# huakunyang/SummerTTS

Hardware: AMD Instinct MI355X
Metric: audio samples/sec (acoustic model + vocoder, phoneme ids -> int16 PCM on host), single_speaker_fast-shaped synthetic blob (higher is better)
Workload: dtype f32 (decoder trunk convs AND the reverse flow's WaveNet convs (wn_flow.hip, one-utterance calls): fp32 operands as 2 fp16 terms = 22-23 of their 24 mantissa bits, 3 fp16 MFMA products per fp32 product, f32 accumulation -- measured error in `parity`, same tolerance as the exact-fp32 leg; batches addi

## Files before the change

include/summertts_hip.h:

```cpp
#ifndef SUMMERTTS_HIP_H_
#define SUMMERTTS_HIP_H_

#include <stdint.h>

#ifdef __cplusplus
extern "C" {
#endif

typedef struct sts_engine sts_engine;

enum {
    STS_OK = 0,
    STS_EINVAL = -1,
    STS_EMODEL = -2,
    STS_EDEVICE = -3,
    STS_ESTATE = -4
};

int sts_create(const float* blob, int64_t blob_bytes, int device, sts_engine** out);
void sts_destroy(sts_engine* e);

int sts_speaker_num(const sts_engine* e);

typedef struct sts_model_info {
    int32_t is_multi_speaker, lang_type, dur_pred_type, dec_type;
    int32_t vocab, hidden, inter_channels, speaker_num, gin_channels;
    int32_t samples_per_frame;
    int32_t sample_rate;
    int64_t blob_floats_consumed;
} sts_model_info;
int sts_get_info(const sts_engine* e, sts_model_info* info);

int sts_infer_ids(sts_engine* e, const int32_t* ids, int32_t n, int32_t sid, float length_scale,
                  int16_t** pcm_out, int32_t* n_out);

typedef int (*sts_chunk_cb)(void* user, const int16_t* pcm, int32_t n_samples, int32_t sample_offset);
int sts_infer_ids_stream(sts_engine* e, const int32_t* ids, int32_t n, int32_t sid, float length_scale,
                         int32_t chunk_frames, sts_chunk_cb cb, void* user, int32_t* n_total);
int sts_stream_halo_frames(const sts_engine* e);

typedef int (*sts_batch_chunk_cb)(void* user, int32_t utt, const int16_t* pcm, int32_t n_samples, int32_t sample_offset);
int sts_infer_ids_batch_stream(sts_engine* e, int32_t B, const int32_t* const* ids, const int32_t* n, const int32_t* sid,
                               const float* length_scale, int32_t chunk_frames, sts_batch_chunk_cb cb, void* user,
                               int32_t* n_total);

int sts_infer_ids_batch(sts_engine* e, int32_t B, const int32_t* const* ids, const int32_t* n,
                        const int32_t* sid, const float* length_scale, int16_t** pcm_out, int32_t* n_out);

int sts_run_batch(sts_engine* e, int32_t B, const int32_t* const* ids, const int32_t* n, const int32_t* sid,
                  const float* length_scale, int32_t* n_out, int64_t* total_out);
int sts_set_host_pcm(sts_engine* e, int enable);
int sts_copy_pcm_device(sts_engine* e, void* device_dst, int64_t capacity_samples);
int sts_copy_pcm_host(sts_engine* e, int16_t* host_dst, int64_t capacity_samples);
int sts_pcm_host_view(sts_engine* e, const int16_t** pcm, int64_t* count);

int sts_set_forced_durations(sts_engine* e, const int32_t* dur, int64_t count);
int sts_set_noise(sts_engine* e, float noise_scale, float noise_scale_w, uint64_t seed);
int sts_get_noise(const sts_engine* e, float* noise_scale, float* noise_scale_w, uint64_t* seed);
int sts_set_output_rate(sts_engine* e, int32_t rate);
int sts_get_output_rate(const sts_engine* e);
int sts_resample_table(int32_t in_rate, int32_t out_rate, int32_t* P, int32_t* Q, int32_t* taps, float* table, int64_t capacity_floats);
#define STS_LOUD_OFF 0
#define STS_LOUD_MEASURE 1
#define STS_LOUD_NORMALIZE 2
typedef struct sts_loudness { float lufs; float peak; float gain; int32_t blocks; } sts_loudness;
int sts_set_loudness(sts_engine* e, int mode, float target_lufs, float peak_dbfs);
int sts_get_loudness_mode(const sts_engine* e, int* mode, float* target_lufs, float* peak_dbfs);
int sts_get_loudness(sts_engine* e, sts_loudness* out, int64_t capacity);
int sts_kweight_coeffs(int32_t rate, double coeffs[10]);
int sts_loudness_measure(int device, const float* x, const int64_t* lengths, int32_t B, int32_t rate,
                         float target_lufs, float peak_dbfs, sts_loudness* out);
#define STS_LIMITER_OFF 0
#define STS_LIMITER_ON 1
typedef struct sts_limiter_stats { float gain; float min_gain; float peak_out; int32_t limited; } sts_limiter_stats;
int sts_set_limiter(sts_engine* e, int mode, float gain_db, float ceiling_dbfs, float lookahead_ms);
int sts_get_limiter_mode(const sts_engine* e, int* mode, float* gain_db, float* ceiling_dbfs, float* lookahead_ms);
int sts_get_limiter(sts_engine* e, sts_limiter_stats* out, int64_t capacity);
int sts_limiter_design(int32_t rate, float gain_db, float ceiling_dbfs, float lookahead_ms, int32_t* H, double* c, double* G);
int sts_limiter_apply(int device, const float* x, const int64_t* lengths, int32_t B, int32_t rate, float gain_db, float ceiling_dbfs,
                      float lookahead_ms, float* y, int16_t* pcm, sts_limiter_stats* stats);
int sts_set_record_taps(sts_engine* e, int enable);
int sts_get_tap(sts_engine* e, const char* name, float** data, int32_t* channels, int64_t* length);
int sts_get_durations(sts_engine* e, int32_t* dur, int64_t capacity);
int sts_set_conv_mode(sts_engine* e, int mode);
int sts_set_conv_math(sts_engine* e, int mode);

enum { STS_DBG_ATTN_BLOCK_MIN_WGS = 1,
       STS_DBG_TAIL_FUSED = 14 ,
       STS_DBG_UPS_ROWPH = 15 ,
       STS_DBG_CHAIN_STREAMS = 13 ,
       STS_DBG_H2P = 11 ,
       STS_DBG_H2P_TILE = 12 ,
       STS_DBG_MEMO_CLEAR = 10 ,
       STS_DBG_PCM_DIRECT = 9 ,
       STS_DBG_DDS_TAIL = 8 ,
       STS_DBG_ATTN_REG = 7 ,
       STS_DBG_LAUNCH_AHEAD = 6 ,
       STS_DBG_FLOW_FUSED = 5  };
enum { STS_DBG_STREAM_RETRY_STEP = 16, STS_DBG_STREAM_DIRECT = 17 };
enum { STS_DBG_POISON = 18 };
int sts_debug_set(sts_engine* e, int key, int value);

typedef struct sts_profile {
    float ms_text_encoder, ms_duration, ms_flow, ms_decoder, ms_total_device;
    float ms_decoder_mfma;
    int32_t decoder_mfma_launches;
    double flops_text_encoder, flops_duration, flops_flow, flops_decoder;
    double flops_decoder_mfma;
    double bytes_decoder_min;
    int64_t frames, samples, phonemes;
    double flops_decoder_mfma_executed;
    double bytes_text_encoder, bytes_duration, bytes_flow;
    float ms_sync_wait_host;
    double flops_decoder_bf16_issued;
    int64_t conv_math_fallbacks;
    int32_t conv_math_pinned;
    int32_t launch_ahead;
    int64_t launch_ahead_misses;
    float us_host_setup;
    float us_host_enqueue;
    float us_host_tail;
    int64_t poison_bytes;
} sts_profile;
int sts_set_profiling(sts_engine* e, int enable);
#define STS_ABI_VERSION 13
int sts_abi_version(void);
int sts_build_flags(void);
int sts_get_profile(const sts_engine* e, sts_profile* p);
int sts_get_profile_ex(const sts_engine* e, void* p, int64_t size_bytes);

int sts_debug_conv1d(int device, const float* x, int32_t Cin, int32_t L, const float* w, const float* bias,
                     int32_t Cout, int32_t k, int32_t pad, int32_t dil, int32_t stride_transposed,
                     int32_t depthwise, float in_slope, int32_t in_act, int mode, float** y, int32_t* Lout);

int sts_debug_conv1d_bench(int device, const float* x, int32_t Cin, int32_t L, const float* w, const float* bias,
                           int32_t Cout, int32_t k, int32_t pad, int32_t dil, int32_t stride_transposed,
                           int32_t depthwise, float in_slope, int32_t in_act, int mode, float** y, int32_t* Lout,
                           int32_t iters, float* ms_out);

int sts_debug_conv_h2p(int device, const float* x, int32_t Cin, int32_t L, const float* w, const float* bias, int32_t Cout, int32_t k,
                       int32_t dil, const float* res, float in_slope, float out_slope, int tile, int members, float* y, float* y16,
                       float* yp, int32_t iters, float* ms_out);

int sts_debug_conv_h2w(int device, const float* x, int32_t C, int32_t L, const float* w, const float* bias, int32_t k, int32_t dil, const float* res,
                       float in_slope, float out_slope, int members, float* y, float* y16, int32_t iters, float* ms_out);

void sts_free(void* p);
const char* sts_last_error(void);

int sts_debug_wino_pack(const float* w, int32_t Cout, int32_t k, int32_t Cin, float* out, int64_t out_floats);

typedef struct sts_pool sts_pool;
int sts_pool_create(const float* blob, int64_t blob_bytes, int device, int n_engines, int max_batch, sts_pool** out);
void sts_pool_destroy(sts_pool* p);
int64_t sts_pool_submit(sts_pool* p, const int32_t* ids, int32_t n, int32_t sid, float length_scale);
int sts_pool_wait(sts_pool* p, int64_t ticket, int16_t** pcm_out, int32_t* n_out);
int sts_pool_stats(sts_pool* p, int64_t* batches, int64_t* requests);
const char* sts_pool_last_error(void);
int64_t sts_pool_submit_ex(sts_pool* p, const int32_t* ids, int32_t n, int32_t sid, float length_scale, float noise_scale,
                           float noise_scale_w, uint64_t seed);
int sts_pool_set_output_rate(sts_pool* p, int32_t rate);
int64_t sts_pool_submit_stream(sts_pool* p, const int32_t* ids, int32_t n, int32_t sid, float length_scale, float noise_scale,
                               float noise_scale_w, uint64_t seed, int32_t chunk_frames, sts_chunk_cb cb, void* user);
int sts_pool_set_loudness(sts_pool* p, int mode, float target_lufs, float peak_dbfs);
int sts_pool_set_limiter(sts_pool* p, int mode, float gain_db, float ceiling_dbfs, float lookahead_ms);

typedef struct sts_multi sts_multi;
int sts_multi_create(const float* blob, int64_t blob_bytes, const int32_t* devices, int32_t n_devices, sts_multi** out);
enum { STS_MULTI_AUTO = 0, STS_MULTI_RCCL = 1, STS_MULTI_DOWNLOAD = 2 };
int sts_multi_create_ex(const float* blob, int64_t blob_bytes, const int32_t* devices, int32_t n_devices, int32_t flags, sts_multi** out);
int sts_multi_gather_mode(const sts_multi* m);
int sts_multi_rccl_ranks(sts_multi* m);
double sts_multi_last_gather_ms(const sts_multi* m);
int sts_multi_set_conv_math(sts_multi* m, int mode);
int sts_multi_set_noise(sts_multi* m, float noise_scale, float noise_scale_w, uint64_t seed);
int sts_multi_set_output_rate(sts_multi* m, int32_t rate);
int sts_multi_set_loudness(sts_multi* m, int mode, float target_lufs, float peak_dbfs);
int sts_multi_set_limiter(sts_multi* m, int mode, float gain_db, float ceiling_dbfs, float lookahead_ms);
int sts_multi_set_rccl_library(const char* path, int allow_repeated_devices);
int64_t sts_multi_gather_layout(const int64_t* counts, int32_t n_ranks, int64_t* offsets);
void sts_multi_destroy(sts_multi* m);
int sts_multi_device_count(const sts_multi* m);
int sts_multi_speaker_num(const sts_multi* m);
int sts_multi_infer_ids_batch(sts_multi* m, int32_t B, const int32_t* const* ids, const int32_t* n, const int32_t* sid,
                              const float* length_scale, int16_t** pcm_out, int32_t* n_out);
int sts_multi_shard_of(const sts_multi* m, int32_t B, const int32_t* n, int32_t* device_slot_out);
const char* sts_multi_last_error(void);

#ifdef __cplusplus
}
#endif
#endif
```

summertts_amd/csrc/capi.hip:

```cpp
#include <stdlib.h>
#include <string.h>

#include <algorithm>
#include <new>
#include <string>
#include <vector>

#include "engine.hpp"

using namespace sts;

struct sts_engine { Engine eng; };

static thread_local std::string g_err;
static int set_err(int code, const std::string& s) { g_err = s; return code; }

extern "C" {

const char* sts_last_error(void) { return g_err.c_str(); }
void sts_free(void* p) { free(p); }

int sts_create(const float* blob, int64_t blob_bytes, int device, sts_engine** out) {
    if (!out) return set_err(STS_EINVAL, "sts_create: null out pointer");
    *out = nullptr;
// ... 19 lines not shown
    info->vocab = m.vocab; info->hidden = m.hidden; info->inter_channels = m.inter;
    info->speaker_num = m.spk_num == 0 ? 1 : m.spk_num; info->gin_channels = m.gin;
    info->samples_per_frame = m.hop_total; info->sample_rate = kNativeRate;
    info->blob_floats_consumed = m.consumed;
    return STS_OK;
}

int sts_run_batch(sts_engine* e, int32_t B, const int32_t* const* ids, const int32_t* n, const int32_t* sid,
                  const float* length_scale, int32_t* n_out, int64_t* total_out) {
    if (!e) return set_err(STS_EINVAL, "null engine");
    int rc = e->eng.run(B, ids, n, sid, length_scale);
    if (rc != STS_OK) return set_err(rc, e->eng.error());
    if (n_out) for (int b = 0; b < B; b++) n_out[b] = e->eng.n_samples[b];
    if (total_out) *total_out = e->eng.total_samples;
    return STS_OK;
}

int sts_copy_pcm_device(sts_engine* e, void* dst, int64_t cap) {
    if (!e || !dst) return set_err(STS_EINVAL, "null argument");
    if (cap < e->eng.total_samples || !e->eng.d_pcm) return set_err(STS_ESTATE, "destination too small or no run yet");
    if (hipMemcpyAsync(dst, e->eng.pcm_in_host_ ? (const void*)e->eng.h_pcm : (const void*)e->eng.d_pcm, (size_t)e->eng.total_samples * 2,
                       e->eng.pcm_in_host_ ? hipMemcpyHostToDevice : hipMemcpyDeviceToDevice, e->eng.stream) != hipSuccess ||
        hipStreamSynchronize(e->eng.stream) != hipSuccess)
        return set_err(STS_EDEVICE, "device copy failed");
    return STS_OK;
}

int sts_copy_pcm_host(sts_engine* e, int16_t* dst, int64_t cap) {
    if (!e || !dst) return set_err(STS_EINVAL, "null argument");
    if (cap < e->eng.total_samples || !e->eng.d_pcm) return set_err(STS_ESTATE, "destination too small or no run yet");
    if (e->eng.h_pcm) { memcpy(dst, e->eng.h_pcm, (size_t)e->eng.total_samples * 2); return STS_OK; }
    if (hipMemcpyAsync(dst, e->eng.d_pcm, (size_t)e->eng.total_samples * 2, hipMemcpyDeviceToHost, e->eng.stream) != hipSuccess ||
        hipStreamSynchronize(e->eng.stream) != hipSuccess)
        return set_err(STS_EDEVICE, "device-to-host copy failed");
    return STS_OK;
}

int sts_pcm_host_view(sts_engine* e, const int16_t** pcm, int64_t* count) {
    if (!e || !pcm || !count) return set_err(STS_EINVAL, "null argument");
    if (!e->eng.h_pcm || !e->eng.d_pcm) return set_err(STS_ESTATE, "no host copy of the PCM (sts_set_host_pcm(e, 1) before the run)");
    *pcm = e->eng.h_pcm; *count = e->eng.total_samples;
    return STS_OK;
}

int sts_infer_ids_batch(sts_engine* e, int32_t B, const int32_t* const* ids, const int32_t* n, const int32_t* sid,
                        const float* length_scale, int16_t** pcm_out, int32_t* n_out) {
    if (!pcm_out || !n_out) return set_err(STS_EINVAL, "null output");
    int64_t total = 0;
    if (!e) return set_err(STS_EINVAL, "null engine");
    const bool was = e->eng.host_pcm;
    e->eng.host_pcm = true;
    int rc = sts_run_batch(e, B, ids, n, sid, length_scale, n_out, &total);
    e->eng.host_pcm = was;
    if (rc != STS_OK) return rc;
    int16_t* all = (int16_t*)malloc((size_t)(total > 0 ? total : 1) * 2);
    if (!all) return set_err(STS_EDEVICE, "out of host memory");
    rc = sts_copy_pcm_host(e, all, total);
    if (rc != STS_OK) { free(all); return rc; }
    int64_t off = 0;
    for (int b = 0; b < B; b++) {
        if (B == 1) { pcm_out[0] = all; break; }
        pcm_out[b] = (int16_t*)malloc((size_t)(n_out[b] > 0 ? n_out[b] : 1) * 2);
        if (!pcm_out[b]) {
            for (int q = 0; q < b; q++) { free(pcm_out[q]); pcm_out[q] = nullptr; }
            free(all);
            return set_err(STS_EDEVICE, "out of host memory");
        }
        memcpy(pcm_out[b], all + off, (size_t)n_out[b] * 2);
        off += n_out[b];
    }
    if (B != 1) free(all);
    return STS_OK;
}

int sts_infer_ids(sts_engine* e, const int32_t* ids, int32_t n, int32_t sid, float length_scale, int16_t** pcm_out,
                  int32_t* n_out) {
    const int32_t* idp[1] = {ids};
    return sts_infer_ids_batch(e, 1, idp, &n, &sid, &length_scale, pcm_out, n_out);
}

int sts_infer_ids_stream(sts_engine* e, const int32_t* ids, int32_t n, int32_t sid, float length_scale, int32_t chunk_frames,
                         sts_chunk_cb cb, void* user, int32_t* n_total) {
    if (!e || !ids || !cb) return set_err(STS_EINVAL, "null argument");
    const int32_t* idp[1] = {ids};
    StreamSpec ss{chunk_frames, cb, user};
    const int rc = e->eng.run(1, idp, &n, &sid, &length_scale, &ss);
    if (rc != STS_OK) return set_err(rc, e->eng.error());
    if (n_total) *n_total = (int32_t)e->eng.total_samples;
    return STS_OK;
}

int sts_infer_ids_batch_stream(sts_engine* e, int32_t B, const int32_t* const* ids, const int32_t* n, const int32_t* sid,
                               const float* length_scale, int32_t chunk_frames, sts_batch_chunk_cb cb, void* user, int32_t* n_total) {
    if (!e) return set_err(STS_EINVAL, "null engine");
    if (B < 1 || !ids || !n || chunk_frames <= 0 || !cb) return set_err(STS_EINVAL, "B >= 1, ids, n, a positive chunk size and a callback are required");
    const int rc = e->eng.run_batch_stream(B, ids, n, sid, length_scale, chunk_frames, cb, user, n_total);
    if (rc != STS_OK) return set_err(rc, e->eng.error());
    return STS_OK;
}

int sts_stream_halo_frames(const sts_engine* e) {
    if (!e) return set_err(STS_EINVAL, "null engine");
    return e->eng.stream_halo();
}

int sts_set_forced_durations(sts_engine* e, const int32_t* dur, int64_t count) {
    if (!e) return set_err(STS_EINVAL, "null engine");
    if (!dur || count <= 0) { e->eng.have_forced = false; return STS_OK; }
    e->eng.forced_dur.assign(dur, dur + count);
    e->eng.have_forced = true;
    return STS_OK;
}

int sts_set_noise(sts_engine* e, float noise_scale, float noise_scale_w, uint64_t seed) {
    if (!e) return set_err(STS_EINVAL, "null engine");
    if (!noise_scale_valid(noise_scale) || !noise_scale_valid(noise_scale_w)) return set_err(STS_EINVAL, "noise scales must be finite and >= 0");
    e->eng.noise = Engine::Noise{noise_scale, noise_scale_w, seed};
    return STS_OK;
}
int sts_get_noise(const sts_engine* e, float* noise_scale, float* noise_scale_w, uint64_t* seed) {
    if (!e) return set_err(STS_EINVAL, "null engine");
    if (noise_scale) *noise_scale = e->eng.noise.ns;
    if (noise_scale_w) *noise_scale_w = e->eng.noise.nsw;
    if (seed) *seed = e->eng.noise.seed;
    return STS_OK;
}
int sts_set_record_taps(sts_engine* e, int enable) { if (!e) return set_err(STS_EINVAL, "null engine"); e->eng.record_taps = enable != 0; return STS_OK; }
int sts_set_conv_math(sts_engine* e, int mode) {
    if (!e) return set_err(STS_EINVAL, "null engine");
    if (mode < 0 || mode > 3) return set_err(STS_EINVAL, "conv math: 0 = split-bf16 (default), 1 = exact fp32, 2 = split-bf16 wherever eligible, 3 = two-term fp16");
    e->eng.conv_math = mode;
    e->eng.h2_consecutive = 0; e->eng.h2_disabled = false;
    return STS_OK;
}
int sts_set_conv_mode(sts_engine* e, int mode) { if (!e) return set_err(STS_EINVAL, "null engine"); e->eng.conv_mode = mode; return STS_OK; }
int sts_debug_set(sts_engine* e, int key, int value) {
    if (!e) return set_err(STS_EINVAL, "null engine");
    switch (key) {
        case STS_DBG_ATTN_BLOCK_MIN_WGS: if (value < 1) return set_err(STS_EINVAL, "threshold must be >= 1"); e->eng.attn_block_min_wgs = value; return STS_OK;
        case STS_DBG_FLOW_FUSED: e->eng.flow_fused = value != 0; return STS_OK;
        case STS_DBG_LAUNCH_AHEAD: if (value < 0 || value > 2) return set_err(STS_EINVAL, "launch_ahead must be 0, 1 or 2"); if ((value == 2) != (e->eng.launch_ahead == 2)) { e->eng.seen_tf_.clear(); e->eng.seen_order_.clear(); } e->eng.launch_ahead = value; return STS_OK;
        case STS_DBG_H2P: e->eng.h2p = value < 0 ? 0 : (value > 4 ? 4 : value); return STS_OK;
        case STS_DBG_H2P_TILE: e->eng.h2p_tile = value; return STS_OK;
        case STS_DBG_CHAIN_STREAMS: e->eng.chain_streams_dbg = value; return STS_OK;
        case STS_DBG_TAIL_FUSED: e->eng.tail_fused = value != 0; return STS_OK;
        case STS_DBG_UPS_ROWPH: e->eng.ups_rowph = value != 0; return STS_OK;
        case STS_DBG_MEMO_CLEAR: e->eng.seen_tf_.clear(); e->eng.seen_order_.clear(); return STS_OK;
        case STS_DBG_ATTN_REG: e->eng.attn_reg = value != 0; return STS_OK;
        case STS_DBG_DDS_TAIL: e->eng.dds_tail = value != 0; return STS_OK;
        case STS_DBG_PCM_DIRECT: e->eng.pcm_direct = value != 0; return STS_OK;
        case STS_DBG_STREAM_RETRY_STEP: e->eng.stream_retry_step = value < 0 ? -1 : value; return STS_OK;
        case STS_DBG_STREAM_DIRECT: e->eng.stream_direct = value != 0; return STS_OK;
        case STS_DBG_POISON: e->eng.poison = (unsigned)value; return STS_OK;
        default: return set_err(STS_EINVAL, "unknown debug key");
    }
}
int sts_set_host_pcm(sts_engine* e, int enable) { if (!e) return set_err(STS_EINVAL, "null engine"); e->eng.host_pcm = enable != 0; return STS_OK; }
int sts_set_profiling(sts_engine* e, int enable) { if (!e) return set_err(STS_EINVAL, "null engine"); e->eng.profiling = enable == 2 ? 2 : (enable != 0 ? 1 : 0); return STS_OK; }

int sts_abi_version(void) { return STS_ABI_VERSION; }

int sts_set_output_rate(sts_engine* e, int32_t rate) {
    if (!e) return set_err(STS_EINVAL, "null engine");
    const int rc = e->eng.set_output_rate(rate);
    return rc == STS_OK ? STS_OK : set_err(rc, e->eng.error());
}
int sts_get_output_rate(const sts_engine* e) {
    if (!e) return set_err(STS_EINVAL, "null engine");
    return e->eng.out_rate;
}
int sts_resample_table(int32_t in_rate, int32_t out_rate, int32_t* P, int32_t* Q, int32_t* taps, float* table, int64_t capacity_floats) {
    ResampleDesign d;
    if (!resample_design(in_rate, out_rate, &d)) return set_err(STS_EINVAL, "rates must be integers in [8000, 48000] with P = out / gcd(in, out) <= 1024");
    const int64_t need = (int64_t)d.P * 2 * d.K;
    if (table && capacity_floats < need) return set_err(STS_EINVAL, "table capacity below P * taps floats");
    if (P) *P = d.P;
    if (Q) *Q = d.Q;
    if (taps) *taps = 2 * d.K;
    if (table) resample_table(d, in_rate, out_rate, table);
    return STS_OK;
}
int sts_set_loudness(sts_engine* e, int mode, float target_lufs, float peak_dbfs) {
    if (!e) return set_err(STS_EINVAL, "null engine");
    const int rc = e->eng.set_loudness(mode, target_lufs, peak_dbfs);
    return rc == STS_OK ? STS_OK : set_err(rc, e->eng.error());
}
int sts_get_loudness_mode(const sts_engine* e, int* mode, float* target_lufs, float* peak_dbfs) {
    if (!e) return set_err(STS_EINVAL, "null engine");
    if (mode) *mode = e->eng.loud_mode;
    if (target_lufs) *target_lufs = e->eng.loud_target;
    if (peak_dbfs) *peak_dbfs = e->eng.loud_peak;
    return STS_OK;
}
int sts_get_loudness(sts_engine* e, sts_loudness* out, int64_t capacity) {
    if (!e) return set_err(STS_EINVAL, "null engine");
    const int64_t n = (int64_t)e->eng.loud_res.size();
    if (!out) return (int)n;
    if (capacity < n) return set_err(STS_EINVAL, "capacity below the last call's utterance count");
    if (n > 0) memcpy(out, e->eng.loud_res.data(), (size_t)n * sizeof(sts_loudness));
    return (int)n;
}
int sts_kweight_coeffs(int32_t rate, double coeffs[10]) {
    if (!coeffs) return set_err(STS_EINVAL, "null argument");
    if (!kweight_coeffs(rate, coeffs)) return set_err(STS_EINVAL, "rate must be an integer in [8000, 48000]");
    return STS_OK;
}
int sts_loudness_measure(int device, const float* x, const int64_t* lengths, int32_t B, int32_t rate, float target_lufs, float peak_dbfs,
                         sts_loudness* out) {
    if (B < 1 || !lengths || !out) return set_err(STS_EINVAL, "B >= 1, lengths and out are required");
    if (!loudness_args_valid(2, target_lufs, peak_dbfs)) return set_err(STS_EINVAL, "target in [-70, 0] LUFS, ceiling in [-30, 0] dBFS");
    LoudArgs a{};
    if (!loud_coef(rate, &a.k)) return set_err(STS_EINVAL, "rate must be an integer in [8000, 48000]");
    std::vector<int> len(B);
    int64_t total = 0, maxl = 0;
    for (int b = 0; b < B; b++) {
        if (lengths[b] < 0 || lengths[b] > (int64_t)1 << 30) return set_err(STS_EINVAL, "lengths must be in [0, 2^30]");
        len[b] = (int)lengths[b]; total += lengths[b]; maxl = std::max<int64_t>(maxl, lengths[b]);
    }
    if (total > 0 && !x) return set_err(STS_EINVAL, "null signal");
    if (hipSetDevice(device) != hipSuccess) return set_err(STS_EDEVICE, "no such device");
    const size_t ws = loud_ws_bytes(B, total), xb = (((size_t)total * 4 + 255) & ~(size_t)255), lb = (((size_t)B * 4 + 255) & ~(size_t)255);
    const size_t ob = (size_t)B * sizeof(sts_loudness);
    char* d = nullptr;
    if (hipMalloc((void**)&d, xb + lb + ob + ws) != hipSuccess) return set_err(STS_EDEVICE, "out of device memory");
    hipStream_t st = nullptr;
    bool ok = hipStreamCreate(&st) == hipSuccess;
    a.x = (const float*)d; a.len = (const int*)(d + xb); a.ilen = 0; a.scale = 1; a.P = 1; a.Q = 1;
    a.target = target_lufs; a.ceiling = peak_dbfs;
    a.out = (float*)(d + xb + lb);
    loud_ws_carve(a, d + xb + lb + ob, B, total);
    ok = ok && (total == 0 || hipMemcpyAsync(d, x, (size_t)total * 4, hipMemcpyHostToDevice, st) == hipSuccess) &&
         hipMemcpyAsync(d + xb, len.data(), (size_t)B * 4, hipMemcpyHostToDevice, st) == hipSuccess;
    if (ok) {
        loudness_run(a, B, maxl, nullptr, st);
        ok = hipGetLastError() == hipSuccess && hipMemcpyAsync(out, a.out, ob, hipMemcpyDeviceToHost, st) == hipSuccess &&
             hipStreamSynchronize(st) == hipSuccess;
    }
    if (st) (void)hipStreamDestroy(st);
    (void)hipFree(d);
    return ok ? STS_OK : set_err(STS_EDEVICE, "loudness measurement failed on the device");
}
int sts_set_limiter(sts_engine* e, int mode, float gain_db, float ceiling_dbfs, float lookahead_ms) {
    if (!e) return set_err(STS_EINVAL, "null engine");
    const int rc = e->eng.set_limiter(mode, gain_db, ceiling_dbfs, lookahead_ms);
    return rc == STS_OK ? STS_OK : set_err(rc, e->eng.error());
}
int sts_get_limiter_mode(const sts_engine* e, int* mode, float* gain_db, float* ceiling_dbfs, float* lookahead_ms) {
    if (!e) return set_err(STS_EINVAL, "null engine");
    if (mode) *mode = e->eng.lim_mode;
    if (gain_db) *gain_db = e->eng.lim_gain_db;
    if (ceiling_dbfs) *ceiling_dbfs = e->eng.lim_ceiling;
    if (lookahead_ms) *lookahead_ms = e->eng.lim_ms;
    return STS_OK;
}
int sts_get_limiter(sts_engine* e, sts_limiter_stats* out, int64_t capacity) {
    if (!e) return set_err(STS_EINVAL, "null engine");
    const int64_t n = (int64_t)e->eng.lim_res.size();
    if (!out) return (int)n;
    if (capacity < n) return set_err(STS_EINVAL, "capacity below the last call's utterance count");
    if (n > 0) memcpy(out, e->eng.lim_res.data(), (size_t)n * sizeof(sts_limiter_stats));
    return (int)n;
}
int sts_limiter_design(int32_t rate, float gain_db, float ceiling_dbfs, float lookahead_ms, int32_t* H, double* c, double* G) {
    LimiterDesign d;
    if (!limiter_design(rate, gain_db, ceiling_dbfs, lookahead_ms, &d))
        return set_err(STS_EINVAL, "rate in [8000, 48000], gain in [-40, 40] dB, ceiling in [-30, 0] dBFS, look-ahead in [0.25, 10] ms");
    if (H) *H = d.H;
    if (c) *c = d.c;
    if (G) *G = d.G;
    return STS_OK;
}
int sts_limiter_apply(int device, const float* x, const int64_t* lengths, int32_t B, int32_t rate, float gain_db, float ceiling_dbfs,
                      float lookahead_ms, float* y, int16_t* pcm, sts_limiter_stats* stats) {
    if (B < 1 || !lengths) return set_err(STS_EINVAL, "B >= 1 and lengths are required");
    LimiterDesign dsg;
    if (!limiter_design(rate, gain_db, ceiling_dbfs, lookahead_ms, &dsg))
        return set_err(STS_EINVAL, "rate in [8000, 48000], gain in [-40, 40] dB, ceiling in [-30, 0] dBFS, look-ahead in [0.25, 10] ms");
    std::vector<int> len(B);
    int64_t total = 0, maxl = 0;
    for (int b = 0; b < B; b++) {
        if (lengths[b] < 0 || lengths[b] > (int64_t)1 << 30) return set_err(STS_EINVAL, "lengths must be in [0, 2^30]");
        len[b] = (int)lengths[b]; total += lengths[b]; maxl = std::max<int64_t>(maxl, lengths[b]);
    }
    if (total > (int64_t)1 << 30) return set_err(STS_EINVAL, "the signals must hold at most 2^30 samples in all");
    if (total > 0 && !x) return set_err(STS_EINVAL, "null signal");
    if (hipSetDevice(device) != hipSuccess) return set_err(STS_EDEVICE, "no such device");
    const size_t xb = (((size_t)total * 4 + 255) & ~(size_t)255), lb = (((size_t)B * 4 + 255) & ~(size_t)255);
    const size_t pb = (((size_t)total * 2 + 255) & ~(size_t)255), sb = (((size_t)B * 16 + 255) & ~(size_t)255);
    char* d = nullptr;
    if (hipMalloc((void**)&d, 2 * xb + lb + pb + sb + 256) != hipSuccess) return set_err(STS_EDEVICE, "out of device memory");
    hipStream_t st = nullptr;
    bool ok = hipStreamCreate(&st) == hipSuccess;
    LimArgs a{};
    a.x = (const float*)d; a.len = (const int*)(d + xb); a.ilen = 0; a.scale = 1; a.P = 1; a.Q = 1;
    a.H = dsg.H; a.c = dsg.c; a.G = dsg.G; a.gloud = nullptr;
    a.y = y ? (float*)(d + xb + lb) : nullptr;
    a.pcm = pcm ? (int16_t*)(d + 2 * xb + lb) : nullptr;
    a.stat = (unsigned*)(d + 2 * xb + lb + pb);
    std::vector<unsigned> raw((size_t)B * 4);
    ok = ok && (total == 0 || hipMemcpyAsync(d, x, (size_t)total * 4, hipMemcpyHostToDevice, st) == hipSuccess) &&
         hipMemcpyAsync(d + xb, len.data(), (size_t)B * 4, hipMemcpyHostToDevice, st) == hipSuccess;
    if (ok) {
        limiter_run(a, B, maxl, st);
        ok = hipGetLastError() == hipSuccess &&
             (!y || total == 0 || hipMemcpyAsync(y, a.y, (size_t)total * 4, hipMemcpyDeviceToHost, st) == hipSuccess) &&
             (!pcm || total == 0 || hipMemcpyAsync(pcm, a.pcm, (size_t)total * 2, hipMemcpyDeviceToHost, st) == hipSuccess) &&
// ... 351 lines not shown
```

summertts_amd/csrc/conv.hip:

```cpp
#include "kernels.hpp"
#include "devmath.hpp"
#include "conv_common.hpp"

namespace sts {

__device__ __forceinline__ float load_in(const ConvArgs& a, const float* xrow, int pos, int in_len, int orig_len) {
    if (pos < 0 || pos >= in_len) return 0.f;
    int src = pos;
    if (a.in_reflect) {
        src = pos - 1;
        if (src < 0) { if (orig_len > 1) src = 1; else return 0.f; }
    }
    float v = xrow[src];
    if (a.in_act) v = v < 0.f ? v * a.in_slope : v;
    return v;
}

#ifndef STS_EXP
#define STS_EXP 0
#endif

#ifndef STS_RA_GROUP
#define STS_RA_GROUP 3
#endif
template <int MW, int NW, int WM, int WN, int RA = 3>
__device__ __forceinline__ void conv_mfma_body(const ConvArgs& a, const int mtiles, const int bx, const int by, const int b) {
    constexpr int MT = 32 * MW * WM, NT = 32 * NW * WN, NTHR = WM * WN * 64;
    extern __shared__ __attribute__((aligned(16))) float smem[];
    const int orig_len = uni(seg_len(a.in_seg, b));
    const int in_len = orig_len + (a.in_reflect ? 1 : 0);
    const int out_len = uni(seg_len(a.out_seg, b));
    const int n_count = a.transposed ? in_len + a.n_extra : out_len;
    const int n0 = bx * NT;
    if (n0 >= n_count) return;
    const int phase = by / mtiles;
    const int m0 = (by - phase * mtiles) * MT;
    const size_t in_base = (size_t)uni(seg_start(a.in_seg, b)), out_base = (size_t)uni(seg_start(a.out_seg, b));
    const float* const xbase = uni(a.x);
    const long x_ld = uni(a.x_ld);
    const int tid = threadIdx.x, lane = tid & 63, wave = tid >> 6;
    const int wm = wave / WN, wn = wave % WN;
    const int l31 = lane & 31, half = lane >> 5;

    const int first = a.tap_off, last = a.tap_off + (a.ntap - 1) * a.tap_step;
    const int lo = first < last ? first : last, hi = first < last ? last : first;
    const int W = NT + (hi - lo);
    constexpr int WIN = NT + MAX_HALO;
    constexpr int ldsw = WIN;
    const int win0 = n0 + lo;

    const float* w = a.w + (size_t)phase * a.ntap * a.Cin_pad * a.Cout_pad;
    const int mbase = m0 + wm * MW * 32;
    f32x16 acc[MW][NW];
#pragma unroll
    for (int i = 0; i < MW; i++)
#pragma unroll
        for (int j = 0; j < NW; j++)
#pragma unroll
            for (int r = 0; r < 16; r++) acc[i][j][r] = 0.f;

    const int nchunk = a.Cin_pad / CK;
    const int nsteps = nchunk * a.ntap;

    const rsrc_t wrs = make_rsrc(w, (unsigned)((size_t)a.ntap * a.Cin_pad * a.Cout_pad * 4));
    const unsigned a_voff = (unsigned)(((size_t)half * a.Cout_pad + mbase + l31) * 4);
    auto load_a = [&](int c, int j, float (&dst)[CK / 2][MW]) {
        const unsigned sbase = (unsigned)((((size_t)j * a.Cin_pad + (size_t)c * CK) * a.Cout_pad) * 4);
#pragma unroll
        for (int p = 0; p < CK / 2; p++)
#pragma unroll
            for (int i = 0; i < MW; i++)
                dst[p][i] = __builtin_bit_cast(float, __builtin_amdgcn_raw_buffer_load_b32(
                    wrs, (int)a_voff, (int)(sbase + (unsigned)(2 * p) * (unsigned)a.Cout_pad * 4u + (unsigned)i * 128u), 0));
    };
    auto load_b = [&](int bufi, int j, float (&dst)[CK / 2][NW]) {
        const float* sb = smem + bufi * (CK * ldsw);
        const int bcol0 = wn * NW * 32 + l31 + j * a.tap_step + a.tap_off - lo;
#pragma unroll
        for (int p = 0; p < CK / 2; p++)
#pragma unroll
            for (int q = 0; q < NW; q++) dst[p][q] = sb[(2 * p + half) * ldsw + bcol0 + q * 32];
    };

    constexpr int RI = (NT + MAX_HALO + NTHR - 1) / NTHR;
    unsigned xoff[RI];
#pragma unroll
    for (int i = 0; i < RI; i++) {
        const int col = tid + i * NTHR;
        const int pos = win0 + col;
        bool v = col < W && pos >= 0 && pos < in_len;
        int src = pos;
        if (a.in_reflect) { src = pos - 1; if (src < 0) { src = 1; v = v && orig_len > 1; } }
        xoff[i] = v ? (unsigned)src * 4u : kOOB;
    }
    float xr[CK][RI];
    int sj = 0, sc = 0;
    auto load_x = [&](int c) {
        if (STS_EXP & 1) { if (c > 0) return; }
#pragma unroll
        for (int i = 0; i < RI; i++)
            if ((i + 1) * NTHR <= WIN || tid < WIN - i * NTHR) {
#pragma unroll
                for (int r = 0; r < CK; r++) {
                    const int ci = c * CK + r;
                    const rsrc_t rs = make_rsrc(xbase + (size_t)ci * x_ld + in_base, ci < a.Cin ? (unsigned)orig_len * 4u : 0u);
                    xr[r][i] = buf_load(rs, xoff[i]);
                }
            }
    };
    auto store_tile = [&](int bufi) {
        if (STS_EXP & 8) { if (bufi >= 0 && sc > 0) return; }
        float* sb = smem + bufi * (CK * ldsw);
#pragma unroll
        for (int i = 0; i < RI; i++)
            if ((i + 1) * NTHR <= WIN || tid < WIN - i * NTHR) {
#pragma unroll
                for (int r = 0; r < CK; r++) {
                    float v = xr[r][i];
                    if (a.in_act) v = v < 0.f ? v * a.in_slope : v;
                    sb[r * ldsw + tid + i * NTHR] = v;
                }
            }
    };

    constexpr int UNR = (RA % 2 == 0) ? RA : 2 * RA;
    float fa[RA][CK / 2][MW], fb[2][CK / 2][NW];
    int aj = 0, ac = 0;
    auto request_a = [&](float (&dst)[CK / 2][MW]) {
        if (!(STS_EXP & 2) || (ac == 0 && aj < 2)) load_a(ac, aj, dst);
        if (++aj == a.ntap) { aj = 0; ac++; }
    };
    auto do_step = [&](float (&acur)[CK / 2][MW], float (&anew)[CK / 2][MW], float (&bcur)[CK / 2][NW],
                       float (&bnxt)[CK / 2][NW], int s) {
        const bool last_tap = sj + 1 == a.ntap;
        int nj = sj + 1, nc = sc;
        if (last_tap) { nj = 0; nc = sc + 1; }
        request_a(anew);
        {
            if (last_tap && s + 1 < nsteps) {
                store_tile(nc & 1);
                if (!(STS_EXP & 4)) __syncthreads();
                if (nc + 1 < nchunk) load_x(nc + 1);
            }
            if (!(STS_EXP & 16)) load_b(nc & 1, nj, bnxt);
        }
#pragma unroll
        for (int p = 0; p < CK / 2; p++)
#pragma unroll
            for (int i = 0; i < MW; i++)
#pragma unroll
                for (int q = 0; q < NW; q++)
                    acc[i][q] = __builtin_amdgcn_mfma_f32_32x32x2f32(acur[p][i], bcur[p][q], acc[i][q], 0, 0, 0);
        sj = nj; sc = nc;
    };
// ... 499 lines not shown
            if (ns == nseg) { ns = 0; nh = sh + 1; if (nh == 2) { nh = 0; nc = sc + 1; } }
            const bool more = s + 1 < nsteps;
            const bool three = ss < n3;
            float v[4];
            load_a(sc, sh, ss, 3, fa[3]);
#pragma unroll
            for (int p = 0; p < 4; p++) v[p] = X[0][p] - X[2][p];
#pragma unroll
            for (int p = 0; p < 4; p++) acc[0] = __builtin_amdgcn_mfma_f32_32x32x2f32(fa[0][p], v[p], acc[0], 0, 0, 0);
            load_a(nc, nh, ns, 0, fa[0]);
#pragma unroll
            for (int p = 0; p < 4; p++) v[p] = X[1][p] + X[2][p];
#pragma unroll
            for (int p = 0; p < 4; p++) acc[1] = __builtin_amdgcn_mfma_f32_32x32x2f32(fa[1][p], v[p], acc[1], 0, 0, 0);
            load_a(nc, nh, ns, 1, fa[1]);
#pragma unroll
            for (int p = 0; p < 4; p++) v[p] = X[2][p] - X[1][p];
#pragma unroll
            for (int p = 0; p < 4; p++) acc[2] = __builtin_amdgcn_mfma_f32_32x32x2f32(fa[2][p], v[p], acc[2], 0, 0, 0);
            load_a(nc, nh, ns, 2, fa[2]);
#pragma unroll
            for (int p = 0; p < 4; p++) v[p] = X[1][p] - X[3][p];
            if (more) {
                if (nc != sc) {
                    store_x(nc & 1, 1);
                    __syncthreads();
                    if (nc + 1 < nchunk) load_x(nc + 1, 0);
                } else if (nh != sh) {
                    if (sc + 1 < nchunk) { store_x((sc + 1) & 1, 0); load_x(sc + 1, 1); }
                }
                load_xv(nc & 1, nh, ns);
            }
            if (three) {
#pragma unroll
                for (int p = 0; p < 4; p++) acc[3] = __builtin_amdgcn_mfma_f32_32x32x2f32(fa[3][p], v[p], acc[3], 0, 0, 0);
            }
            ss = ns; sh = nh; sc = nc;
        }
    }
    __syncthreads();
    {
        const int q = l31 / d, rr = l31 - q * d;
        const int pa = 60 * wn + 2 * d * q + rr, pb = pa + d;
        const int ga = n0 - h2 + pa, gb = n0 - h2 + pb;
        const bool ia = ga >= 0 && ga < len, ib = gb >= 0 && gb < len;
        if (l31 < 30) {
            float b1v[16];
#pragma unroll
            for (int r = 0; r < 16; r++) b1v[r] = a.b1 ? a.b1[m0 + (r & 3) + 8 * (r >> 2) + 4 * half] : 0.f;
            static_for<0, 16>([&](auto rc) {
                constexpr int r = decltype(rc)::value;
                const int row = m0 + (r & 3) + 8 * (r >> 2) + 4 * half;
                const float bv = b1v[r];
                float ya = acc[0][r] + acc[1][r] + acc[2][r] + bv;
                float yb = acc[1][r] - acc[2][r] - acc[3][r] + bv;
                ya = ya < 0.f ? ya * G.slope : ya;
                yb = yb < 0.f ? yb * G.slope : yb;
                t1[row * LD2 + (pa & 1) * H2 + (pa >> 1)] = ia ? ya : 0.f;
                t1[row * LD2 + (pb & 1) * H2 + (pb >> 1)] = ib ? yb : 0.f;
            });
        }
#pragma unroll
        for (int i = 0; i < 4; i++)
#pragma unroll
            for (int r = 0; r < 16; r++) acc[i][r] = 0.f;
    }
    __syncthreads();

    {
        int n3, n2; wino_split(a.k2, &n3, &n2);
        const int nseg = n3 + n2, nsteps = nchunk * 2 * nseg;
        const rsrc_t wrs = make_rsrc(a.wu2, (unsigned)(nseg * 4 * C * C * 4));
        auto load_a = [&](int c, int h, int sg, int xi, float (&dst)[4]) {
            const unsigned sbase = ((unsigned)sg * 4u + (unsigned)xi) * xi_stride + (unsigned)((c * CK + h * 8) * C) * 4u;
#pragma unroll
            for (int p = 0; p < 4; p++)
                dst[p] = __builtin_bit_cast(float, __builtin_amdgcn_raw_buffer_load_b32(wrs, (int)a_voff, (int)(sbase + (unsigned)(2 * p * C * 4)), 0));
        };
        auto load_xv = [&](int c, int h, int sg) {
            const int j0 = sg < n3 ? 3 * sg : 3 * n3 + 2 * (sg - n3);
            const float* sb = t1 + (c * CK + h * 8 + half) * LD2 + 30 * wn + l31;
#pragma unroll
            for (int m = 0; m < 4; m++) {
                const int j = j0 + m;
                const float* sm = sb + (j & 1) * H2 + (j >> 1);
#pragma unroll
                for (int p = 0; p < 4; p++) X[m][p] = sm[2 * p * LD2];
            }
        };
        int sc = 0, sh = 0, ss = 0;
        load_a(0, 0, 0, 0, fa[0]);
        load_a(0, 0, 0, 1, fa[1]);
        load_a(0, 0, 0, 2, fa[2]);
        load_xv(0, 0, 0);
        for (int s = 0; s < nsteps; s++) {
            int ns = ss + 1, nh = sh, nc = sc;
            if (ns == nseg) { ns = 0; nh = sh + 1; if (nh == 2) { nh = 0; nc = sc + 1; } }
            const bool more = s + 1 < nsteps;
            const bool three = ss < n3;
            float v[4];
            load_a(sc, sh, ss, 3, fa[3]);
#pragma unroll
            for (int p = 0; p < 4; p++) v[p] = X[0][p] - X[2][p];
#pragma unroll
            for (int p = 0; p < 4; p++) acc[0] = __builtin_amdgcn_mfma_f32_32x32x2f32(fa[0][p], v[p], acc[0], 0, 0, 0);
            load_a(nc, nh, ns, 0, fa[0]);
#pragma unroll
            for (int p = 0; p < 4; p++) v[p] = X[1][p] + X[2][p];
#pragma unroll
            for (int p = 0; p < 4; p++) acc[1] = __builtin_amdgcn_mfma_f32_32x32x2f32(fa[1][p], v[p], acc[1], 0, 0, 0);
            load_a(nc, nh, ns, 1, fa[1]);
#pragma unroll
            for (int p = 0; p < 4; p++) v[p] = X[2][p] - X[1][p];
#pragma unroll
            for (int p = 0; p < 4; p++) acc[2] = __builtin_amdgcn_mfma_f32_32x32x2f32(fa[2][p], v[p], acc[2], 0, 0, 0);
            load_a(nc, nh, ns, 2, fa[2]);
#pragma unroll
            for (int p = 0; p < 4; p++) v[p] = X[1][p] - X[3][p];
            load_xv(more ? nc : 0, nh, ns);
            if (three) {
#pragma unroll
                for (int p = 0; p < 4; p++) acc[3] = __builtin_amdgcn_mfma_f32_32x32x2f32(fa[3][p], v[p], acc[3], 0, 0, 0);
            }
            ss = ns; sh = nh; sc = nc;
        }
    }
    if (l31 < 30) {
        const int oa = 60 * wn + 2 * l31, ob = oa + 1;
        const bool va = oa < NT && n0 + oa < len, vb = ob < NT && n0 + ob < len;
        const size_t opos = base + (size_t)(n0 + oa);
        static_for<0, 2>([&](auto hc) {
            constexpr int hb = decltype(hc)::value * 8;
            float b2v[8], xa[8], xb[8];
#pragma unroll
            for (int r = 0; r < 8; r++) {
                const int row = m0 + ((hb + r) & 3) + 8 * ((hb + r) >> 2) + 4 * half;
                const size_t o = (size_t)row * G.ld + opos;
                b2v[r] = a.b2 ? a.b2[row] : 0.f;
                xa[r] = va ? a.x[o] : 0.f;
                xb[r] = vb ? a.x[o + 1] : 0.f;
            }
            static_for<0, 8>([&](auto rc) {
                constexpr int r = decltype(rc)::value;
                const int row = m0 + ((hb + r) & 3) + 8 * ((hb + r) >> 2) + 4 * half;
                const float bv = b2v[r];
                const float ya = acc[0][hb + r] + acc[1][hb + r] + acc[2][hb + r] + bv;
                const float yb = acc[1][hb + r] - acc[2][hb + r] - acc[3][hb + r] + bv;
                const size_t o = (size_t)row * G.ld + opos;
                if (va) a.y[o] = ya + xa[r];
                if (vb) a.y[o + 1] = yb + xb[r];
            });
        });
    }
}

template <int MW, int NW>
__global__ __launch_bounds__(1024) void conv_mfma_splitk_kernel(ConvArgs a, int mtiles) {
    constexpr int G = 4, E = MW * NW * 16;
    constexpr int D = MW * NW == 1 ? 6 : (MW * NW == 2 ? 4 : 3);
    extern __shared__ __attribute__((aligned(16))) float red[];
    const int KS = blockDim.x >> 6;
    const int nsl = a.kslices > 1 ? a.kslices : 1;
    const int b = blockIdx.z / nsl, slice = blockIdx.z - b * nsl;
    const int orig_len = seg_len(a.in_seg, b);
    const int in_len = orig_len + (a.in_reflect ? 1 : 0);
    const int out_len = seg_len(a.out_seg, b);
    const int n_count = a.transposed ? in_len + a.n_extra : out_len;
    const int n0 = blockIdx.x * 32 * NW;
    if (n0 >= n_count) return;
    const int phase = blockIdx.y / mtiles;
    const int m0 = (blockIdx.y - phase * mtiles) * 32 * MW;
    const size_t in_base = (size_t)seg_start(a.in_seg, b), out_base = (size_t)seg_start(a.out_seg, b);
    const int tid = threadIdx.x, lane = tid & 63, wave = tid >> 6;
    const int l31 = lane & 31, half = lane >> 5;
    const float* w = a.w + (size_t)phase * a.ntap * a.Cin_pad * a.Cout_pad;
    bool mvalid[MW];
#pragma unroll
    for (int i = 0; i < MW; i++) mvalid[i] = (m0 + i * 32) < a.Cout_pad;

    f32x16 acc[MW][NW];
#pragma unroll
    for (int i = 0; i < MW; i++)
#pragma unroll
        for (int q = 0; q < NW; q++)
#pragma unroll
            for (int r = 0; r < 16; r++) acc[i][q][r] = 0.f;

    const int gpt = a.Cin_pad / (2 * G);
    const int gall = a.ntap * gpt;
    const int gper = (gall + nsl - 1) / nsl;
    const int gfirst = slice * gper;
    const int ngroups = (STS_EXP & 64) ? gfirst : (gfirst + gper < gall ? gfirst + gper : gall);
    float ra[D][G][MW], rb[D][G][NW];
    const int swave = __builtin_amdgcn_readfirstlane(wave);
    const int sKS = __builtin_amdgcn_readfirstlane(KS);
    const rsrc_t xrs = make_rsrc(a.x + in_base, (unsigned)(((size_t)(a.Cin - 1) * a.x_ld + orig_len) * 4));
    const rsrc_t wrs = make_rsrc(w, (unsigned)((size_t)a.ntap * a.Cin_pad * a.Cout_pad * 4));
    const unsigned ld4 = (unsigned)a.x_ld * 4u;
    const unsigned x_lane = (unsigned)half * ld4;
    const unsigned a_lane = (unsigned)(((size_t)half * a.Cout_pad + m0 + l31) * 4);
    const int lanepos = n0 + l31;
    int lj = (gfirst + swave) / gpt, lc = (gfirst + swave - lj * gpt) * 2 * G;
    const int jstep = sKS / gpt, cstep = (sKS - jstep * gpt) * 2 * G;

    auto load_group = [&](float (&fa)[G][MW], float (&fb)[G][NW]) {
        const int shift = lj * a.tap_step + a.tap_off;
        unsigned off[NW];
#pragma unroll
        for (int q = 0; q < NW; q++) {
            int pos = lanepos + q * 32 + shift;
            bool v = pos >= 0 && pos < in_len;
            if (a.in_reflect) { pos = pos - 1; if (pos < 0) { pos = 1; v = v && orig_len > 1; } }
            off[q] = v ? (unsigned)pos * 4u + x_lane : kOOB;
        }
        const unsigned xs0 = (unsigned)lc * ld4;
        const unsigned ws0 = (unsigned)((((size_t)lj * a.Cin_pad + lc) * a.Cout_pad) * 4);
#pragma unroll
        for (int i = 0; i < G; i++) {
            const bool cv = lc + 2 * i + half < a.Cin;
#pragma unroll
            for (int q = 0; q < NW; q++)
                fb[i][q] = __builtin_bit_cast(float, __builtin_amdgcn_raw_buffer_load_b32(xrs, (int)(cv ? off[q] : kOOB), (int)(xs0 + (unsigned)(2 * i) * ld4), 0));
#pragma unroll
            for (int k = 0; k < MW; k++)
                fa[i][k] = __builtin_bit_cast(float, __builtin_amdgcn_raw_buffer_load_b32(
                    wrs, (int)a_lane, (int)(ws0 + (unsigned)(2 * i) * (unsigned)a.Cout_pad * 4u + (unsigned)k * 128u), 0));
        }
        lj += jstep; lc += cstep;
        if (lc >= a.Cin_pad) { lc -= a.Cin_pad; lj++; }
    };

    int gnext = gfirst + swave;
#pragma unroll
    for (int d = 0; d < D; d++) { if (gnext < ngroups) load_group(ra[d], rb[d]); gnext += sKS; }
    int gcur = gfirst + swave;
    while (gcur < ngroups) {
#pragma unroll
        for (int d = 0; d < D; d++) {
            if (gcur < ngroups) {
#pragma unroll
                for (int i = 0; i < G; i++) {
                    float bq[NW];
#pragma unroll
                    for (int q = 0; q < NW; q++) {
                        float v = rb[d][i][q];
                        if (a.in_act) v = v < 0.f ? v * a.in_slope : v;
                        bq[q] = v;
                    }
#pragma unroll
                    for (int k = 0; k < MW; k++)
#pragma unroll
                        for (int q = 0; q < NW; q++)
                            acc[k][q] = __builtin_amdgcn_mfma_f32_32x32x2f32(ra[d][i][k], bq[q], acc[k][q], 0, 0, 0);
                }
                if (gnext < ngroups) load_group(ra[d], rb[d]);
            }
            gnext += sKS; gcur += sKS;
        }
    }

    static_for<0, MW>([&](auto ic) {
        constexpr int i = decltype(ic)::value;
        static_for<0, NW>([&](auto qc) {
            constexpr int q = decltype(qc)::value;
            static_for<0, 16>([&](auto rc) {
                constexpr int r = decltype(rc)::value;
                red[((size_t)wave * E + (i * NW + q) * 16 + r) * 64 + lane] = acc[i][q][r];
            });
        });
    });
    __syncthreads();
    const int out_off = a.out_off + phase;
    const bool gate = a.epi == EPI_GATE;
    for (int e = wave; e < E; e += KS) {
        const int i = e / (NW * 16);
        const int q = (e >> 4) % NW, r = e & 15;
        if (gate && r >= 8) continue;
        const int n = n0 + q * 32 + l31;
        const int pos = n * a.out_stride + out_off;
        if (n >= n_count || pos < 0 || pos >= out_len) continue;
        const size_t opos = out_base + (size_t)pos;
        const int rowp = m0 + i * 32 + (r & 3) + 8 * (r >> 2) + 4 * half;
        float v = 0.f, v2 = 0.f;
        for (int k = 0; k < KS; k++) {
            v += red[((size_t)k * E + (i * NW + q) * 16 + r) * 64 + lane];
            if (gate) v2 += red[((size_t)k * E + (i * NW + q) * 16 + r + 8) * 64 + lane];
        }
        if (gate) {
            if (!mvalid[i]) continue;
            if (a.bias) { v += a.bias[rowp]; v2 += a.bias[rowp + 16]; }
            if (a.ubias) { v += a.ubias[(size_t)rowp * a.ubias_ld + b]; v2 += a.ubias[(size_t)(rowp + 16) * a.ubias_ld + b]; }
            const int ch = (rowp >> 5) * 16 + (rowp & 15);
            if (ch < a.H) a.y[(size_t)ch * a.y_ld + opos] = tanh_ref(v) * sigmoid_ref(v2);
        } else {
            if (rowp >= a.Cout) continue;
            if (nsl > 1) {
                if (slice == 0) { if (a.bias) v += a.bias[rowp]; if (a.ubias) v += a.ubias[(size_t)rowp * a.ubias_ld + b]; }
                a.y[(size_t)slice * a.kslice_stride + (size_t)rowp * a.y_ld + opos] = v;
                continue;
            }
            if (a.bias) v += a.bias[rowp];
            if (a.ubias) v += a.ubias[(size_t)rowp * a.ubias_ld + b];
            epi_scalar(a, rowp, opos, v);
        }
    }
}

struct TileCfg { int MW, NW, WM, WN; };
static const TileCfg kTiles[] = {
    {2, 2, 2, 2},
    {2, 2, 1, 4},
    {1, 4, 1, 4},
    {2, 1, 1, 4},
    {1, 1, 1, 4},
    {1, 2, 1, 4},
};
constexpr int kNumTiles = 6;

bool conv_mfma_eligible(const ConvArgs& a) {
    if (a.depthwise) return false;
    if (a.Cin < 32) return false;
    if (a.Cout < 8 && a.max_n >= 4096) return false;
    if (a.Cin_pad % CK != 0 || a.Cout_pad % 32 != 0) return false;
    int first = a.tap_off, last = a.tap_off + (a.ntap - 1) * a.tap_step;
    int halo = first < last ? last - first : first - last;
    if (halo > MAX_HALO) return false;
    if (a.epi == EPI_GATE && !a.gate_perm) return false;
    if (a.epi == EPI_TANH_PCM) return false;
    return true;
}

static int pick_tile(const ConvArgs& a, int nphase) {
    const long nt = (a.max_n + 127) / 128;
    if (a.Cout_pad % 64 == 0 && nt * (a.Cout_pad / 64) * nphase * a.B >= 512) return 3;
    return 4;
}

template <int MW, int NW, int WM, int WN>
static void launch_mfma(const ConvArgs& a, int nphase, hipStream_t st) {
    constexpr int MT = 32 * MW * WM, NT = 32 * NW * WN;
    const int mt = (a.Cout_pad + MT - 1) / MT;
    const int nx = (a.max_n + NT - 1) / NT, ny = mt * nphase;
    size_t lds = (size_t)2 * CK * (NT + MAX_HALO) * sizeof(float);
    hipLaunchKernelGGL((conv_mfma_kernel<MW, NW, WM, WN>), dim3(mapped_grid(nx, ny, a.B)), dim3(WM * WN * 64), lds, st, a, mt, nx, ny);
}

template <int MW, int NW>
static void launch_splitk(const ConvArgs& a, int nphase, hipStream_t st) {
    const int mt = (a.Cout_pad + 32 * MW - 1) / (32 * MW);
    const int nt = (a.max_n + 32 * NW - 1) / (32 * NW);
    const int nsl = a.kslices > 1 ? a.kslices : 1;
    const long steps = ((long)a.ntap * (a.Cin_pad / 8) + nsl - 1) / nsl;
    constexpr int E = MW * NW * 16;
    const bool sparse = (long)mt * nt * nphase * a.B * nsl <= 256;
    const int ks_cap = E <= 16 ? 16 : (E <= 32 ? (sparse ? 16 : 8) : 4);
    int ks = 1;
    while (ks < ks_cap && steps / (ks * 2) >= 6 && (long)mt * nt * nphase * a.B * nsl * ks * 2 <= 4096) ks *= 2;
    dim3 grid(nt, mt * nphase, a.B * nsl);
    size_t lds = (size_t)ks * E * 64 * sizeof(float);
    hipLaunchKernelGGL((conv_mfma_splitk_kernel<MW, NW>), grid, dim3(ks * 64), lds, st, a, mt);
}

template <int MW, int NW, int WM, int WN>
static void launch_mfma_group(const ConvGroup& G, hipStream_t st) {
    constexpr int MT = 32 * MW * WM, NT = 32 * NW * WN;
    const ConvArgs& a = G.g[0];
    const int mt = (a.Cout_pad + MT - 1) / MT;
    const int nx = (a.max_n + NT - 1) / NT;
    size_t lds = (size_t)2 * CK * (NT + MAX_HALO) * sizeof(float);
    hipLaunchKernelGGL((conv_mfma_group_kernel<MW, NW, WM, WN>), dim3(mapped_grid(nx, mt, a.B * G.n)), dim3(WM * WN * 64), lds, st, G,
                       mt, a.B, nx, mt);
}

bool resblock_layer_eligible(const ResLayerGroup& G) {
    if (G.n < 1 || G.n > kMaxGroup || (G.C != 32 && G.C != 64 && G.C != 128) || G.max_n <= 0 || G.B <= 0) return false;
    for (int i = 0; i < G.n; i++) {
        const ResLayerArgs& a = G.g[i];
        if (!(a.k1 & 1) || !(a.k2 & 1) || a.k1 < 1 || a.k2 < 1) return false;
        if (a.dil1 * (a.k1 - 1) > RL_XW - RL_W1 || a.k2 - 1 > 32) return false;
        if (a.x == a.y) return false;
    }
    return true;
}

void resblock_layer(const ResLayerGroup& Gin, hipStream_t st) {
    ResLayerGroup G = Gin;
    for (int i = 1; i < G.n; i++)
        for (int j = i; j > 0 && G.g[j].k1 + G.g[j].k2 > G.g[j - 1].k1 + G.g[j - 1].k2; j--) {
            ResLayerArgs t = G.g[j]; G.g[j] = G.g[j - 1]; G.g[j - 1] = t;
        }
    int nx = 0;
    for (int i = 0; i < G.n; i++) {
        const int NT = RL_W1 - (G.g[i].k2 - 1);
        const int n = (G.max_n + NT - 1) / NT;
        if (n > nx) nx = n;
    }
    const size_t stage = (size_t)2 * CK * RL_XW, park = (size_t)G.C * RL_W1 + 64;
    const size_t lds = (stage > park ? stage : park) * sizeof(float);
    const dim3 grid(mapped_grid(nx, 1, G.B * G.n));
    if (G.C == 32) hipLaunchKernelGGL((resblock_layer_kernel<1, 1>), grid, dim3(256), lds, st, G, nx);
    else if (G.C == 64) hipLaunchKernelGGL((resblock_layer_kernel<2, 1>), grid, dim3(256), lds, st, G, nx);
    else hipLaunchKernelGGL((resblock_layer_kernel<2, 2>), grid, dim3(512), lds, st, G, nx);
}

bool conv_wino_eligible(const ConvArgs& a) {
    if (!a.wu || a.transposed || a.depthwise || a.in_reflect || a.out_stride != 1 || a.out_off != 0) return false;
    const int d = a.tap_step;
    if (d <= 0 || d > 6 || 30 % d != 0 || a.ntap < 2) return false;
    if (a.Cin_pad % CK != 0 || a.Cout_pad % 32 != 0 || a.Cin < 32) return false;
    if ((a.ntap - 1) * d > MAX_HALO || 121 + d * ((a.ntap + 1) / 2) >= WINO_H) return false;
    if (a.epi == EPI_GATE || a.epi == EPI_TANH_PCM) return false;
    int n3, n2; wino_split(a.ntap, &n3, &n2);
    return n3 == a.wino_n3 && n2 == a.wino_n2 && n3 >= 0;
}
static size_t wino_lds() { return (size_t)2 * CK * WINO_LD * sizeof(float); }
void conv_wino(const ConvArgs& a, hipStream_t st) {
    if (a.max_n <= 0 || a.B <= 0) return;
    const int nx = (a.max_n + WINO_NT - 1) / WINO_NT, ny = a.Cout_pad / 32;
    hipLaunchKernelGGL(conv_wino_kernel, dim3(mapped_grid(nx, ny, a.B)), dim3(256), wino_lds(), st, a, nx, ny);
}
void wino_pack(const float* w, long s_out, long s_tap, long s_in, int Cout, int k, int Cin, int Cin_pad, int Cout_pad, float* dst) {
    int n3, n2; wino_split(k, &n3, &n2);
    const int nseg = n3 + n2;
    const size_t slab = (size_t)Cin_pad * Cout_pad;
    for (size_t i = 0; i < (size_t)nseg * 4 * slab; i++) dst[i] = 0.f;
    for (int sg = 0; sg < nseg; sg++) {
        const int j0 = sg < n3 ? 3 * sg : 3 * n3 + 2 * (sg - n3), len = sg < n3 ? 3 : 2;
        for (int o = 0; o < Cout; o++)
            for (int ci = 0; ci < Cin; ci++) {
                double g[3] = {0, 0, 0};
                for (int t = 0; t < len; t++) g[t] = (double)w[(size_t)o * s_out + (size_t)(j0 + t) * s_tap + (size_t)ci * s_in];
                const double u[4] = {g[0], 0.5 * (g[0] + g[1] + g[2]), 0.5 * (g[0] - g[1] + g[2]), g[2]};
                for (int xi = 0; xi < 4; xi++) dst[((size_t)sg * 4 + xi) * slab + (size_t)ci * Cout_pad + o] = (float)u[xi];
            }
    }
}

bool resblock_wino_eligible(const ResLayerGroup& G) {
    if (!resblock_layer_eligible(G)) return false;
    for (int i = 0; i < G.n; i++) {
        const ResLayerArgs& a = G.g[i];
        if (!a.wu1 || !a.wu2 || a.k1 < 2 || a.k2 < 2 || a.k2 > 15) return false;
        if (a.dil1 < 1 || a.dil1 > 6 || 30 % a.dil1 != 0 || (a.k1 - 1) * a.dil1 > MAX_HALO) return false;
    }
    return true;
}

template <int WM, int WN>
static void launch_resblock_wino(const ResLayerGroup& G, hipStream_t st) {
    constexpr int P = 60 * WN, LD1 = 2 * (30 * WN + 40), LD2 = 2 * (30 * WN + 16);
    int nx = 0;
    for (int i = 0; i < G.n; i++) {
        const int NT = P - (G.g[i].k2 - 1);
        const int n = (G.max_n + NT - 1) / NT;
        if (n > nx) nx = n;
    }
    const size_t stage = (size_t)2 * CK * LD1, park = (size_t)32 * WM * LD2 + 64;
    const size_t lds = (stage > park ? stage : park) * sizeof(float);
    hipLaunchKernelGGL((resblock_wino_kernel<WM, WN>), dim3(mapped_grid(nx, 1, G.B * G.n)), dim3(64 * WM * WN), lds, st, G, nx);
}

void resblock_wino(const ResLayerGroup& Gin, hipStream_t st) {
    ResLayerGroup G = Gin;
    for (int i = 1; i < G.n; i++)
        for (int j = i; j > 0 && G.g[j].k1 + G.g[j].k2 > G.g[j - 1].k1 + G.g[j - 1].k2; j--) {
            ResLayerArgs t = G.g[j]; G.g[j] = G.g[j - 1]; G.g[j - 1] = t;
        }
    if (G.C == 32) launch_resblock_wino<1, 4>(G, st);
    else if (G.C == 64) launch_resblock_wino<2, 2>(G, st);
    else launch_resblock_wino<4, 2>(G, st);
}

bool conv_group_eligible(const ConvGroup& G) {
    if (G.n < 2 || G.n > kMaxGroup) return false;
    const ConvArgs& r = G.g[0];
    for (int i = 0; i < G.n; i++) {
        const ConvArgs& a = G.g[i];
        if (!conv_mfma_eligible(a) || a.transposed || a.epi == EPI_GATE) return false;
        if (a.Cout_pad != r.Cout_pad || a.max_n != r.max_n || a.B != r.B) return false;
    }
    return true;
}

void conv_mfma_group(const ConvGroup& Gin, hipStream_t st, int tile) {
    ConvGroup G = Gin;
    if (G.g[0].max_n <= 0 || G.g[0].B <= 0) return;
    for (int i = 1; i < G.n; i++)
        for (int j = i; j > 0 && (long)G.g[j].ntap * G.g[j].Cin_pad > (long)G.g[j - 1].ntap * G.g[j - 1].Cin_pad; j--) {
            ConvArgs t = G.g[j]; G.g[j] = G.g[j - 1]; G.g[j - 1] = t;
        }
    if (tile != 1 && tile != 3 && tile != 4 && tile != 5) {
        const ConvArgs& a = G.g[0];
        const long nt = (a.max_n + 127) / 128;
        tile = (a.Cout_pad % 64 == 0 && nt * (a.Cout_pad / 64) * a.B * G.n >= 1024) ? 3 : 4;
    }
    switch (tile) {
        case 1: launch_mfma_group<2, 2, 1, 4>(G, st); break;
        case 3: launch_mfma_group<2, 1, 1, 4>(G, st); break;
        case 5: launch_mfma_group<1, 2, 1, 4>(G, st); break;
        default: launch_mfma_group<1, 1, 1, 4>(G, st); break;
    }
}

void conv_mfma(const ConvArgs& a, hipStream_t st, int tile) {
    int nphase = a.transposed ? a.out_stride : 1;
    if (a.max_n <= 0 || a.B <= 0) return;
    bool splitk = tile == 6 || tile == 7 || a.kslices > 1;
    int nw = tile == 7 ? 2 : 1;
    if (a.kslices > 1 && tile != 7) tile = 6;
    if (tile < 0 || tile > 7) {
        tile = pick_tile(a, nphase);
        const TileCfg& t = kTiles[tile];
// ... 206 lines not shown
```

summertts_amd/csrc/engine.hip:

```cpp
#include "run_ctx.hpp"
#include <time.h>
#include "knobs.hpp"
#include "../../include/tts_logger.h"

#include <algorithm>
#include <chrono>
#include <math.h>
#include <stdlib.h>
#include <string.h>
#include <thread>

namespace sts {

Engine::~Engine() {
    if (stream) (void)hipStreamSynchronize(stream);
    free_model(model);
    if (arenaT_.base) (void)hipFree(arenaT_.base);
    if (arenaF_.base) (void)hipFree(arenaF_.base);
    if (pinned_) (void)hipHostFree(pinned_);
    if (pinned_pcm_) (void)hipHostFree(pinned_pcm_);
    if (d_rs_table) (void)hipFree(d_rs_table);
    if (loud_host_) (void)hipHostFree(loud_host_);
    if (lim_host_) (void)hipHostFree(lim_host_);
    if (ovf_host_) (void)hipHostFree(ovf_host_);
    if (hmap_) (void)hipHostFree(hmap_);
    if (arrive_) (void)hipFree(arrive_);
    if (have_events_) {
        for (auto& e : ev_) (void)hipEventDestroy(e);
        (void)hipEventDestroy(ev_fork_);
        if (ev_setup_) (void)hipEventDestroy(ev_setup_);
        for (auto& e : ev_join_) (void)hipEventDestroy(e);
        for (auto& a : aux_) if (a) (void)hipStreamDestroy(a);
    }
    if (stream) (void)hipStreamDestroy(stream);
}

static int default_conv_math();
static inline void cpu_relax() {
#if defined(__x86_64__) || defined(__i386__)
    __builtin_ia32_pause();
#elif defined(__aarch64__) || defined(__arm__)
    asm volatile("yield" ::: "memory");
#else
    std::this_thread::yield();
#endif
}

int Engine::init(const float* blob, int64_t bytes, int dev) {
    conv_math = default_conv_math();
    int count = 0;
    if (hipGetDeviceCount(&count) != hipSuccess || count <= 0)
        return fail(STS_EDEVICE, "no HIP device visible: the SummerTTS HIP engine needs an AMD GPU (gfx950) -- there is no CPU fallback");
    if (dev < 0 || dev >= count) return fail(STS_EINVAL, "device index out of range");
    device = dev;
    HIPCK(hipSetDevice(dev));
    HIPCK(hipStreamCreateWithFlags(&stream, hipStreamNonBlocking));
    for (auto& e : ev_) HIPCK(hipEventCreate(&e));
    HIPCK(hipEventCreateWithFlags(&ev_fork_, hipEventDisableTiming));
    HIPCK(hipEventCreateWithFlags(&ev_setup_, hipEventDisableTiming));
    for (auto& e : ev_join_) HIPCK(hipEventCreateWithFlags(&e, hipEventDisableTiming));
    {
        int lo = 0, hi = 0;
        (void)hipDeviceGetStreamPriorityRange(&lo, &hi);
        for (int k = 0; k < kAux; k++) {
            int pr = lo + (hi - lo) * k / (kAux > 1 ? kAux - 1 : 1);
            HIPCK(hipStreamCreateWithPriority(&aux_[k], hipStreamNonBlocking, pr));
        }
    }
    cur_ = stream;
    have_events_ = true;
    if (!blob || bytes < 32) return fail(STS_EMODEL, "model blob too small");
    if (!load_model(blob, bytes / (int64_t)sizeof(float), model)) return fail(STS_EMODEL, "model parse failed: " + model.error);
    return STS_OK;
}

bool Engine::ensure(Arena& a, size_t bytes) {
    if (bytes <= a.cap) return true;
    (void)hipStreamSynchronize(stream);
    if (a.base) (void)hipFree(a.base);
    a.base = nullptr; a.cap = 0;
    size_t want = bytes + bytes / 4 + (1u << 20);
    if (hipMalloc((void**)&a.base, want) != hipSuccess) { if (hipMalloc((void**)&a.base, bytes) != hipSuccess) return false; want = bytes; }
    a.cap = want;
    return true;
}

bool Engine::ensure_pinned(size_t bytes) {
    if (bytes <= pinned_cap_) return true;
    (void)hipStreamSynchronize(stream);
    if (pinned_) (void)hipHostFree(pinned_);
    pinned_ = nullptr; pinned_cap_ = 0;
    size_t want = bytes * 2 + 4096;
    if (hipHostMalloc((void**)&pinned_, want, hipHostMallocDefault) != hipSuccess) return false;
    pinned_cap_ = want;
    return true;
}

void Engine::poison_arena(const Arena& a) {
    if (!poison || !a.base || a.used == 0) return;
    const size_t words = (a.used + 3) / 4;
    if (hipMemsetD32Async((hipDeviceptr_t)a.base, (int)poison, words, stream) == hipSuccess) poison_bytes_ += (int64_t)words * 4;
}
void Engine::poison_host16(void* p, size_t samples) {
    if (!poison || !p) return;
    const uint16_t v = (uint16_t)(poison & 0xffffu);
    uint16_t* q = (uint16_t*)p;
    for (size_t i = 0; i < samples; i++) q[i] = v;
    poison_bytes_ += (int64_t)samples * 2;
}
void Engine::poison_host32(void* p, size_t words) {
    if (!poison || !p) return;
    uint32_t* q = (uint32_t*)p;
    for (size_t i = 0; i < words; i++) q[i] = poison;
    poison_bytes_ += (int64_t)words * 4;
}

void Engine::stage_begin(int s) { cur_stage_ = s; }
static double now_us() { return std::chrono::duration<double, std::micro>(std::chrono::steady_clock::now().time_since_epoch()).count(); }
void Engine::mark(int i) { if (profiling == 1 || (profiling == 2 && (i == 5 || i == 6))) (void)hipEventRecord(ev_[i], stream); }

static int default_conv_math() {
    const char* v = getenv("STS_CONV_MATH");
    if (!v || !*v) return 3;
    if (!strcmp(v, "f16x2") || !strcmp(v, "3")) return 3;
    if (!strcmp(v, "bf16x3") || !strcmp(v, "0")) return 0;
    if (!strcmp(v, "f32") || !strcmp(v, "fp32") || !strcmp(v, "1")) return 1;
    tts_log(TTS_LOG_WARNING, (std::string("summertts_hip: STS_CONV_MATH=") + v + " is not one of f16x2 | bf16x3 | f32 -- ignored, the default (f16x2) applies\n").c_str());
    return 3;
}

ConvArgs Engine::conv_args(const DConv& c, const float* x, const Lvl& lin, float* y, const Lvl& lout, const ConvOpt& o, double* flops) {
    ConvArgs a;
    memset(&a, 0, sizeof(a));
    a.x = x; a.x_ld = lin.ld; a.y = y; a.y_ld = lout.ld;
    a.w = c.w; a.wb3 = c.wb3; a.bias = c.bias; a.ubias = o.ubias; a.ubias_ld = lout.nb;
    if (conv_math == 3 && c.wh2) { a.wb3 = c.wh2; a.math = 1; a.wscale = c.h2_scale; a.ovf = ovf_; }
    a.res = o.res; a.res_ld = o.res_ld ? o.res_ld : lout.ld;
    a.aux = o.aux; a.aux_ld = o.aux_ld ? o.aux_ld : lout.ld;
    a.pcm = o.pcm;
    a.Cin = c.Cin; a.Cout = c.Cout; a.Cin_pad = c.Cin_pad; a.Cout_pad = c.Cout_pad;
    if (c.transposed) {
        a.ntap = c.J; a.tap_step = -1; a.tap_off = 0; a.out_stride = c.stride; a.out_off = -c.pad;
        a.transposed = 1; a.n_extra = c.J - 1; a.max_n = lin.max_len + c.J - 1;
    } else {
        a.ntap = c.k; a.tap_step = c.dil; a.tap_off = -(o.pad_l >= 0 ? o.pad_l : c.pad); a.out_stride = 1; a.out_off = 0;
        a.max_n = lout.max_len;
    }
    a.depthwise = c.depthwise;
    a.in_act = o.in_act; a.in_slope = o.slope; a.in_reflect = o.reflect;
    a.epi = o.epi; a.epi_flag = o.epi_flag; a.epi_scale = o.epi_scale; a.H = c.H; a.gate_perm = c.gate_perm;
    a.in_seg = lin.seg; a.out_seg = lout.seg; a.B = lout.nb;
    a.kslices = o.kslices; a.kslice_stride = o.kslice_stride;
    if (o.nsum >= 2) { a.xs1 = o.sum1; a.xs2 = o.sum2; a.nsum = o.nsum; }
    const double positions = c.transposed ? (double)lin.total : (double)lout.total;
    const double fl = 2.0 * c.macs_per_out * positions;
    flops_[cur_stage_] += fl;
    {
        const size_t wfl = c.depthwise ? (size_t)c.k * c.Cout : (size_t)c.k * c.Cin * c.Cout;
        double by = 4.0 * ((double)c.Cin * lin.total + (double)c.Cout * lout.total);
        if (o.res || o.epi == EPI_SUB || o.epi == EPI_RESSKIP) by += 4.0 * (double)c.Cout * lout.total;
        bytes_[cur_stage_] += by;
        bytes_w_[cur_stage_] += 4.0 * (double)wfl;
    }
    if (flops) *flops = fl;
    return a;
}

void Engine::conv(const DConv& c, const float* x, const Lvl& lin, float* y, const Lvl& lout, const ConvOpt& o) {
    double fl = 0;
    ConvArgs a = conv_args(c, x, lin, y, lout, o, &fl);
    const bool can_mfma = conv_mode != 1 && conv_mfma_eligible(a);
    const bool use_bf3 = conv_mode == 0 && conv_math != 1 && o.tile < 0 && conv_bf3_eligible(a) &&
                         (in_mfma_region_ || conv_math == 2 || conv_bf3_blocks(a) >= 384);
    if (use_bf3 && c.transposed && ups_rowph && a.epi == EPI_STORE && !a.ubias && (a.math == 1 ? c.wh2r : c.wb3r)) {
        a.wb3 = a.math == 1 ? c.wh2r : c.wb3r;
        a.bias = c.bias ? c.bias_r : nullptr;
        a.Cout = a.Cout_pad = c.Cout_pad * c.stride;
        a.rowph = c.stride;
    }
    if (a.nsum >= 2 && !(use_bf3 ? conv_bf3_takes_sum(a) : (!can_mfma && conv_cout1_takes(a)))) {
        const float* r[3] = {x, o.sum1, o.sum2};
        sum_scale(o.sum_dst, r, a.nsum, o.sum_n, cur_);
        a.x = o.sum_dst; a.xs1 = a.xs2 = nullptr; a.nsum = 0;
    }
    if (use_bf3) {
        if (in_mfma_region_) { mfma_flops_ += fl; bf16_exec_ += products() * fl; mfma_launches_++; }
        static const int bt = exp_int("STS_BF3_TILE", -1);
        conv_bf3(a, cur_, bt);
    } else if (can_mfma) {
        if (in_mfma_region_) { mfma_flops_ += fl; mfma_exec_ += fl; mfma_launches_++; }
        conv_mfma(a, cur_, o.tile >= 0 ? o.tile : (conv_mode >= 2 ? conv_mode - 2 : -1));
    } else {
        if (a.kslices > 1 && a.kslice_stride > 0)
            (void)hipMemsetAsync(a.y + a.kslice_stride, 0, (size_t)(a.kslices - 1) * (size_t)a.kslice_stride * sizeof(float), cur_);
        conv_generic(a, cur_);
    }
}

int Engine::pick_kslices(const DConv& c, const Lvl& lout) const {
    if (conv_mode != 0 || c.depthwise || c.transposed || c.Cin < 32) return 1;
    const long tiles = (long)((lout.max_len + 31) / 32) * (c.Cout_pad / 32) * lout.nb;
    const long groups = (long)c.k * (c.Cin_pad / 8);
    int s = 1;
    while (s < 8 && tiles * (s * 2) <= 256 && groups / (s * 2) >= 24) s *= 2;
    return s;
}

void Engine::ln(const DLn& l, const float* a, const float* b, const float* res, float* y, const Lvl& lv, int pre_relu, int post_gelu, int nb, long b_stride) {
    LnArgs g;
    memset(&g, 0, sizeof(g));
    g.a = a; g.a_ld = lv.ld; g.b = b; g.b_ld = lv.ld; g.res = res; g.res_ld = lv.ld; g.y = y; g.y_ld = lv.ld;
    g.nb = nb; g.b_stride = b_stride;
    g.gamma = l.g; g.beta = l.b; g.C = l.C; g.pre_relu = pre_relu; g.post_gelu = post_gelu;
    g.seg = lv.seg; g.B = lv.nb; g.max_len = lv.max_len;
    bytes_[cur_stage_] += 4.0 * (double)l.C * (double)lv.total * (2.0 + (b ? 1.0 : 0.0) + (res ? 1.0 : 0.0));
    layer_norm(g, cur_);
}

float* Engine::dds(const DDds& d, float* h, float* t1, float* t2, const Lvl& lv, const DConv* pre, const float* pre_in, const float* pre_res,
                   const SplineTail* tail, bool* tail_done) {
    if (tail_done) *tail_done = false;
    static const bool no_col = exp_flag("STS_NO_COL_LAYER");
    float* cur = h;
    bool pre_pending = pre != nullptr;
    auto run_pre = [&]() {
        if (!pre_pending) return;
        pre_pending = false;
        const float* in = pre_in;
        if (!in) { (void)hipMemsetAsync(t2, 0, (size_t)lv.total * sizeof(float), cur_); in = t2; }
        ConvOpt oa; oa.epi = EPI_RESADD; oa.res = pre_res;
        conv(*pre, in, lv, h, lv, oa);
    };
    for (int i = 0; i < d.n; i++) {
        const DConv& c = d.sep[i];
        const DConv& pw = d.pw[i];
        if (!no_col && conv_mode != 1 && !pw.depthwise && pw.k == 1 && pw.Cin == pw.Cout && pw.Cin == d.n1[i].C && pw.Cin == d.n2[i].C &&
            pw.Cin_pad == pw.Cin) {
            ColLayerArgs g;
            memset(&g, 0, sizeof(g));
            float* nxt = cur == h ? t1 : h;
            g.x = cur; g.x_ld = lv.ld;
            g.dw_w = c.w; g.dw_b = c.bias; g.dw_k = c.k; g.dw_dil = c.dil; g.dw_pad = c.pad; g.dw_ld = c.Cout_pad;
            g.g1 = d.n1[i].g; g.b1 = d.n1[i].b;
            g.wc = pw.wc; g.bias = pw.bias;
            g.g2 = d.n2[i].g; g.b2 = d.n2[i].b; g.post_gelu = 1;
            g.res = cur; g.res_ld = lv.ld; g.y = nxt; g.y_ld = lv.ld; g.C = pw.Cin;
            g.seg = lv.seg; g.B = lv.nb; g.max_len = lv.max_len;
            if (pre_pending && i == 0 && pre->Cin == 1 && pre->k == 1 && pre->Cout == pw.Cin && !pre->depthwise && pre_res) {
                g.x = pre_res; g.res = pre_res; g.xs_w = pre->w; g.xs_b = pre->bias; g.xr = pre_in;
                if (col_layer_eligible(g)) {
                    pre_pending = false;
                    flops_[cur_stage_] += 2.0 * pre->macs_per_out * (double)lv.total;
                } else { g.x = cur; g.res = cur; g.xs_w = g.xs_b = g.xr = nullptr; }
            }
            run_pre();
            if (tail && tail_done && dds_tail && i == d.n - 1 && tail->proj && tail->proj->k == 1 && !tail->proj->depthwise && tail->proj->Cout == 29 &&
                tail->proj->Cout_pad == 32 && tail->proj->Cin == pw.Cin && tail->proj->Cin_pad == pw.Cin && tail->proj->w && tail->proj->bias) {
                ColLayerArgs gt = g;
                gt.tp_w = tail->proj->w; gt.tp_b = tail->proj->bias; gt.tp_fs = tail->filter_sqrt;
                gt.tp_r0 = tail->r0; gt.tp_r1 = tail->r1; gt.tp_o0 = tail->o0; gt.tp_o1 = tail->o1;
                if (col_layer_eligible(gt)) {
                    flops_[cur_stage_] += 2.0 * (c.macs_per_out + pw.macs_per_out + tail->proj->macs_per_out) * (double)lv.total;
                    bytes_[cur_stage_] += 4.0 * ((double)pw.Cin * lv.total + (double)pw.Cin * pw.Cout + (double)pw.Cin * 32 + 4.0 * lv.total);
                    col_layer(gt, cur_);
                    *tail_done = true;
                    return nxt;
                }
            }
            if (col_layer_eligible(g)) {
                flops_[cur_stage_] += 2.0 * (c.macs_per_out + pw.macs_per_out) * (double)lv.total;
                bytes_[cur_stage_] += 4.0 * ((double)pw.Cin * lv.total * 2.0 + (double)pw.Cin * pw.Cout);
                col_layer(g, cur_);
                cur = nxt;
                continue;
            }
        }
        run_pre();
        {
            LnArgs g;
            memset(&g, 0, sizeof(g));
            g.a = cur; g.a_ld = lv.ld; g.y = t2; g.y_ld = lv.ld;
            g.gamma = d.n1[i].g; g.beta = d.n1[i].b; g.C = d.n1[i].C; g.post_gelu = 1;
            g.dw_w = c.w; g.dw_b = c.bias; g.dw_k = c.k; g.dw_dil = c.dil; g.dw_pad = c.pad; g.dw_ld = c.Cout_pad;
            g.seg = lv.seg; g.B = lv.nb; g.max_len = lv.max_len;
            flops_[cur_stage_] += 2.0 * c.macs_per_out * (double)lv.total;
            bytes_[cur_stage_] += 4.0 * (double)g.C * (double)lv.total * 2.0;
            layer_norm(g, cur_);
        }
        float* other = cur == h ? t1 : h;
        conv(pw, t2, lv, other, lv, ConvOpt());
        ln(d.n2[i], other, nullptr, cur, cur, lv, 0, 1);
    }
    return cur;
}

void Engine::tap(const char* name, const float* d, int channels, long ld, long length) {
    if (!record_taps) return;
    Tap& t = taps[name];
    t.channels = channels; t.length = length;
    t.data.resize((size_t)channels * length);
    (void)hipStreamSynchronize(stream);
    (void)hipMemcpy2D(t.data.data(), (size_t)length * sizeof(float), d, (size_t)ld * sizeof(float),
                      (size_t)length * sizeof(float), (size_t)channels, hipMemcpyDeviceToHost);
}

int Engine::set_output_rate(int rate) {
    if (rate == 0) rate = kNativeRate;
    ResampleDesign d;
    if (rate != kNativeRate && !resample_design(kNativeRate, rate, &d)) return fail(STS_EINVAL, "output rate must be 0 or an integer in [8000, 48000] with P = rate / gcd(16000, rate) <= 1024");
    if (rate == out_rate) return STS_OK;
    if (rate == kNativeRate) { out_rate = rate; rs = ResampleDesign(); return STS_OK; }
    std::vector<float> h((size_t)d.P * 2 * d.K);
    resample_table(d, kNativeRate, rate, h.data());
    HIPCK(hipSetDevice(device));
    if (stream) HIPCK(hipStreamSynchronize(stream));
    float* t = nullptr;
    HIPCK(hipMalloc((void**)&t, h.size() * sizeof(float)));
    if (hipMemcpy(t, h.data(), h.size() * sizeof(float), hipMemcpyHostToDevice) != hipSuccess) { (void)hipFree(t); return fail(STS_EDEVICE, "resampler table upload failed"); }
    if (d_rs_table) (void)hipFree(d_rs_table);
    d_rs_table = t; out_rate = rate; rs = d;
    return STS_OK;
}
int Engine::set_loudness(int mode, float target, float peak) {
    if (!loudness_args_valid(mode, target, peak))
        return fail(STS_EINVAL, "loudness: mode 0 (off), 1 (measure) or 2 (normalize), target in [-70, 0] LUFS, ceiling in [-30, 0] dBFS");
    loud_mode = mode; loud_target = target; loud_peak = peak;
    return STS_OK;
}
int Engine::set_limiter(int mode, float gain_db, float ceiling_dbfs, float lookahead_ms) {
    if (!limiter_args_valid(mode, gain_db, ceiling_dbfs, lookahead_ms))
        return fail(STS_EINVAL, "limiter: mode 0 (off) or 1 (on), gain in [-40, 40] dB, ceiling in [-30, 0] dBFS, look-ahead in [0.25, 10] ms");
    lim_mode = mode; lim_gain_db = gain_db; lim_ceiling = ceiling_dbfs; lim_ms = lookahead_ms;
    return STS_OK;
}
int Engine::stream_halo() const {
    const int h = decoder_halo_frames(model);
    long long extra = resampling() ? rs.K : 0;
    if (lim_mode != 0) {
        LimiterDesign d;
        if (limiter_design(out_rate, lim_gain_db, lim_ceiling, lim_ms, &d)) {
            const long long P = resampling() ? rs.P : 1, Q = resampling() ? rs.Q : 1;
            extra += (2LL * d.H * Q + P - 1) / P + 1;
        }
    }
    return h + (int)((extra + model.hop_total - 1) / model.hop_total);
}

int Engine::run_setup(RunCtx& c) {
    Model& M = model;
    const int B = c.B; const int32_t* const* ids = c.ids; const int32_t* n = c.n; const int32_t* sid = c.sid; const float* ls = c.ls;
    std::vector<int>& offT = c.offT; std::vector<int>& lenT = c.lenT;
    offT.assign(B, 0); lenT.assign(B, 0);
    long& Ttot = c.Ttot; int& maxT = c.maxT;
    Ttot = 0; maxT = 0;
    for (int b = 0; b < B; b++) {
        if (n[b] <= 0 || !ids[b]) return fail(STS_EINVAL, "utterance with no phonemes");
        for (int i = 0; i < n[b]; i++)
            if (ids[b][i] < 0 || ids[b][i] >= M.vocab) return fail(STS_EINVAL, "phoneme id outside the model vocabulary");
        offT[b] = (int)Ttot; lenT[b] = n[b]; Ttot += n[b]; if (n[b] > maxT) maxT = n[b];
    }
    if (Ttot > (1 << 24)) return fail(STS_EINVAL, "batch too large");
    if ((size_t)(M.hidden / 2 + 8 + 5 * (size_t)maxT) * 4 > 150 * 1024) return fail(STS_EINVAL, "utterance too long for the attention kernel");
    if (have_forced && (long)forced_dur.size() != Ttot) { have_forced = false; return fail(STS_EINVAL, "forced durations do not match the batch"); }

    c.nz.resize(B);
    for (int b = 0; b < B; b++) {
        c.nz[b] = (int)noise_utt.size() == B ? noise_utt[b] : Noise{noise.ns, noise.nsw, noise.seed + (uint64_t)b};
        if (M.dur_type != 0) c.nz[b].nsw = 0.f;
        c.any_ns |= c.nz[b].ns != 0.f; c.any_nsw |= c.nz[b].nsw != 0.f;
    }

    const int H = c.H = M.hidden, C = c.C = M.inter;
    const int FF = c.FF = M.n_layers ? M.ffn[0].c1.Cout : 0;
    const int fdp = c.fdp = M.dur_type == 0 ? M.sdp_pre.Cout : M.fix_c1.Cout;
    const int wnH = c.wnH = M.n_flows ? M.cp[0].wn.H : 0;
    const int wnL = c.wnL = M.n_flows ? M.cp[0].wn.n : 0;

    Lvl& lvT = c.lvT; lvT = Lvl(); lvT.nb = B; lvT.max_len = maxT; lvT.total = Ttot; lvT.ld = Ttot;
    const int ffn2_slices = c.ffn2_slices = M.n_layers ? pick_kslices(M.ffn[0].c2, lvT) : 1;
    BufT& bt = c.bt;
    auto layoutT = [&](Arena& A) {
        A.used = 0;
        bt.meta_i = A.get<int>((size_t)9 * B + 8 + 5 * (size_t)B + 2 * (size_t)Ttot);
        bt.ls = (float*)(bt.meta_i + ((size_t)9 * B + 8));
        bt.ns = bt.ls + B; bt.nsw = bt.ns + B;
        bt.seed = (uint64_t*)(bt.nsw + B);
        bt.ids = (int*)(bt.seed + B);
        bt.forced = bt.ids + Ttot;
        bt.x = A.get<float>((size_t)H * Ttot); bt.qkv = A.get<float>((size_t)3 * H * Ttot);
        bt.att = A.get<float>((size_t)H * Ttot); bt.y = A.get<float>((size_t)H * Ttot * ffn2_slices);
        bt.x1 = A.get<float>((size_t)H * Ttot); bt.ffh = A.get<float>((size_t)FF * Ttot);
        bt.m = A.get<float>((size_t)C * Ttot);
        bt.logs = (c.any_ns || record_taps) ? A.get<float>((size_t)C * Ttot) : nullptr;
        bt.dh = A.get<float>((size_t)(fdp > H ? fdp : H) * Ttot); bt.dt1 = A.get<float>((size_t)fdp * Ttot);
        bt.dt2 = A.get<float>((size_t)fdp * Ttot); bt.dc = A.get<float>((size_t)fdp * Ttot);
        bt.dhh = A.get<float>((size_t)fdp * Ttot); bt.dp29 = A.get<float>((size_t)29 * Ttot);
        for (auto& r : bt.dr) r = A.get<float>(Ttot);
        bt.dlogw = A.get<float>(Ttot);
        bt.dur = A.get<int>(Ttot + B); bt.cum = A.get<int>(Ttot);
        bt.frames = bt.dur + Ttot;
        bt.g = A.get<float>((size_t)(M.gin > 0 ? M.gin : 1) * B);
        bt.cond_dp = A.get<float>((size_t)(fdp > H ? fdp : H) * B);
        bt.cond_dec = A.get<float>((size_t)(M.up_init > 0 ? M.up_init : 1) * B);
        bt.cond_wn = A.get<float>((size_t)(2 * wnH * wnL + 4) * B * (M.n_flows > 0 ? M.n_flows : 1));
    };
    arenaT_.measuring = true; layoutT(arenaT_);
    if (!ensure(arenaT_, arenaT_.used + 4096)) return fail(STS_EDEVICE, "out of device memory (phoneme-level workspace)");
    arenaT_.measuring = false; layoutT(arenaT_);
    poison_arena(arenaT_);

    const size_t meta_ints = c.meta_ints = (size_t)9 * B + 8;
    const size_t up_bytes = c.up_bytes = (meta_ints + 5 * (size_t)B + 2 * (size_t)Ttot) * 4 + 1024;
    if (!ensure_pinned(up_bytes + ((size_t)Ttot + B) * 4)) return fail(STS_EDEVICE, "pinned host allocation failed");
    int* pm = c.pm = (int*)pinned_;
    int* p_offT = c.p_offT = pm, *p_lenT = c.p_lenT = pm + B, *p_sid = c.p_sid = pm + 2 * B, *p_one = c.p_one = pm + 5 * B;
    c.p_offF = pm + 3 * B; c.p_lenF = pm + 4 * B;
    for (int b = 0; b < B; b++) { p_offT[b] = offT[b]; p_lenT[b] = lenT[b]; p_sid[b] = sid ? sid[b] : 0; }
    p_one[0] = 0; p_one[1] = B;
    if (B == 1) { int* pw0 = pm + 5 * B + 2; c.p_offF[0] = 0; c.p_lenF[0] = 0; pw0[0] = 0; pw0[1] = 0; pw0[2] = 0; }
    int* d_offT = c.d_offT = bt.meta_i, *d_lenT = c.d_lenT = bt.meta_i + B, *d_one = c.d_one = bt.meta_i + 5 * B;
    c.d_sid = bt.meta_i + 2 * B; c.d_offF = bt.meta_i + 3 * B; c.d_lenF = bt.meta_i + 4 * B; c.d_win = bt.meta_i + 5 * B + 2;
    float* p_ls = (float*)(pm + meta_ints);
    for (int b = 0; b < B; b++) p_ls[b] = ls ? ls[b] : 1.0f;
    float* p_ns = p_ls + B; float* p_nsw = p_ns + B; uint64_t* p_seed = (uint64_t*)(p_nsw + B);
    for (int b = 0; b < B; b++) { p_ns[b] = c.nz[b].ns; p_nsw[b] = c.nz[b].nsw; p_seed[b] = c.nz[b].seed; }
    int* p_ids = (int*)(p_seed + B);
    for (int b = 0; b < B; b++) memcpy(p_ids + offT[b], ids[b], sizeof(int) * n[b]);
    int* p_forced = p_ids + Ttot;
    if (have_forced) memcpy(p_forced, forced_dur.data(), sizeof(int) * Ttot);
    HIPCK(hipMemcpyAsync(bt.meta_i, pm, (meta_ints + 5 * (size_t)B + (size_t)Ttot * (have_forced ? 2 : 1)) * 4, hipMemcpyHostToDevice, stream));
    if (B > 1) HIPCK(hipEventRecord(ev_setup_, stream));

    static const bool no_inline_seg_knob = exp_flag("STS_NO_INLINE_SEG");
    const bool no_inline_seg = c.no_inline_seg = no_inline_seg_knob;
    const bool inl = c.inl = B == 1 && !no_inline_seg;
    c.ms = M.is_ms == 1;
    lvT.seg = inl ? SegView{nullptr, nullptr, 1, 0, 0, lenT[0]} : SegView{d_offT, d_lenT, 1, 0, 0, 0};
    Lvl& lvB = c.lvB; lvB = Lvl(); lvB.seg = no_inline_seg ? SegView{d_one, d_one + 1, 1, 0, 0, 0} : SegView{nullptr, nullptr, 1, 0, 0, B};
    lvB.nb = 1; lvB.max_len = B; lvB.total = B; lvB.ld = B;

    return STS_OK;
}

int Engine::run_text_encoder(RunCtx& c) {
    RUN_ALIASES(c)
    stage_begin(0);
    static const bool no_colp = exp_flag("STS_NO_COL_LAYER") || exp_flag("STS_NO_COL_PROJ");
    const long colp_blocks = (long)((Ttot + 15) / 16);
    const bool colp_grid = (long)((maxT + 15) / 16) * B <= 512;
    auto produce_x_and_conv = [&](int l, const DConv& c, float* y) {
        ColProjArgs pj;
        memset(&pj, 0, sizeof(pj));
        pj.x_out = bt.x; pj.x_ld = Ttot; pj.wc = c.wc; pj.bias = c.bias_rows; pj.Cout = c.Cout; pj.npass = (c.Cout + H - 1) / H;
        pj.y = y; pj.y_ld = Ttot; pj.C = H; pj.seg = lvT.seg; pj.B = B; pj.max_len = maxT;
        if (l == 0) { pj.ids = bt.ids; pj.emb = M.emb; pj.vocab = M.vocab; pj.emb_scale = sqrtf((float)M.hidden); }
        else { pj.a = bt.x1; pj.a_ld = Ttot; pj.bp = bt.y; pj.b_ld = Ttot; pj.nb = ffn2_slices; pj.b_stride = (long)H * Ttot;
               pj.gamma = M.ln2[l - 1].g; pj.beta = M.ln2[l - 1].b; }
        const bool ok = !no_colp && conv_mode != 1 && colp_grid && (pj.npass == 1 || colp_blocks >= 24) && c.k == 1 && c.Cin == H && M.emb_size == H && c.wc &&
                        (l == 0 || M.ln2[l - 1].C == H) && col_proj_eligible(pj);
        if (ok) {
            flops_[0] += 2.0 * c.macs_per_out * (double)Ttot;
            bytes_[0] += 4.0 * ((double)H * Ttot * (l == 0 ? 1.0 : 2.0 + ffn2_slices) + (double)c.Cout * Ttot + (double)H * c.Cout);
            col_proj(pj, stream);
            return;
        }
        if (l == 0) embed(bt.ids, M.emb, M.vocab, M.emb_size, sqrtf((float)M.hidden), bt.x, Ttot, (int)Ttot, stream);
        else ln(M.ln2[l - 1], bt.x1, bt.y, nullptr, bt.x, lvT, 0, 0, ffn2_slices, (long)H * Ttot);
        conv(c, bt.x, lvT, y, lvT, ConvOpt());
    };
    for (int l = 0; l < M.n_layers; l++) {
        const DMha& a = M.mha[l];
        produce_x_and_conv(l, a.qkv, bt.qkv);
        AttnArgs at;
        memset(&at, 0, sizeof(at));
        at.q = bt.qkv; at.k = bt.qkv + (size_t)H * Ttot; at.v = bt.qkv + (size_t)2 * H * Ttot; at.o = bt.att; at.ld = Ttot;
        at.relk = a.relk; at.relv = a.relv; at.kc = a.kc; at.px = a.px; at.win = a.win; at.nheads = 2;
        at.seg = lvT.seg; at.B = B; at.max_len = maxT; at.block_min_wgs = attn_block_min_wgs; at.attn_reg = attn_reg;
        attention(at, stream);
        flops_[0] += 2.0 * 2.0 * (double)a.ch * (double)maxT * (double)Ttot;
        bytes_[0] += 4.0 * 4.0 * (double)H * (double)Ttot;
        {
            static const bool no_col = exp_flag("STS_NO_COL_LAYER");
            ColLayerArgs g;
            memset(&g, 0, sizeof(g));
            g.x = bt.att; g.x_ld = Ttot; g.wc = a.o.wc; g.bias = a.o.bias;
            g.add = bt.x; g.add_ld = Ttot; g.g2 = M.ln1[l].g; g.b2 = M.ln1[l].b; g.y = bt.x1; g.y_ld = Ttot; g.C = H;
            g.seg = lvT.seg; g.B = B; g.max_len = maxT;
            if (!no_col && conv_mode != 1 && a.o.Cin == H && a.o.Cout == H && a.o.Cin_pad == H && M.ln1[l].C == H && col_layer_eligible(g)) {
                flops_[0] += 2.0 * a.o.macs_per_out * (double)Ttot;
                bytes_[0] += 4.0 * ((double)H * Ttot * 3.0 + (double)H * H);
                col_layer(g, stream);
            } else {
                conv(a.o, bt.att, lvT, bt.y, lvT, ConvOpt());
                ln(M.ln1[l], bt.x, bt.y, nullptr, bt.x1, lvT, 0, 0);
            }
        }
        const DFfn& f = M.ffn[l];
        ConvOpt o1; o1.pad_l = f.ksize == 1 ? 0 : (f.ksize - 1) / 2;
        conv(f.c1, bt.x1, lvT, bt.ffh, lvT, o1);
        ConvOpt o2 = o1; o2.in_act = 1; o2.slope = 0.f;
        o2.kslices = ffn2_slices; o2.kslice_stride = (long)H * Ttot;
        conv(f.c2, bt.ffh, lvT, bt.y, lvT, o2);
    }
    produce_x_and_conv(M.n_layers, M.proj, bt.m);
    if (bt.logs) conv(M.proj_logs, bt.x, lvT, bt.logs, lvT, ConvOpt());
    tap("x_enc", bt.x, H, Ttot, Ttot);
    tap("m", bt.m, C, Ttot, Ttot);
    if (bt.logs) tap("logs", bt.logs, C, Ttot, Ttot);
    mark(1);
    return STS_OK;
}

int Engine::run_durations(RunCtx& c) {
    Model& M = model;
    const int B = c.B; const StreamSpec* const ss = c.ss; const long Ttot = c.Ttot;
    [[maybe_unused]] const int H = c.H, fdp = c.fdp;
    Lvl &lvT = c.lvT, &lvB = c.lvB; BufT& bt = c.bt;
    const size_t up_bytes = c.up_bytes; int* const pm = c.pm; int* const p_offF = c.p_offF; int* const p_lenF = c.p_lenF;
    int* const d_sid = c.d_sid; int* const d_offF = c.d_offF;
    const bool inl = c.inl, ms = c.ms; const int maxT = c.maxT; (void)maxT;

    stage_begin(1);
    if (ms) gather_speaker(M.emb_g, M.spk_num, M.gin, d_sid, B, bt.g, stream);

    const float* r_final = nullptr;
    if (M.dur_type == 0) {
        ConvOpt op;
        if (ms) { conv(M.sdp_cond, bt.g, lvB, bt.cond_dp, lvB, ConvOpt()); op.ubias = bt.cond_dp; }
        conv(M.sdp_pre, bt.x, lvT, bt.dh, lvT, op);
        const float* dh = dds(M.sdp_dds, bt.dh, bt.dt1, bt.dt2, lvT);
        conv(M.sdp_proj, dh, lvT, bt.dc, lvT, ConvOpt());
        const float *r0 = nullptr, *r1 = nullptr;
        float *n0 = bt.dr[2], *n1 = bt.dr[3], *s0 = bt.dr[0], *s1 = bt.dr[1];
        if (c.any_nsw) { sdp_noise(lvT.seg, B, maxT, bt.nsw, bt.seed, bt.dr[0], bt.dr[1], stream); r0 = bt.dr[0]; r1 = bt.dr[1]; }
        else if (M.sdp_flows <= 1) { HIPCK(hipMemsetAsync(bt.dr[0], 0, (size_t)Ttot * 4, stream)); r0 = bt.dr[0]; }
        for (int i = M.sdp_flows - 1; i > 0; i--) {
            const DConvFlow& cf = M.cf[i];
            const SplineTail tl{&cf.proj, sqrtf((float)cf.filter), r0, r1, n0, n1};
            bool tail_done = false;
            const float* dhh = dds(cf.dds, bt.dhh, bt.dt1, bt.dt2, lvT, &cf.pre, r0, bt.dc, &tl, &tail_done);
            if (!tail_done) {
                conv(cf.proj, dhh, lvT, bt.dp29, lvT, ConvOpt());
                spline_step(bt.dp29, Ttot, sqrtf((float)cf.filter), r0, r1, n0, n1, Ttot, stream);
            }
            r0 = n0; r1 = n1;
            float* t;
            t = n0; n0 = s0; s0 = t;
            t = n1; n1 = s1; s1 = t;
        }
        r_final = r0;
    } else {
        const float* xin = bt.x;
        if (ms) {
            conv(M.fix_cond, bt.g, lvB, bt.cond_dp, lvB, ConvOpt());
            HIPCK(hipMemcpyAsync(bt.dh, bt.x, (size_t)H * Ttot * 4, hipMemcpyDeviceToDevice, stream));
            add_ubias(bt.dh, Ttot, bt.cond_dp, H, lvT.seg, B, maxT, stream);
            xin = bt.dh;
        }
        conv(M.fix_c1, xin, lvT, bt.dt1, lvT, ConvOpt());
        ln(M.fix_n1, bt.dt1, nullptr, nullptr, bt.dt1, lvT, 1, 0);
        conv(M.fix_c2, bt.dt1, lvT, bt.dt2, lvT, ConvOpt());
        ln(M.fix_n2, bt.dt2, nullptr, nullptr, bt.dt2, lvT, 1, 0);
        conv(M.fix_proj, bt.dt2, lvT, bt.dr[0], lvT, ConvOpt());
        r_final = bt.dr[0];
    }
    static const bool no_mapped = exp_flag("STS_NO_MAPPED_SYNC");
    const size_t hm_ints = (size_t)Ttot + B + 1;
    if (!no_mapped && hm_ints > hmap_cap_) {
        (void)hipStreamSynchronize(stream);
        if (hmap_) (void)hipHostFree(hmap_);
        hmap_ = nullptr; hmap_dev_ = nullptr; hmap_cap_ = 0;
        if (hipHostMalloc((void**)&hmap_, (hm_ints * 2 + 64) * 4, hipHostMallocMapped) == hipSuccess &&
            hipHostGetDevicePointer((void**)&hmap_dev_, hmap_, 0) == hipSuccess) { hmap_cap_ = hm_ints * 2 + 64; memset(hmap_, 0, hmap_cap_ * 4); }
        else { if (hmap_) (void)hipHostFree(hmap_); hmap_ = nullptr; hmap_dev_ = nullptr; }
        if (!arrive_ && hipMalloc((void**)&arrive_, 64) == hipSuccess) (void)hipMemsetAsync(arrive_, 0, 64, stream);
    }
    const bool mapped = c.mapped = !no_mapped && hmap_ && arrive_;
    if (mapped) { seq_ = seq_ == 0x7fffffff ? 1 : seq_ + 1; }
    long pred = 0;
    c.req_keys.assign(B, 0ull);
    for (int b = 0; b < B; b++) {
        unsigned long long h = 1469598103934665603ull;
        auto mix = [&h](unsigned v) { for (int q = 0; q < 4; q++) { h ^= (v >> (8 * q)) & 0xffu; h *= 1099511628211ull; } };
        mix((unsigned)c.n[b]);
        if (launch_ahead != 2) {
            mix((unsigned)(c.sid ? c.sid[b] : 0)); { const float lsb = c.ls ? c.ls[b] : 1.0f; unsigned u; memcpy(&u, &lsb, 4); mix(u); }
            for (int t = 0; t < c.n[b]; t++) mix((unsigned)c.ids[b][t]);
        }
        if (c.nz[b].nsw != 0.f) {
            unsigned u; memcpy(&u, &c.nz[b].nsw, 4); mix(u); mix((unsigned)c.nz[b].seed); mix((unsigned)(c.nz[b].seed >> 32));
            h ^= 0x5bd1e995ull; h *= 1099511628211ull;
        }
        c.req_keys[b] = h | 1ull;
    }
    c.predF.clear();
    if (launch_ahead && !ss && !have_forced && !record_taps && mapped) {
        c.predF.resize(B);
        for (int b = 0; b < B; b++) {
            const auto it = seen_tf_.find(c.req_keys[b]);
            if (it == seen_tf_.end()) { c.predF.clear(); break; }
            c.predF[b] = it->second;
        }
    }
    if (B == 1 && !c.predF.empty()) pred = c.predF[0];
    c.ahead = pred > 0;
    c.ahead_b = B > 1 && !c.predF.empty();
    c.hop = M.hop_total;
    const long cap = c.ahead ? (pred + 63) / 64 * 64 : 0;
    durations(r_final, M.dur_type == 0 ? 1 : 0, M.ea_m, M.ea_logs, bt.ls, have_forced ? bt.forced : nullptr, bt.dlogw,
              bt.dur, bt.cum, bt.frames, lvT.seg, B, stream, mapped ? hmap_dev_ : nullptr, Ttot, seq_, arrive_,
              c.ahead ? c.d_lenF : nullptr, c.ahead ? c.d_win + 2 : nullptr, (int)cap);
    c.forced = have_forced;
    have_forced = false;
    mark(2);
    sync_wait_ms_ = 0;
    if (c.ahead) {
        c.Ftot = cap; c.maxF = (int)cap;
        return frame_geometry(c);
    }
    if (c.ahead_b) {
        HIPCK(hipEventSynchronize(ev_setup_));
        c.Ftot = 0; c.maxF = 0;
        for (int b = 0; b < B; b++) {
            const int f = (int)c.predF[b];
            c.p_offF[b] = (int)c.Ftot; c.p_lenF[b] = f; c.Ftot += f; if (f > c.maxF) c.maxF = f;
        }
        return frame_geometry(c);
    }
    int rc = wait_frame_counts(c);
    if (rc != STS_OK) return rc;
    return frame_geometry(c);
}

static inline int wait_class(long phonemes) { int c = 0; while ((1L << (c + 1)) <= phonemes && c < 23) c++; return c; }
void Engine::nap_before_wait(int which, long phonemes) {
    if (!polite_wait) return;
    const WaitEst& e = wait_est_[which][wait_class(phonemes)];
    if (e.us <= 0.0 || e.phonemes <= 0) return;
    const double scale = phonemes < e.phonemes ? (double)phonemes / (double)e.phonemes : 1.0;
    const double nap = e.us * scale * 0.8 - 70.0;
    if (nap < 40.0) return;
    struct timespec ts; ts.tv_sec = (time_t)(nap * 1e-6); ts.tv_nsec = (long)((nap - (double)ts.tv_sec * 1e6) * 1e3);
    (void)nanosleep(&ts, nullptr);
}
void Engine::note_wait(int which, long phonemes, double waited_us, bool was_ready_at_wake) {
    if (!polite_wait) return;
    WaitEst& e = wait_est_[which][wait_class(phonemes)];
    if (e.us <= 0.0) { e.us = waited_us * 0.5; e.phonemes = phonemes; }
    else if (was_ready_at_wake) e.us *= 0.85;
    else { e.us = e.us * 0.7 + waited_us * 0.3; e.phonemes = phonemes; }
}
int Engine::final_sync(long phonemes) {
    if (!polite_wait) { HIPCK(hipStreamSynchronize(stream)); return STS_OK; }
    const double t0 = now_us();
    nap_before_wait(1, phonemes);
// ... 654 lines not shown
```

summertts_amd/csrc/engine.hpp:

```cpp
#pragma once
#include <hip/hip_runtime.h>

#include <deque>
#include <map>
#include <unordered_map>
#include <string>
#include <vector>

#include "../../include/summertts_hip.h"
#include "kernels.hpp"
#include "model.hpp"

namespace sts {

struct Arena {
    char* base = nullptr; size_t cap = 0, used = 0; bool measuring = false;
    void* alloc(size_t bytes) {
        size_t a = (used + 255) & ~(size_t)255;
        used = a + bytes;
        if (measuring) return nullptr;
        return base + a;
    }
    template <typename T> T* get(size_t count) { return (T*)alloc(count * sizeof(T)); }
};

struct Lvl {
    SegView seg; int nb = 0; int max_len = 0; long total = 0; long ld = 0;
};

struct ConvOpt {
    int in_act = 0; float slope = 0.f; int reflect = 0;
    int epi = EPI_STORE, epi_flag = 0; float epi_scale = 1.f;
    const float* res = nullptr; long res_ld = 0;
    float* aux = nullptr; long aux_ld = 0;
    int16_t* pcm = nullptr;
    const float* ubias = nullptr;
    int pad_l = -1;
    int tile = -1;
    int kslices = 1; long kslice_stride = 0;
    const float* sum1 = nullptr; const float* sum2 = nullptr; int nsum = 0; float* sum_dst = nullptr; long sum_n = 0;
};

struct StreamSpec {
    int chunk_frames; int (*cb)(void* user, const int16_t* pcm, int32_t n_samples, int32_t sample_offset); void* user;
    int (*bcb)(void* user, int32_t utt, const int16_t* pcm, int32_t n_samples, int32_t sample_offset) = nullptr;
    int32_t* delivered = nullptr;
};
int decoder_halo_frames(const Model& M);
struct WinGeom;
inline bool noise_scale_valid(float s) { return s >= 0.f && s <= 3.0e38f; }
inline bool loudness_args_valid(int mode, float target, float peak) {
    return mode >= 0 && mode <= 2 && target >= -70.f && target <= 0.f && peak >= -30.f && peak <= 0.f;
}
void limiter_stats_decode(const unsigned* raw, int B, sts_limiter_stats* out);

struct Tap { std::vector<float> data; int channels = 0; long length = 0; };
constexpr int kNativeRate = 16000;

class Engine {
public:
    ~Engine();
    int init(const float* blob, int64_t bytes, int device);
    int run(int B, const int32_t* const* ids, const int32_t* n, const int32_t* sid, const float* ls, const StreamSpec* ss = nullptr);
    int run_once(int B, const int32_t* const* ids, const int32_t* n, const int32_t* sid, const float* ls, const StreamSpec* ss);
    int run_batch_stream(int B, const int32_t* const* ids, const int32_t* n, const int32_t* sid, const float* ls, int chunk_frames,
                         int (*cb)(void*, int32_t, const int16_t*, int32_t, int32_t), void* user, int32_t* n_total);
    const std::string& error() const { return err_; }

    Model model;
    int device = 0;
    std::vector<int32_t> n_samples;
    int64_t total_samples = 0;
    int16_t* d_pcm = nullptr;
    const int16_t* pcm_hbm() const { return pcm_in_host_ ? nullptr : d_pcm; }
    float host_us_setup_ = 0, host_us_enq_ = 0;
    double host_t0_ = 0, host_t_sync_ = 0;
    bool pcm_in_host_ = false;
    const int16_t* h_pcm = nullptr;
    bool host_pcm = false;
    std::vector<int32_t> durations_h;
    std::map<std::string, Tap> taps;
    sts_profile prof{};
    struct Noise { float ns = 0.f, nsw = 0.f; uint64_t seed = 0; };
    Noise noise;
    std::vector<Noise> noise_utt;
    int out_rate = kNativeRate;
    ResampleDesign rs;
    float* d_rs_table = nullptr;
    bool resampling() const { return out_rate != kNativeRate; }
    long long out_count(long long native) const { return resampling() ? (native * rs.P + rs.Q - 1) / rs.Q : native; }
    int set_output_rate(int rate);
    int stream_halo() const;
    int loud_mode = 0; float loud_target = -16.f, loud_peak = -1.f;
    std::vector<sts_loudness> loud_res;
    int set_loudness(int mode, float target, float peak);
    int lim_mode = 0; float lim_gain_db = 0.f, lim_ceiling = -1.f, lim_ms = 5.f;
    std::vector<sts_limiter_stats> lim_res;
    int set_limiter(int mode, float gain_db, float ceiling_dbfs, float lookahead_ms);
    std::vector<int32_t> forced_dur; bool have_forced = false;
    bool record_taps = false; int profiling = 0;
    int conv_mode = 0;
    int conv_math = 3;
    long h2_fallbacks = 0;
    int h2_consecutive = 0; bool h2_disabled = false;
    double products() const { return conv_math == 3 ? 3.0 : 6.0; }
    int pcm_direct = 1;
    int dds_tail = 1;
    int attn_reg = 1;
    int attn_block_min_wgs = 96;
    int launch_ahead = 1;
    long ahead_misses = 0;
    static constexpr size_t kMemoEntries = 1024;
    std::unordered_map<unsigned long long, long> seen_tf_; std::deque<unsigned long long> seen_order_;
    bool polite_wait = false;
    struct WaitEst { double us = 0.0; long phonemes = 0; };
    WaitEst wait_est_[2][24];
    void nap_before_wait(int which, long phonemes);
    void note_wait(int which, long phonemes, double waited_us, bool was_ready_at_wake);
    int final_sync(long phonemes);
    int ups_rowph = 1;
    int tail_fused = 1;
    int chain_streams_dbg = -1;
    int h2p = 1;
    int h2p_tile = -1;
    int flow_fused = 1;
    int stream_retry_step = -1;
    int stream_direct = 0;
    unsigned poison = 0;
    int64_t poison_bytes_ = 0;
    hipStream_t stream = nullptr;

private:
    int fail(int code, const std::string& msg) { err_ = msg; return code; }
    bool ensure(Arena& a, size_t bytes);
    bool ensure_pinned(size_t bytes);
    void poison_arena(const Arena& a);
    void poison_host16(void* p, size_t samples);
    void poison_host32(void* p, size_t words);
    ConvArgs conv_args(const DConv& c, const float* x, const Lvl& lin, float* y, const Lvl& lout, const ConvOpt& o, double* flops);
    void conv(const DConv& c, const float* x, const Lvl& lin, float* y, const Lvl& lout, const ConvOpt& o);
    void ln(const DLn& l, const float* a, const float* b, const float* res, float* y, const Lvl& lv, int pre_relu, int post_gelu, int nb = 1, long b_stride = 0);
    int pick_kslices(const DConv& c, const Lvl& lout) const;
    struct SplineTail { const DConv* proj; float filter_sqrt; const float* r0; const float* r1; float* o0; float* o1; };
    float* dds(const DDds& d, float* h, float* t1, float* t2, const Lvl& lv, const DConv* pre = nullptr, const float* pre_in = nullptr,
               const float* pre_res = nullptr, const SplineTail* tail = nullptr, bool* tail_done = nullptr);
    struct RunCtx;
    struct ResStage;
    int run_setup(RunCtx& c);
    int run_text_encoder(RunCtx& c);
    int run_durations(RunCtx& c);
    int run_frame_workspace(RunCtx& c);
    int run_flow(RunCtx& c);
    int run_decode(RunCtx& c, int nw, long Wtot, int maxW, int zoff0, int wlen0);
    int decode_end(RunCtx& c, const float* wave, const WinGeom& win, long Wtot, int maxW);
    int wait_frame_counts(RunCtx& c);
    int frame_geometry(RunCtx& c);
    int run_output(RunCtx& c);
    int run_stream_steps(RunCtx& c);
    void tap(const char* name, const float* d, int channels, long ld, long length);
    void stage_begin(int s);
    void mark(int i);

    std::string err_;
    Arena arenaT_, arenaF_;
    char* pinned_ = nullptr; size_t pinned_cap_ = 0;
    char* pinned_pcm_ = nullptr; size_t pinned_pcm_cap_ = 0;
    int16_t* pinned_pcm_dev_ = nullptr;
    unsigned* ovf_host_ = nullptr; unsigned* ovf_ = nullptr;
    int* hmap_ = nullptr; int* hmap_dev_ = nullptr; size_t hmap_cap_ = 0;
    unsigned* arrive_ = nullptr; int seq_ = 0;
    float* loud_host_ = nullptr; float* loud_dev_ = nullptr; int loud_cap_ = 0;
    LoudCoef loud_k_{}; int loud_k_rate_ = 0;
    unsigned* lim_host_ = nullptr; int lim_cap_ = 0;
    hipEvent_t ev_[8] = {};
    static constexpr int kAux = 3;
    hipStream_t aux_[kAux] = {};
    hipEvent_t ev_fork_ = nullptr, ev_join_[kAux] = {};
    hipEvent_t ev_setup_ = nullptr;
    hipStream_t cur_ = nullptr;
    bool have_events_ = false;
    int cur_stage_ = 0;
    double flops_[4] = {0, 0, 0, 0};
    double bytes_[4] = {0, 0, 0, 0};
    double bytes_w_[4] = {0, 0, 0, 0};
    double mfma_flops_ = 0, mfma_exec_ = 0, bf16_exec_ = 0, sync_wait_ms_ = 0; int mfma_launches_ = 0; bool in_mfma_region_ = false;
};

}
```

summertts_amd/csrc/kernels.hpp:

```cpp
#pragma once
#include <hip/hip_runtime.h>
#include <stdint.h>

namespace sts {

struct SegView {
    const int* off;
    const int* len;
    int scale;
    int extra;
    int ioff, ilen;
};

enum Epilogue : int {
    EPI_STORE = 0,
    EPI_RESADD = 1,
    EPI_SUB = 3,
    EPI_GATE = 4,
    EPI_RESSKIP = 5,
    EPI_TANH_PCM = 6,
};

struct ConvArgs {
    const float* x; long x_ld;
    float* y; long y_ld;
    const float* w;
    const float* bias;
    const float* ubias; int ubias_ld;
    const float* res; long res_ld;
    float* aux; long aux_ld;
    int16_t* pcm;
    int Cin, Cout, Cin_pad, Cout_pad, ntap;
    int tap_step, tap_off;
    int out_stride, out_off;
    int transposed, n_extra;
    int depthwise;
    int in_act; float in_slope;
    int in_reflect;
    int epi, epi_flag; float epi_scale; int H;
    int gate_perm;
    SegView in_seg, out_seg;
    int B, max_n;
    int kslices; long kslice_stride;
    const float* wu; int wino_n3, wino_n2;
    const void* wb3;
    int keep_lo, keep_hi;
    int math; float wscale; unsigned* ovf;
    const float* xs1; const float* xs2; int nsum;
    int rowph;
};

__host__ __device__ inline void wino_split(int k, int* n3, int* n2) { *n2 = (k % 3 == 0) ? 0 : (k % 3 == 2 ? 1 : 2); *n3 = (k - 2 * *n2) / 3; }
void wino_pack(const float* w, long s_out, long s_tap, long s_in, int Cout, int k, int Cin, int Cin_pad, int Cout_pad, float* dst);
bool conv_wino_eligible(const ConvArgs& a);
void conv_wino(const ConvArgs& a, hipStream_t st);

struct LnArgs {
    const float* a; long a_ld;
    const float* b; long b_ld;
    int nb; long b_stride;
    const float* res; long res_ld;
    float* y; long y_ld;
    const float* gamma; const float* beta;
    int C;
    int pre_relu, post_gelu;
    const float* dw_w; const float* dw_b; int dw_k, dw_dil, dw_pad, dw_ld;
    SegView seg; int B, max_len;
};

struct ColLayerArgs {
    const float* x; long x_ld;
    const float* xs_w; const float* xs_b; const float* xr;
    const float* dw_w; const float* dw_b; int dw_k, dw_dil, dw_pad, dw_ld;
    const float* g1; const float* b1;
    const float* wc; const float* bias;
    const float* add; long add_ld;
    const float* g2; const float* b2; int post_gelu;
    const float* res; long res_ld;
    float* y; long y_ld;
    int C;
    SegView seg; int B, max_len;
    const float* tp_w; const float* tp_b;
    float tp_fs;
    const float* tp_r0; const float* tp_r1;
    float* tp_o0; float* tp_o1;
};
bool col_layer_eligible(const ColLayerArgs& a);
bool col_layer_width_ok(int C);
void col_layer_pack(const float* w, int C, float* dst);
void col_layer(const ColLayerArgs& a, hipStream_t st);

struct ColProjArgs {
    const int* ids; const float* emb; int vocab; float emb_scale;
    const float* a; long a_ld; const float* bp; long b_ld; int nb; long b_stride;
    const float* gamma; const float* beta;
    float* x_out; long x_ld;
    const float* wc; const float* bias; int Cout, npass;
    float* y; long y_ld;
    int C;
    SegView seg; int B, max_len;
};
bool col_proj_eligible(const ColProjArgs& a);
void col_proj(const ColProjArgs& a, hipStream_t st);
void col_proj_pack(const float* w, int C, int Cout, float* dst);

struct AttnArgs {
    const float* q; const float* k; const float* v; float* o; long ld;
    const float* relk; const float* relv;
    int kc, px, win, nheads;
    SegView seg; int B, max_len;
    int block_min_wgs;
    int attn_reg;
};


struct FlowLayerArgs {
    SegView seg; int B, max_len; long tot;
    int H, half, G, Cg, k, halo;
    int layer;
    const float* x0; long x0_ld; const float* pend; int pend_n; long pend_stride; float* x0_out; long x0_out_ld;
    const void* w_pre; const float* b_pre; float s_pre;
    const float* h_in; const float* part_in; int part_n; long part_stride;
    float* h_out;
    float* part_out;
    float* macc; long macc_stride; int macc_init;
    const void* w_gate; const float* b_gate; float s_gate;
    const float* ubias; int ubias_ld;
    const void* w_c; float s_c; int rows_c, rows_res;
    const float* b_res; const float* b_m;
    unsigned* ovf;
};
struct FlowFinishArgs {
    SegView seg; int B, max_len; int half;
    const float* src; long src_ld; float* dst; long dst_ld;
    const float* macc; int n; long macc_stride;
};
bool flow_layer_shape_ok(int H, int half, int k, int dil, int n_layers);
int flow_layer_groups(int H);
void flow_layer(const FlowLayerArgs& a, hipStream_t st);
void flow_finish(const FlowFinishArgs& a, hipStream_t st);

bool conv_mfma_eligible(const ConvArgs& a);
void conv_mfma(const ConvArgs& a, hipStream_t st, int tile = -1);
constexpr int kMaxGroup = 4;
struct ConvGroup { ConvArgs g[kMaxGroup]; int n; };
struct ResLayerArgs {
    const float* x; float* y;
    const float *w1, *b1, *w2, *b2;
    int k1, dil1, k2;
    const float *wu1, *wu2;
    const void *wb1, *wb2;
    float ws1, ws2;
};
struct ResLayerGroup {
    ResLayerArgs g[kMaxGroup];
    int n, C; long ld; float slope;
    SegView seg; int B; int max_n;
    int math; unsigned* ovf;
};
bool resblock_layer_eligible(const ResLayerGroup& G);
void resblock_layer(const ResLayerGroup& G, hipStream_t st);
bool resblock_wino_eligible(const ResLayerGroup& G);
void resblock_wino(const ResLayerGroup& G, hipStream_t st);
bool conv_group_eligible(const ConvGroup& G);
bool conv_bf3_eligible(const ConvArgs& a);
bool conv_bf3_takes_sum(const ConvArgs& a);
bool conv_cout1_takes(const ConvArgs& a);
void conv_bf3(const ConvArgs& a, hipStream_t st, int tile = -1);
long conv_bf3_blocks(const ConvArgs& a);
bool conv_bf3_group_eligible(const ConvGroup& G);
void conv_bf3_group(const ConvGroup& G, hipStream_t st, int tile = -1);
size_t bf3_pack(const float* wp, int nphase, int ntap, int Cin_pad, int Cout_pad, void* dst, bool perm_k = false, int math = 0, float* wscale = nullptr);
bool resblock_bf3_eligible(const ResLayerGroup& G);
void resblock_bf3(const ResLayerGroup& G, hipStream_t st, int variant = -1);
void conv_mfma_group(const ConvGroup& G, hipStream_t st, int tile = -1);

struct H2PArgs {
    const void* xp; long xp_ld;
    const void* wb; float wscale;
    const float* bias;
    const float* res16; long res_ld;
    float* y; long y_ld;
    float* y16; long y16_ld;
    void* yp; long yp_ld; float yp_slope;
    int Cin, Cout, ntap, tap_step, tap_off;
};
struct H2PGroup { H2PArgs g[kMaxGroup]; int n; SegView seg; int B, max_n; unsigned* ovf; };
bool conv_h2p_group_eligible(const H2PGroup& G);
void conv_h2p_group(const H2PGroup& G, hipStream_t st, int tile = -1);
struct H2WArgs {
    const float* x16; long x_ld;
    const void* wu; float wscale;
    const float* bias;
    const float* res16; long res_ld;
    float* y16; long y16_ld;
    float* y; long y_ld;
    float in_slope, out_slope;
    int C, k, dil;
};
struct H2WGroup { H2WArgs g[kMaxGroup]; int n; SegView seg; int B, max_n; unsigned* ovf; };
bool conv_h2w_group_eligible(const H2WGroup& G);
void conv_h2w_group(const H2WGroup& G, hipStream_t st);
int h2w_transform_weights(const float* wp, int k, int Cin, int Cout, float* dst);
void to_x16(const float* x, long x_ld, int C, long n, float* x16, long out_ld, hipStream_t st);
void split_planes(const float* x, long x_ld, int C, const SegView& seg, int nb, long max_n, float slope, void* planes, float* x16, long out_ld,
                  unsigned* ovf, hipStream_t st);
void conv_generic(const ConvArgs& a, hipStream_t st);

void embed(const int* ids, const float* emb, int vocab, int H, float scale, float* x, long ld, int total, hipStream_t st);
void layer_norm(const LnArgs& a, hipStream_t st);
void attention(const AttnArgs& a, hipStream_t st);
void add_ubias(float* y, long ld, const float* u, int C, SegView seg, int B, int max_len, hipStream_t st);
void gather_speaker(const float* emb_g, int spk_num, int gin, const int* sid, int B, float* g, hipStream_t st);
void sum_scale(float* y, const float* const* r, int count, long n, hipStream_t st);
void flip_channels(float* x, long ld, int C, long n, float* tmp, hipStream_t st);

void spline_step(const float* h, long ld, float filter_sqrt, const float* r0, const float* r1,
                 float* o0, float* o1, long n, hipStream_t st);
void durations(const float* r0, int sdp, float ea_m, float ea_logs, const float* ls, const int* forced,
               float* logw_out, int* dur, int* cum, int* frames, SegView seg, int B, hipStream_t st,
               int* host_out = nullptr, long total = 0, int seq = 0, unsigned* arrive = nullptr,
               int* len_out = nullptr, int* win_len_out = nullptr, int cap = 0);
struct PriorNoise { const float* logs; const float* ns; const uint64_t* seed; };
void expand_frames(const float* m, long m_ld, const int* cum, SegView segT, SegView segF, int C,
                   float* z, long z_ld, int B, int max_frames, hipStream_t st, const PriorNoise* nz = nullptr);
void sdp_noise(SegView seg, int B, int max_len, const float* nsw, const uint64_t* seed, float* r0, float* r1, hipStream_t st);

void istft_spectrum(const float* sb, long ld, int rows, float* spec, long total, hipStream_t st);
void istft_ola(const float* spec, long ld, int bands, int band_rows, SegView seg_frames, float* tm, long tm_ld,
               SegView seg_tm, int B, int max_n, hipStream_t st);
void synth_fir(const float* tm, long tm_ld, SegView seg_tm, const float* fir, int ntap, int pad, float gain, float bias,
               float* wave, int16_t* pcm, SegView seg_out, int B, int max_n, hipStream_t st);
bool istft_tail_fused_ok(int bands, int ntap, int pad);
void istft_tail_fused(const float* sb, long ld, SegView seg_frames, const float* fir, int ntap, int pad, float gain, float bias, float* wave, int16_t* pcm,
                      SegView seg_out, int B, int max_n, hipStream_t st);
void quantize_pcm(const float* wave, int16_t* pcm, long n, hipStream_t st);

constexpr int kResampleMinRate = 8000, kResampleMaxRate = 48000, kResampleMaxP = 1024, kResampleMaxK = 72;
struct ResampleDesign { int P = 1, Q = 1, K = 0; };
bool resample_design(int in_rate, int out_rate, ResampleDesign* d);
void resample_table(const ResampleDesign& d, int in_rate, int out_rate, float* table);
struct ResampleArgs {
    const float* x; SegView seg;
    const float* table; int P, Q, K;
    int16_t* pcm; float* wave_out;
    int stream; long long u0, L_utt, j0, j1;
    const long long* wtab;
};
void resample_pcm(const ResampleArgs& a, int nwin, long long max_out, hipStream_t st);
void stream_pack(const int16_t* src, int16_t* dst, const int* src_off, const int* dst_off, int nwin, long long max_n, hipStream_t st);

constexpr int kLoudMinRate = 8000, kLoudMaxRate = 48000, kLoudPow = 9;
bool kweight_coeffs(int rate, double c[10]);
struct LoudCoef { double c[10]; double Mp[kLoudPow][16]; int S; };
bool loud_coef(int rate, LoudCoef* k);
struct LoudArgs {
    const float* x;
    const int* len; int ilen, scale, P, Q;
    float target, ceiling;
    LoudCoef k;
    long long* utab; double* E; double* tsum; float* tpeak; float* gain;
    float* out;
    int no_clamp;
};
size_t loud_ws_bytes(int B, long long total_samples);
void loud_ws_carve(LoudArgs& a, void* ws, int B, long long total_samples);
void loudness_run(const LoudArgs& a, int B, long long max_len, int16_t* pcm, hipStream_t st);

constexpr int kLimMinRate = 8000, kLimMaxRate = 48000, kLimMaxH = 480;
bool limiter_args_valid(int mode, float gain_db, float ceiling_dbfs, float lookahead_ms);
struct LimiterDesign { int H = 0; double c = 1.0, G = 1.0; };
bool limiter_design(int rate, float gain_db, float ceiling_dbfs, float lookahead_ms, LimiterDesign* d);
struct LimArgs {
    const float* x;
    const int* len; int ilen, scale, P, Q;
    int H; double c, G;
    const float* gloud;
    float* y; int16_t* pcm;
    unsigned* stat;
    const long long* wtab;
    int use_seg1; long long seg1[7];
};
void limiter_run(const LimArgs& a, int B, long long max_out, hipStream_t st);

}
```

summertts_amd/csrc/misc_kernels.hip:

```cpp
#include "kernels.hpp"
#include "devmath.hpp"
#include "knobs.hpp"
#include "noise.hpp"
#include <stdlib.h>

namespace sts {

__device__ __forceinline__ int seg_start(const SegView& s, int b) { return (s.off ? s.off[b] : s.ioff) * s.scale + b * s.extra; }
__device__ __forceinline__ int seg_len(const SegView& s, int b) { return (s.off ? s.len[b] : s.ilen) * s.scale + s.extra; }

__device__ __forceinline__ float wave_sum(float v) {
#pragma unroll
    for (int o = 32; o > 0; o >>= 1) v += __shfl_xor(v, o, 64);
    return v;
}

__global__ void embed_kernel(const int* ids, const float* emb, int vocab, int H, float scale, float* x, long ld, int total) {
    long i = (long)blockIdx.x * blockDim.x + threadIdx.x;
    if (i >= (long)H * total) return;
    int h = (int)(i / total), pos = (int)(i - (long)h * total);
    int id = ids[pos];
    if (id < 0 || id >= vocab) id = 0;
    x[(size_t)h * ld + pos] = emb[(size_t)h * vocab + id] * scale;
}
void embed(const int* ids, const float* emb, int vocab, int H, float scale, float* x, long ld, int total, hipStream_t st) {
    long n = (long)H * total;
    if (n <= 0) return;
    hipLaunchKernelGGL(embed_kernel, dim3((unsigned)((n + 255) / 256)), dim3(256), 0, st, ids, emb, vocab, H, scale, x, ld, total);
}

constexpr int LN_G = 32;
__device__ __forceinline__ float ln_input(const LnArgs& a, int c, size_t p, int pos, int len) {
    float v;
    if (a.dw_w) {
        v = a.dw_b ? a.dw_b[c] : 0.f;
        const float* row = a.a + (size_t)c * a.a_ld + (p - pos);
        int j = 0;
        for (; j + 2 < a.dw_k; j += 3) {
            const int q0 = pos + j * a.dw_dil - a.dw_pad, q1 = q0 + a.dw_dil, q2 = q1 + a.dw_dil;
            const float w0 = a.dw_w[(size_t)j * a.dw_ld + c], w1 = a.dw_w[(size_t)(j + 1) * a.dw_ld + c], w2 = a.dw_w[(size_t)(j + 2) * a.dw_ld + c];
            const float x0 = row[q0 >= 0 && q0 < len ? q0 : pos], x1 = row[q1 >= 0 && q1 < len ? q1 : pos], x2 = row[q2 >= 0 && q2 < len ? q2 : pos];
            v += w0 * ((q0 >= 0 && q0 < len) ? x0 : 0.f);
            v += w1 * ((q1 >= 0 && q1 < len) ? x1 : 0.f);
            v += w2 * ((q2 >= 0 && q2 < len) ? x2 : 0.f);
        }
        for (; j < a.dw_k; j++) {
            const int q = pos + j * a.dw_dil - a.dw_pad;
            if (q >= 0 && q < len) v += a.dw_w[(size_t)j * a.dw_ld + c] * row[q];
        }
    } else {
        v = a.a[(size_t)c * a.a_ld + p];
    }
    if (a.b) {
        if (a.nb > 1) {
            float pb[8];
#pragma unroll
            for (int q = 0; q < 8; q++) pb[q] = q < a.nb ? a.b[(size_t)q * a.b_stride + (size_t)c * a.b_ld + p] : 0.f;
            float bs = pb[0];
#pragma unroll
            for (int q = 1; q < 8; q++) bs += pb[q];
            v += bs;
        } else {
            v += a.b[(size_t)c * a.b_ld + p];
        }
    }
    if (a.pre_relu && v < 0.f) v = 0.f;
    return v;
}
__global__ __launch_bounds__(1024) void layer_norm_kernel(LnArgs a) {
    __shared__ float rs[LN_G][33], rq[LN_G][33];
    const int b = blockIdx.y;
    const int len = seg_len(a.seg, b);
    const int tx = threadIdx.x & 31, cy = threadIdx.x >> 5;
    const int pos = blockIdx.x * 32 + tx;
    const bool live = pos < len;
    const size_t p = (size_t)seg_start(a.seg, b) + (live ? pos : 0);
    constexpr int MAXV = 8;
    float vals[MAXV], gam[MAXV], bet[MAXV], rsd[MAXV];
    float s = 0.f, sq = 0.f;
    if (live) {
#pragma unroll
        for (int u = 0; u < MAXV; u++) {
            const int c = cy + u * LN_G;
            if (c < a.C) { gam[u] = a.gamma[c]; bet[u] = a.beta[c]; rsd[u] = a.res ? a.res[(size_t)c * a.res_ld + p] : 0.f; }
        }
#pragma unroll
        for (int u = 0; u < MAXV; u++) {
            const int c = cy + u * LN_G;
            if (c < a.C) { const float v = ln_input(a, c, p, pos, len); vals[u] = v; s += v; sq += v * v; }
        }
        for (int c = cy + MAXV * LN_G; c < a.C; c += LN_G) { const float v = ln_input(a, c, p, pos, len); s += v; sq += v * v; }
    }
    rs[cy][tx] = s; rq[cy][tx] = sq;
    __syncthreads();
    if (!live) return;
    s = 0.f; sq = 0.f;
#pragma unroll
    for (int k = 0; k < LN_G; k++) { s += rs[k][tx]; sq += rq[k][tx]; }
    const float mean = s / (float)a.C;
    const float scale = (float)(1. / (float)a.C);
    const float var = sq * scale - mean * mean;
    const float den = (float)sqrt((double)var + 1e-05);
    auto finish = [&](int c, float v) {
        float o = ((v - mean) / den) * a.gamma[c] + a.beta[c];
        if (a.post_gelu) o = gelu_ref(o);
        if (a.res) o = a.res[(size_t)c * a.res_ld + p] + o;
        a.y[(size_t)c * a.y_ld + p] = o;
    };
#pragma unroll
    for (int u = 0; u < MAXV; u++) {
        const int c = cy + u * LN_G;
        if (c < a.C) {
            float o = ((vals[u] - mean) / den) * gam[u] + bet[u];
            if (a.post_gelu) o = gelu_ref(o);
            if (a.res) o = rsd[u] + o;
            a.y[(size_t)c * a.y_ld + p] = o;
        }
    }
    for (int c = cy + MAXV * LN_G; c < a.C; c += LN_G) finish(c, ln_input(a, c, p, pos, len));
}
void layer_norm(const LnArgs& a, hipStream_t st) {
    if (a.max_len <= 0 || a.B <= 0) return;
    hipLaunchKernelGGL(layer_norm_kernel, dim3((a.max_len + 31) / 32, a.B), dim3(1024), 0, st, a);
}

__global__ __launch_bounds__(256) void attention_kernel(AttnArgs a) {
    extern __shared__ __attribute__((aligned(16))) float sm[];
    const int b = blockIdx.z, h = blockIdx.y, i = blockIdx.x;
    const int T = seg_len(a.seg, b);
    if (i >= T) return;
    const size_t base = (size_t)seg_start(a.seg, b);
    const int kc = a.kc, tid = threadIdx.x, lane = tid & 63, wave = tid >> 6;
    float* qs = sm;
    float* red = sm + kc;
    float* P = sm + kc + 8;
    float* part = P + T;
    const float sq = sqrtf((float)kc);
    for (int c = tid; c < kc; c += 256) qs[c] = a.q[(size_t)(h * kc + c) * a.ld + base + i] / sq;
    __syncthreads();
    float* qrel = part + 4 * T;
    if (a.win > 0) {
        const int l16 = tid & 15;
        for (int r = tid >> 4; r < a.px; r += 16) {
            float s = 0.f;
            for (int c = l16; c < kc; c += 16) s += qs[c] * a.relk[(size_t)c * a.px + r];
#pragma unroll
            for (int o = 8; o > 0; o >>= 1) s += __shfl_xor(s, o, 16);
            if (l16 == 0) qrel[r] = s;
        }
    }
    const int cw = (kc + 3) / 4, c0 = wave * cw, c1 = c0 + cw < kc ? c0 + cw : kc;
    for (int j = lane; j < T; j += 64) {
        const float* kp = a.k + (size_t)(h * kc) * a.ld + base + j;
        float s0 = 0.f, s1 = 0.f, s2 = 0.f, s3 = 0.f;
        int c = c0;
#pragma unroll 2
        for (; c + 3 < c1; c += 4) {
            s0 += qs[c] * kp[(size_t)c * a.ld];
            s1 += qs[c + 1] * kp[(size_t)(c + 1) * a.ld];
            s2 += qs[c + 2] * kp[(size_t)(c + 2) * a.ld];
            s3 += qs[c + 3] * kp[(size_t)(c + 3) * a.ld];
        }
        for (; c < c1; c++) s0 += qs[c] * kp[(size_t)c * a.ld];
        part[wave * T + j] = (s0 + s1) + (s2 + s3);
    }
    __syncthreads();
    float psum = 0.f;
    for (int j = tid; j < T; j += 256) {
        float sc = (part[j] + part[T + j]) + (part[2 * T + j] + part[3 * T + j]);
        const int r = j - i + a.win;
        if (a.win > 0 && r >= 0 && r < a.px) sc += qrel[r];
        const float e = expf(sc);
        P[j] = e;
        psum += e;
    }
    psum = wave_sum(psum);
    if (lane == 0) red[wave] = psum;
    __syncthreads();
    const float sum = red[0] + red[1] + red[2] + red[3];
    for (int j = tid; j < T; j += 256) P[j] = P[j] / sum;
    __syncthreads();
    for (int cc = tid >> 1; cc < kc; cc += 128) {
        const int jh = tid & 1;
        const int j0 = jh ? (T + 1) / 2 : 0, j1 = jh ? T : (T + 1) / 2;
        const float* vp = a.v + (size_t)(h * kc + cc) * a.ld + base;
        float o0 = 0.f, o1 = 0.f, o2 = 0.f, o3 = 0.f;
        int j = j0;
        for (; j + 3 < j1; j += 4) {
            o0 += P[j] * vp[j]; o1 += P[j + 1] * vp[j + 1]; o2 += P[j + 2] * vp[j + 2]; o3 += P[j + 3] * vp[j + 3];
        }
        for (; j < j1; j++) o0 += P[j] * vp[j];
        float o = (o0 + o1) + (o2 + o3);
        o += __shfl_xor(o, 1, 64);
        if (jh == 0) {
            float orel = 0.f;
            if (a.win > 0) {
                for (int r = 0; r < a.px; r++) {
                    const int jj = i + r - a.win;
                    if (jj >= 0 && jj < T) orel += P[jj] * a.relv[(size_t)cc * a.px + r];
                }
            }
            a.o[(size_t)(h * kc + cc) * a.ld + base + i] = o + orel;
        }
    }
}
constexpr int ATR_CW = 24;
constexpr int ATR_LD = 65;

template <int JPL>
__global__ __launch_bounds__(256) void attention_reg_kernel(AttnArgs a) {
    extern __shared__ __attribute__((aligned(16))) float sm[];
    constexpr int TMAX = 64 * JPL;
    const int b = blockIdx.z, h = blockIdx.y, i = blockIdx.x;
    const int T = seg_len(a.seg, b);
    if (i >= T) return;
    const size_t base = (size_t)seg_start(a.seg, b);
    const int kc = a.kc, px = a.px, win = a.win, tid = threadIdx.x, lane = tid & 63;
    const int wave = __builtin_amdgcn_readfirstlane(tid >> 6);
    float* red = sm;
    float* P = sm + 8;
    float* part = P + TMAX;
    float* qr = part + 4 * TMAX;
    float* buf = qr + 128;
    const int cw = (kc + 3) / 4, c0 = wave * cw, nc = (c0 + cw < kc ? c0 + cw : kc) - c0;
    const float sq = sqrtf((float)kc);

    float qv[ATR_CW], kv[ATR_CW][JPL], rk[ATR_CW], vv[ATR_CW][JPL], rv[16];
    int jc[JPL];
#pragma unroll
    for (int jj = 0; jj < JPL; jj++) jc[jj] = lane + 64 * jj < T ? lane + 64 * jj : T - 1;
    const int occ = tid >> 1, ohf = tid & 1;
    const int occ_c = occ < kc ? occ : kc - 1, lane_px = lane < px ? lane : px - 1;
    const int qch = c0 + lane < kc ? c0 + lane : kc - 1;
    const float qlane = a.q[(size_t)(h * kc + qch) * a.ld + base + i];
#pragma unroll
    for (int c = 0; c < ATR_CW; c++) {
        const int ch = c0 + c < kc ? c0 + c : kc - 1;
#pragma unroll
        for (int jj = 0; jj < JPL; jj++) kv[c][jj] = a.k[(size_t)(h * kc + ch) * a.ld + base + jc[jj]];
    }
    if (win > 0) {
#pragma unroll
        for (int c = 0; c < ATR_CW; c++) {
            const int ch = c0 + c < kc ? c0 + c : kc - 1;
            rk[c] = a.relk[(size_t)ch * px + lane_px];
        }
    }
#pragma unroll
    for (int c = 0; c < ATR_CW; c++) {
        const int ch = c0 + c < kc ? c0 + c : kc - 1;
#pragma unroll
        for (int jj = 0; jj < JPL; jj++) vv[c][jj] = a.v[(size_t)(h * kc + ch) * a.ld + base + jc[jj]];
    }
    if (win > 0) {
#pragma unroll
        for (int r = 0; r < 16; r++) rv[r] = a.relv[(size_t)occ_c * px + (r < px ? r : px - 1)];
    }
    const float qscaled = qlane / sq;
#pragma unroll
    for (int c = 0; c < ATR_CW; c++) {
        const bool live = c < nc;
        qv[c] = __builtin_bit_cast(float, __builtin_amdgcn_readlane(__builtin_bit_cast(int, qscaled), c));
        rk[c] = (live && win > 0) ? rk[c] : 0.f;
#pragma unroll
        for (int jj = 0; jj < JPL; jj++) {
            const bool ok = live && lane + 64 * jj < T;
            kv[c][jj] = ok ? kv[c][jj] : 0.f;
            vv[c][jj] = ok ? vv[c][jj] : 0.f;
        }
    }

#pragma unroll
    for (int jj = 0; jj < JPL; jj++) {
        float s0 = 0.f, s1 = 0.f, s2 = 0.f, s3 = 0.f;
#pragma unroll
// ... 142 lines not shown
        v += __shfl_xor(v, 1, 64); v += __shfl_xor(v, 2, 64); v += __shfl_xor(v, 4, 64); v += __shfl_xor(v, 8, 64);
        if (col == 0) rsum[wave * 16 + 4 * quad + r] = v;
    }
    __syncthreads();
    for (int e = tid; e < ntile * 256; e += 256) {
        const int i = e & 15;
        const float sum = (rsum[i] + rsum[16 + i]) + (rsum[32 + i] + rsum[48 + i]);
        P[e] = P[e] / sum;
    }
    __syncthreads();

    const int nct = kc / 16;
    attn_f32x4 oacc[8];
#pragma unroll
    for (int n = 0; n < 8; n++) oacc[n] = attn_f32x4{0.f, 0.f, 0.f, 0.f};
    for (int j0 = 0; j0 < T; j0 += 64) {
        for (int e0 = tid; e0 < kc * 64; e0 += 256 * 8) {
            float vv[8];
#pragma unroll
            for (int u = 0; u < 8; u++) {
                const int e = e0 + u * 256, c = e >> 6, jj = e & 63;
                vv[u] = (e < kc * 64 && j0 + jj < T) ? a.v[(size_t)(h * kc + c) * a.ld + base + j0 + jj] : 0.f;
            }
#pragma unroll
            for (int u = 0; u < 8; u++) {
                const int e = e0 + u * 256, c = e >> 6, jj = e & 63;
                if (e < kc * 64) vbuf[jj * VLD + c] = vv[u];
            }
        }
        __syncthreads();
        for (int ks = wave; ks < 16; ks += 4) {
            const int jj = 4 * ks + quad;
            if (j0 + 4 * ks >= T) break;
            const float pa = P[(size_t)(j0 + jj) * 16 + col];
#pragma unroll
            for (int n = 0; n < 8; n++)
                if (n < nct) oacc[n] = __builtin_amdgcn_mfma_f32_16x16x4f32(pa, vbuf[jj * VLD + n * 16 + col], oacc[n], 0, 0, 0);
        }
        __syncthreads();
    }
    float* red = vbuf;
#pragma unroll
    for (int n = 0; n < 8; n++)
        if (n < nct) {
#pragma unroll
            for (int r = 0; r < 4; r++) red[((wave * 8 + n) * 64 + lane) * 4 + r] = oacc[n][r];
        }
    __syncthreads();
    for (int e = tid; e < nct * 256; e += 256) {
        const int n = e >> 8, ln = (e >> 2) & 63, r = e & 3;
        const int i = 4 * (ln >> 4) + r, ch = n * 16 + (ln & 15);
        if (i0 + i >= T) continue;
        float o = 0.f;
#pragma unroll
        for (int w = 0; w < 4; w++) o += red[((w * 8 + n) * 64 + ln) * 4 + r];
        float orel = 0.f;
        if (win > 0) {
            float rv[32];
#pragma unroll
            for (int rr = 0; rr < 32; rr++) rv[rr] = rr < px ? a.relv[(size_t)ch * px + rr] : 0.f;
#pragma unroll
            for (int rr = 0; rr < 32; rr++) {
                const int jj = i0 + i + rr - win;
                if (rr < px && jj >= 0 && jj < T) orel += P[(size_t)jj * 16 + i] * rv[rr];
            }
        }
        a.o[(size_t)(h * kc + ch) * a.ld + base + i0 + i] = o + orel;
    }
}

static size_t attention_mfma_lds(const AttnArgs& a, int Tpad) {
    const size_t red = (size_t)4 * 8 * 64 * 4, vb = (size_t)64 * (a.kc + ATT_VLD_PAD);
    return ((size_t)a.kc * 16 + 16 * 32 + 64 + (size_t)Tpad * 16 + (vb > red ? vb : red)) * sizeof(float);
}

void attention(const AttnArgs& a, hipStream_t st) {
    if (a.max_len <= 0 || a.B <= 0) return;
    {
        static const bool no_mfma = exp_flag("STS_NO_ATTN_MFMA");
        const int Tpad = (a.max_len + 63) / 64 * 64;
        const size_t lds = attention_mfma_lds(a, Tpad);
        const long wgs = (long)((a.max_len + 15) / 16) * a.nheads * a.B;
        const long min_wgs = a.block_min_wgs > 0 ? a.block_min_wgs : 96;
        if (!no_mfma && wgs >= min_wgs && a.kc % 16 == 0 && a.kc <= 128 && a.px <= 32 && lds <= 150 * 1024) {
            if (lds > 48 * 1024)
                hipFuncSetAttribute((const void*)attention_mfma_kernel, hipFuncAttributeMaxDynamicSharedMemorySize, (int)lds);
            hipLaunchKernelGGL(attention_mfma_kernel, dim3((a.max_len + 15) / 16, a.nheads, a.B), dim3(256), lds, st, a, Tpad);
            return;
        }
    }
    if (a.attn_reg && a.kc <= 4 * ATR_CW && a.px <= 16 && a.max_len <= 256) {
        if (a.max_len <= 128) hipLaunchKernelGGL(attention_reg_kernel<2>, dim3(a.max_len, a.nheads, a.B), dim3(256), attention_reg_lds(2), st, a);
        else hipLaunchKernelGGL(attention_reg_kernel<4>, dim3(a.max_len, a.nheads, a.B), dim3(256), attention_reg_lds(4), st, a);
        return;
    }
    size_t lds = (size_t)(a.kc + 8 + (a.px > 16 ? a.px : 16) + 5 * (size_t)a.max_len) * sizeof(float);
    if (lds > 48 * 1024)
        hipFuncSetAttribute((const void*)attention_kernel, hipFuncAttributeMaxDynamicSharedMemorySize, (int)lds);
    hipLaunchKernelGGL(attention_kernel, dim3(a.max_len, a.nheads, a.B), dim3(256), lds, st, a);
}

__global__ void add_ubias_kernel(float* y, long ld, const float* u, SegView seg, int B) {
    const int b = blockIdx.z, c = blockIdx.y;
    const int pos = blockIdx.x * 256 + threadIdx.x;
    if (pos >= seg_len(seg, b)) return;
    y[(size_t)c * ld + seg_start(seg, b) + pos] += u[(size_t)c * B + b];
}
void add_ubias(float* y, long ld, const float* u, int C, SegView seg, int B, int max_len, hipStream_t st) {
    if (max_len <= 0 || C <= 0 || B <= 0) return;
    hipLaunchKernelGGL(add_ubias_kernel, dim3((max_len + 255) / 256, C, B), dim3(256), 0, st, y, ld, u, seg, B);
}

__global__ void gather_speaker_kernel(const float* emb_g, int spk_num, int gin, const int* sid, int B, float* g) {
    int i = blockIdx.x * blockDim.x + threadIdx.x;
    if (i >= gin * B) return;
    int c = i / B, b = i - c * B;
    int s = sid[b];
    if (s < 0 || s >= spk_num) s = 0;
    g[i] = emb_g[(size_t)c * spk_num + s];
}
void gather_speaker(const float* emb_g, int spk_num, int gin, const int* sid, int B, float* g, hipStream_t st) {
    int n = gin * B;
    if (n <= 0) return;
    hipLaunchKernelGGL(gather_speaker_kernel, dim3((n + 255) / 256), dim3(256), 0, st, emb_g, spk_num, gin, sid, B, g);
}

struct SumPtrs { const float* r[8]; };
__global__ void sum_scale_kernel(float* y, SumPtrs p, int count, float div, long n, int vec) {
    long i = ((long)blockIdx.x * blockDim.x + threadIdx.x) * 4;
    if (i >= n) return;
    if (vec && i + 3 < n) {
        float4 a = *reinterpret_cast<const float4*>(p.r[0] + i);
        for (int k = 1; k < count; k++) {
            const float4 b = *reinterpret_cast<const float4*>(p.r[k] + i);
            a.x += b.x; a.y += b.y; a.z += b.z; a.w += b.w;
        }
        a.x = a.x / div; a.y = a.y / div; a.z = a.z / div; a.w = a.w / div;
        *reinterpret_cast<float4*>(y + i) = a;
    } else {
        for (long j = i; j < n && j < i + 4; j++) {
            float a = p.r[0][j];
            for (int k = 1; k < count; k++) a += p.r[k][j];
            y[j] = a / div;
        }
    }
}
void sum_scale(float* y, const float* const* r, int count, long n, hipStream_t st) {
    if (n <= 0 || count <= 0 || count > 8) return;
    SumPtrs p;
    for (int k = 0; k < 8; k++) p.r[k] = r[k < count ? k : 0];
    int vec = ((uintptr_t)y & 15) == 0;
    for (int k = 0; k < count; k++) vec = vec && (((uintptr_t)r[k] & 15) == 0);
    long thr = (n + 3) / 4;
    hipLaunchKernelGGL(sum_scale_kernel, dim3((unsigned)((thr + 255) / 256)), dim3(256), 0, st, y, p, count, (float)count, n, vec);
}

__global__ void flip_copy_kernel(const float* x, long ld, int C, long n, float* tmp) {
    long i = (long)blockIdx.x * blockDim.x + threadIdx.x;
    if (i >= n) return;
    const int c = blockIdx.y;
    tmp[(size_t)c * n + i] = x[(size_t)(C - 1 - c) * ld + i];
}
__global__ void copy_back_kernel(float* x, long ld, long n, const float* tmp) {
    long i = (long)blockIdx.x * blockDim.x + threadIdx.x;
    if (i >= n) return;
    const int c = blockIdx.y;
    x[(size_t)c * ld + i] = tmp[(size_t)c * n + i];
}
void flip_channels(float* x, long ld, int C, long n, float* tmp, hipStream_t st) {
    if (n <= 0 || C <= 0) return;
    dim3 g((unsigned)((n + 255) / 256), C);
    hipLaunchKernelGGL(flip_copy_kernel, g, dim3(256), 0, st, x, ld, C, n, tmp);
    hipLaunchKernelGGL(copy_back_kernel, g, dim3(256), 0, st, x, ld, n, tmp);
}

__global__ void spline_step_kernel(const float* h, long ld, float fs, const float* r0, const float* r1,
                                   float* o0, float* o1, long n) {
    long i = (long)blockIdx.x * blockDim.x + threadIdx.x;
    if (i >= n) return;
    float hv[29];
#pragma unroll
    for (int j = 0; j < 29; j++) hv[j] = h[(size_t)j * ld + i];
    const float a = r0 ? r0[i] : 0.f;
    o0[i] = rq_spline_inverse(r1 ? r1[i] : 0.f, hv, fs);
    o1[i] = a;
}
void spline_step(const float* h, long ld, float filter_sqrt, const float* r0, const float* r1, float* o0, float* o1,
                 long n, hipStream_t st) {
    if (n <= 0) return;
    hipLaunchKernelGGL(spline_step_kernel, dim3((unsigned)((n + 127) / 128)), dim3(128), 0, st, h, ld, filter_sqrt, r0, r1, o0, o1, n);
}

constexpr int kMaxDur = 100000;
__global__ __launch_bounds__(256) void durations_kernel(const float* r0, int sdp, float ea_m, float ea_logs,
                                                        const float* ls, const int* forced, float* logw_out,
                                                        int* dur, int* cum, int* frames, SegView seg,
                                                        int* host_out, long total, int seq, unsigned* arrive, int B,
                                                        int* len_out, int* win_len_out, int cap) {
    __shared__ int wsum[4];
    __shared__ int carry_s;
    const int b = blockIdx.x;
    const int T = seg_len(seg, b);
    const size_t base = (size_t)seg_start(seg, b);
    const int tid = threadIdx.x, lane = tid & 63, wave = tid >> 6;
    if (tid == 0) carry_s = 0;
    __syncthreads();
    const float scale = ls[b];
    for (int t0 = 0; t0 < T; t0 += 256) {
        const int t = t0 + tid;
        int d = 0;
        if (t < T) {
            float lw = r0[base + t];
            if (sdp) lw = (lw - ea_m) * expf(ea_logs * (-1.0f));
            if (logw_out) logw_out[base + t] = lw;
            if (forced) d = forced[base + t];
            else {
                const float w = expf(lw) * scale;
                const float c = ceilf(w);
                d = (c >= (float)kMaxDur) ? kMaxDur : (c > 0.f ? (int)c : 0);
            }
            if (d < 0) d = 0;
            dur[base + t] = d;
            if (host_out) host_out[1 + base + t] = d;
        }
        int v = d;
#pragma unroll
        for (int o = 1; o < 64; o <<= 1) { int u = __shfl_up(v, o, 64); if (lane >= o) v += u; }
        if (lane == 63) wsum[wave] = v;
        __syncthreads();
        int pre = carry_s;
        for (int k = 0; k < wave; k++) pre += wsum[k];
        if (t < T) cum[base + t] = pre + v;
        __syncthreads();
        if (tid == 255) carry_s = pre + v;
        __syncthreads();
    }
    if (tid == 0) {
        const int f = carry_s < 1 ? 1 : carry_s;
        frames[b] = f;
        if (len_out) { const int fc = f < cap ? f : cap; len_out[b] = fc; win_len_out[b] = fc; }
    }
    if (host_out) {
        if (tid == 0) host_out[1 + total + b] = carry_s < 1 ? 1 : carry_s;
        __threadfence_system();
        __syncthreads();
        if (tid == 0) {
            const unsigned prev = atomicAdd(arrive, 1u);
            if (prev == (unsigned)B - 1u) {
                *arrive = 0u;
                __threadfence_system();
                __hip_atomic_store(host_out, seq, __ATOMIC_RELEASE, __HIP_MEMORY_SCOPE_SYSTEM);
            }
        }
    }
}
void durations(const float* r0, int sdp, float ea_m, float ea_logs, const float* ls, const int* forced,
               float* logw_out, int* dur, int* cum, int* frames, SegView seg, int B, hipStream_t st,
               int* host_out, long total, int seq, unsigned* arrive, int* len_out, int* win_len_out, int cap) {
    if (B <= 0) return;
    hipLaunchKernelGGL(durations_kernel, dim3(B), dim3(256), 0, st, r0, sdp, ea_m, ea_logs, ls, forced, logw_out, dur, cum, frames, seg,
                       host_out, total, seq, arrive, B, len_out, win_len_out, cap);
}

template <bool NOISE>
__global__ __launch_bounds__(256) void expand_frames_kernel(const float* m, long m_ld, const int* cum, SegView segT,
                                                            SegView segF, int C, float* z, long z_ld, PriorNoise nz) {
    const int b = blockIdx.z;
    const int F = seg_len(segF, b), T = seg_len(segT, b);
    const int f = blockIdx.x * 256 + threadIdx.x;
    if (blockIdx.x * 256 >= F) return;
    const size_t tb = (size_t)seg_start(segT, b), fb = (size_t)seg_start(segF, b);
    __shared__ int cs[1024];
    const bool staged = T <= 1024;
    if (staged) {
        for (int i = threadIdx.x; i < T; i += 256) cs[i] = cum[tb + i];
        __syncthreads();
    }
    if (f >= F) return;
    int lo = 0, hi = T;
    if (staged) { while (lo < hi) { int mid = (lo + hi) >> 1; if (cs[mid] > f) hi = mid; else lo = mid + 1; } }
    else { while (lo < hi) { int mid = (lo + hi) >> 1; if (cum[tb + mid] > f) hi = mid; else lo = mid + 1; } }
    const int c0 = blockIdx.y * 16, c1 = c0 + 16 < C ? c0 + 16 : C;
    if (lo >= T) { for (int c = c0; c < c1; c++) z[(size_t)c * z_ld + fb + f] = 0.f; return; }
    if constexpr (NOISE) {
        const float ns = nz.ns[b];
        if (ns != 0.f) {
            const uint64_t seed = nz.seed[b];
            for (int c = c0; c < c1; c++) {
                const float eps = noise_normal(seed, kNoiseStreamPrior, (uint64_t)c * (uint64_t)F + (uint64_t)f);
                const float v = __fmul_rn(__fmul_rn(eps, nz.logs[(size_t)c * m_ld + tb + lo]), ns);
                z[(size_t)c * z_ld + fb + f] = __fadd_rn(m[(size_t)c * m_ld + tb + lo], v);
            }
            return;
        }
    }
#pragma unroll 4
    for (int c = c0; c < c1; c++) z[(size_t)c * z_ld + fb + f] = m[(size_t)c * m_ld + tb + lo];
}
void expand_frames(const float* m, long m_ld, const int* cum, SegView segT, SegView segF, int C, float* z, long z_ld,
                   int B, int max_frames, hipStream_t st, const PriorNoise* nz) {
    if (B <= 0 || max_frames <= 0) return;
    const dim3 grid((max_frames + 255) / 256, (C + 15) / 16, B);
    if (nz && nz->logs) hipLaunchKernelGGL(expand_frames_kernel<true>, grid, dim3(256), 0, st, m, m_ld, cum, segT, segF, C, z, z_ld, *nz);
    else hipLaunchKernelGGL(expand_frames_kernel<false>, grid, dim3(256), 0, st, m, m_ld, cum, segT, segF, C, z, z_ld, PriorNoise{});
}

// ... 191 lines not shown
```

summertts_amd/csrc/run_ctx.hpp:

```cpp
#pragma once
#include "engine.hpp"

namespace sts {

#define HIPCK(call)                                                                           \
    do {                                                                                      \
        hipError_t e__ = (call);                                                              \
        if (e__ != hipSuccess) return fail(STS_EDEVICE, std::string(#call) + ": " + hipGetErrorString(e__)); \
    } while (0)

struct BufT {
    int *meta_i; float* ls; float *ns, *nsw; uint64_t* seed; int* ids; int* forced;
    float *x, *qkv, *att, *y, *x1, *ffh, *m, *logs;
    float *dh, *dt1, *dt2, *dc, *dhh, *dp29, *dr[4], *dlogw;
    int *dur, *cum, *frames;
    float *g, *cond_dp, *cond_dec, *cond_wn;
};
struct BufF {
    float *z, *h, *acts, *out, *x0, *regA, *regB, *tailA, *tailB, *tailC, *wave, *fliptmp;
    float *ff_h[2], *ff_part[2], *ff_macc[2], *ff_alt;
    int16_t* pcm;
    int16_t* pcm_nat; float* wave_out;
    int16_t* pcm_rs; char* lws;
    char* limws; float* wave_lim;
    char* stab; int16_t* spack; float *gwin, *cond_win;
};
static inline size_t stream_tab_ll_off(int nw) { return ((size_t)(6 * nw + 1) * 4 + 7) & ~(size_t)7; }
static inline size_t stream_tab_lim_off(int nw) { return stream_tab_ll_off(nw) + (size_t)nw * 5 * 8; }
static inline size_t stream_tab_bytes(int nw) { return stream_tab_lim_off(nw) + (size_t)nw * 7 * 8; }

struct Engine::RunCtx {
    int B = 0; const int32_t* const* ids = nullptr; const int32_t* n = nullptr; const int32_t* sid = nullptr; const float* ls = nullptr;
    const StreamSpec* ss = nullptr;
    std::vector<int> offT, lenT; long Ttot = 0; int maxT = 0;
    int H = 0, C = 0, FF = 0, fdp = 0, wnH = 0, wnL = 0, ffn2_slices = 1;
    Lvl lvT, lvB, lv1;
    BufT bt; BufF bf;
    size_t meta_ints = 0, up_bytes = 0;
    int *pm = nullptr, *p_offT = nullptr, *p_lenT = nullptr, *p_sid = nullptr, *p_offF = nullptr, *p_lenF = nullptr, *p_one = nullptr;
    int *d_offT = nullptr, *d_lenT = nullptr, *d_sid = nullptr, *d_offF = nullptr, *d_lenF = nullptr, *d_one = nullptr, *d_win = nullptr;
    bool inl = false, no_inline_seg = false, ms = false;
    long Ftot = 0; int maxF = 0, hop = 0;
    long Fld = 0; int maxFld = 0; bool ahead = false, ahead_b = false, mapped = false, forced = false;
    std::vector<Engine::Noise> nz; bool any_ns = false, any_nsw = false;
    std::vector<unsigned long long> req_keys; std::vector<long> predF;
    int halo = 0; long Wcap = 0; int upS = 1; long Lsb = 0; int sbC = 0;
    long long Ocap = 0;
    bool bstream = false;
    bool use_ff = false; int ffG = 0;
};
#define RUN_ALIASES(c)                                                                                                              \
    [[maybe_unused]] Model& M = model;                                                                                              \
    [[maybe_unused]] const int B = (c).B; [[maybe_unused]] const StreamSpec* const ss = (c).ss;                                     \
    [[maybe_unused]] const long Ttot = (c).Ttot; [[maybe_unused]] const int maxT = (c).maxT;                                        \
    [[maybe_unused]] const int H = (c).H, C = (c).C, FF = (c).FF, fdp = (c).fdp, wnH = (c).wnH, wnL = (c).wnL, ffn2_slices = (c).ffn2_slices; \
    [[maybe_unused]] Lvl &lvT = (c).lvT, &lvB = (c).lvB, &lv1 = (c).lv1;                                                            \
    [[maybe_unused]] BufT& bt = (c).bt; [[maybe_unused]] BufF& bf = (c).bf;                                                         \
    [[maybe_unused]] const size_t up_bytes = (c).up_bytes;                                                                          \
    [[maybe_unused]] int* const pm = (c).pm; [[maybe_unused]] int* const p_offF = (c).p_offF; [[maybe_unused]] int* const p_lenF = (c).p_lenF; \
    [[maybe_unused]] int* const d_sid = (c).d_sid; [[maybe_unused]] int* const d_offF = (c).d_offF; [[maybe_unused]] int* const d_lenF = (c).d_lenF; \
    [[maybe_unused]] int* const d_win = (c).d_win;                                                                                  \
    [[maybe_unused]] const bool inl = (c).inl, no_inline_seg = (c).no_inline_seg, ms = (c).ms;                                      \
    [[maybe_unused]] const long Ftot = (c).Ftot; [[maybe_unused]] const int maxF = (c).maxF, hop = (c).hop;                         \
    [[maybe_unused]] const long Fld = (c).Fld; [[maybe_unused]] const int maxFld = (c).maxFld; [[maybe_unused]] const bool ahead = (c).ahead; \
    [[maybe_unused]] const int halo = (c).halo; [[maybe_unused]] const long Wcap = (c).Wcap, Lsb = (c).Lsb;                         \
    [[maybe_unused]] const int upS = (c).upS, sbC = (c).sbC;                                                                        \
    [[maybe_unused]] const bool use_ff = (c).use_ff; [[maybe_unused]] const int ffG = (c).ffG;

}
```

summertts_amd/engine.py:

```python
from __future__ import annotations

import ctypes as C
import os
import subprocess
from typing import Dict, List, Optional, Sequence

import numpy as np

_HERE = os.path.dirname(os.path.abspath(__file__))
LIB_PATH = os.environ.get("SUMMERTTS_HIP_LIB") or os.path.join(_HERE, "lib", "libsummertts_hip.so")
CSRC = os.path.join(_HERE, "csrc")


def build_library(verbose: bool = False) -> str:
    subprocess.run(["make", "-C", CSRC, "-j8"], check=True, stdout=None if verbose else subprocess.DEVNULL)
    return LIB_PATH


class ModelInfo(C.Structure):
    _fields_ = [("is_multi_speaker", C.c_int32), ("lang_type", C.c_int32), ("dur_pred_type", C.c_int32),
                ("dec_type", C.c_int32), ("vocab", C.c_int32), ("hidden", C.c_int32), ("inter_channels", C.c_int32),
                ("speaker_num", C.c_int32), ("gin_channels", C.c_int32), ("samples_per_frame", C.c_int32),
                ("sample_rate", C.c_int32), ("blob_floats_consumed", C.c_int64)]

# ... 230 lines not shown
        def _cb(user, pcm, n, off):
            arr = np.ctypeslib.as_array(pcm, shape=(n,)).copy()
            t = time.perf_counter() - t0
            chunks.append(arr); times.append(t)
            return 1 if (on_chunk and on_chunk(arr, off, t)) else 0
        CB = C.CFUNCTYPE(C.c_int, C.c_void_p, C.POINTER(C.c_int16), C.c_int32, C.c_int32)
        cb = CB(_cb)
        total = C.c_int32()
        self.lib.sts_infer_ids_stream.argtypes = [C.c_void_p, C.c_void_p, C.c_int32, C.c_int32, C.c_float, C.c_int32, CB,
                                                  C.c_void_p, C.POINTER(C.c_int32)]
        _check(self.lib, self.lib.sts_infer_ids_stream(self.h, a.ctypes.data, a.size, sid, length_scale, chunk_frames, cb, None,
                                                       C.byref(total)))
        return chunks, times

    def infer_batch_stream(self, ids, chunk_frames: int, sid: Optional[Sequence[int]] = None,
                           length_scale: Optional[Sequence[float]] = None, on_chunk=None, n_total: Optional[list] = None):
        import time
        B = len(ids)
        arrs = [np.ascontiguousarray(x, dtype=np.int32) for x in ids]
        ptrs = (C.c_void_p * max(B, 1))(*[a.ctypes.data for a in arrs])
        n = np.array([a.size for a in arrs], dtype=np.int32)
        sid_a = None if sid is None else np.ascontiguousarray(sid, dtype=np.int32)
        ls_a = None if length_scale is None else np.ascontiguousarray(length_scale, dtype=np.float32)
        tot = np.zeros(max(B, 1), dtype=np.int32)
        chunks = [[] for _ in range(B)]
        times = [[] for _ in range(B)]
        t0 = time.perf_counter()

        def _cb(user, utt, pcm, ns, off):
            arr = np.ctypeslib.as_array(pcm, shape=(ns,)).copy() if ns else np.zeros(0, np.int16)
            t = time.perf_counter() - t0
            chunks[utt].append(arr); times[utt].append(t)
            return 1 if (on_chunk and on_chunk(utt, arr, off, t)) else 0
        cb = BATCH_CHUNK_CB(_cb)
        _check(self.lib, self.lib.sts_infer_ids_batch_stream(self.h, B, ptrs, n.ctypes.data,
                                                             None if sid_a is None else sid_a.ctypes.data,
                                                             None if ls_a is None else ls_a.ctypes.data, chunk_frames, cb, None,
                                                             tot.ctypes.data))
        if n_total is not None:
            n_total[:] = [int(v) for v in tot[:B]]
        return chunks, times

    def stream_halo_frames(self) -> int:
        return int(self.lib.sts_stream_halo_frames(self.h))

    def prepare(self, ids: Sequence[Sequence[int]], sid: Optional[Sequence[int]] = None,
                length_scale: Optional[Sequence[float]] = None) -> "PreparedBatch":
        return PreparedBatch(ids, sid, length_scale)

    def run_batch(self, ids, sid: Optional[Sequence[int]] = None, length_scale: Optional[Sequence[float]] = None) -> np.ndarray:
        p = ids if isinstance(ids, PreparedBatch) else PreparedBatch(ids, sid, length_scale)
        _check(self.lib, self.lib.sts_run_batch(self.h, p.B, p.ptrs, p.n_p, p.sid_p, p.ls_p, p.n_out_p, p.total_ref))
        self._total = int(p.total.value)
        self._n_out = p.n_out.copy()
        return self._n_out

    def pcm_host(self, copy: bool = True) -> np.ndarray:
        if not copy:
            ptr, cnt = C.POINTER(C.c_int16)(), C.c_int64()
            _check(self.lib, self.lib.sts_pcm_host_view(self.h, C.byref(ptr), C.byref(cnt)))
            if cnt.value == 0:
                return np.empty(0, np.int16)
            v = np.ctypeslib.as_array(ptr, shape=(cnt.value,))
            v.flags.writeable = False
            return v
        out = np.empty(self._total, np.int16)
        _check(self.lib, self.lib.sts_copy_pcm_host(self.h, out.ctypes.data, out.size))
        return out

    def profile_struct(self) -> "Profile":
        p = Profile()
        _check(self.lib, self.lib.sts_get_profile_ex(self.h, C.byref(p), C.sizeof(p)))
        return p

    def pcm_to_device_ptr(self, ptr: int, capacity: int) -> None:
        _check(self.lib, self.lib.sts_copy_pcm_device(self.h, C.c_void_p(ptr), capacity))

    def infer_batch(self, ids, sid=None, length_scale=None) -> List[np.ndarray]:
        n_out = self.run_batch(ids, sid, length_scale)
        flat = self.pcm_host()
        offs = np.concatenate([[0], np.cumsum(n_out)])
        return [flat[offs[b]:offs[b + 1]].copy() for b in range(len(n_out))]

    def set_forced_durations(self, dur: Optional[Sequence[int]]):
        if dur is None:
            _check(self.lib, self.lib.sts_set_forced_durations(self.h, None, 0))
            return
        d = np.ascontiguousarray(dur, dtype=np.int32)
        _check(self.lib, self.lib.sts_set_forced_durations(self.h, d.ctypes.data, d.size))

    def set_record_taps(self, on: bool):
        _check(self.lib, self.lib.sts_set_record_taps(self.h, 1 if on else 0))

    def set_noise(self, noise_scale: float = 0.0, noise_scale_w: float = 0.0, seed: int = 0):
        _check(self.lib, self.lib.sts_set_noise(self.h, float(noise_scale), float(noise_scale_w), int(seed) & 0xFFFFFFFFFFFFFFFF))

    def noise(self):
        ns, nsw, seed = C.c_float(), C.c_float(), C.c_uint64()
        _check(self.lib, self.lib.sts_get_noise(self.h, C.byref(ns), C.byref(nsw), C.byref(seed)))
        return ns.value, nsw.value, seed.value

    def set_output_rate(self, rate: int):
        _check(self.lib, self.lib.sts_set_output_rate(self.h, int(rate)))

    def output_rate(self) -> int:
        return int(self.lib.sts_get_output_rate(self.h))

    def set_loudness(self, mode: int, target_lufs: float = -16.0, peak_dbfs: float = -1.0):
        _check(self.lib, self.lib.sts_set_loudness(self.h, int(mode), float(target_lufs), float(peak_dbfs)))

    def loudness_mode(self):
        m, t, p = C.c_int(), C.c_float(), C.c_float()
        _check(self.lib, self.lib.sts_get_loudness_mode(self.h, C.byref(m), C.byref(t), C.byref(p)))
        return m.value, t.value, p.value

    def loudness(self) -> np.ndarray:
        n = self.lib.sts_get_loudness(self.h, None, 0)
        if n < 0:
            _check(self.lib, n)
        out = np.zeros(n, LOUDNESS_DTYPE)
        if n:
            rc = self.lib.sts_get_loudness(self.h, out.ctypes.data, n)
            if rc < 0:
                _check(self.lib, rc)
        return out

    def set_limiter(self, mode: int, gain_db: float = 0.0, ceiling_dbfs: float = -1.0, lookahead_ms: float = 5.0):
        _check(self.lib, self.lib.sts_set_limiter(self.h, int(mode), float(gain_db), float(ceiling_dbfs), float(lookahead_ms)))

    def limiter_mode(self):
        m, g, c, l = C.c_int(), C.c_float(), C.c_float(), C.c_float()
        _check(self.lib, self.lib.sts_get_limiter_mode(self.h, C.byref(m), C.byref(g), C.byref(c), C.byref(l)))
        return m.value, g.value, c.value, l.value

    def limiter(self) -> np.ndarray:
        n = self.lib.sts_get_limiter(self.h, None, 0)
        if n < 0:
            _check(self.lib, n)
        out = np.zeros(n, LIMITER_DTYPE)
        if n:
            rc = self.lib.sts_get_limiter(self.h, out.ctypes.data, n)
            if rc < 0:
                _check(self.lib, rc)
        return out

    def set_conv_math(self, mode):
        m = {"bf16x3": 0, "f32": 1, "bf16x3_all": 2, "f16x2": 3}.get(mode, mode)
        _check(self.lib, self.lib.sts_set_conv_math(self.h, int(m)))

    def set_conv_mode(self, mode: int):
        _check(self.lib, self.lib.sts_set_conv_mode(self.h, mode))

    def debug_set(self, key: str, value: int):
        _check(self.lib, self.lib.sts_debug_set(self.h, {"attn_block_min_wgs": 1, "flow_fused": 5, "launch_ahead": 6, "attn_reg": 7, "dds_tail": 8, "pcm_direct": 9, "memo_clear": 10, "h2p": 11, "h2p_tile": 12, "chain_streams": 13, "tail_fused": 14, "ups_rowph": 15, "stream_retry_step": 16, "stream_direct": 17, "poison": 18}[key], int(value)))

    def set_profiling(self, on):
        _check(self.lib, self.lib.sts_set_profiling(self.h, 2 if on == 2 else (1 if on else 0)))

    def profile(self) -> dict:
        p = Profile()
        _check(self.lib, self.lib.sts_get_profile_ex(self.h, C.byref(p), C.sizeof(p)))
        return p.as_dict()

    def tap(self, name: str) -> np.ndarray:
        ptr = C.POINTER(C.c_float)()
        ch, ln = C.c_int32(), C.c_int64()
        _check(self.lib, self.lib.sts_get_tap(self.h, name.encode(), C.byref(ptr), C.byref(ch), C.byref(ln)))
        a = np.ctypeslib.as_array(ptr, shape=(ch.value, ln.value)).copy()
        self.lib.sts_free(ptr)
        return a

    def durations(self, total_phonemes: int) -> np.ndarray:
        d = np.zeros(total_phonemes, np.int32)
        _check(self.lib, self.lib.sts_get_durations(self.h, d.ctypes.data, d.size))
        return d

    def close(self):
        if getattr(self, "h", None) is not None and self.h:
            self.lib.sts_destroy(self.h)
            self.h = None

    def __del__(self):
        try:
            self.close()
        except Exception:
            pass


def debug_conv1d(x: np.ndarray, w: np.ndarray, bias: Optional[np.ndarray], pad: int, dil: int = 1,
                 stride_transposed: int = 0, depthwise: bool = False, in_slope: float = 0.0, in_act: int = 0,
                 mode: int = 0, device: int = 0, iters: int = 0):
    lib = load_library()
    x = np.ascontiguousarray(x, np.float32)
    w = np.ascontiguousarray(w, np.float32)
    cout, k = w.shape[0], w.shape[1]
    b = None if bias is None else np.ascontiguousarray(bias, np.float32)
    y = C.POINTER(C.c_float)()
    lout = C.c_int32()
    ms = C.c_float(0.0)
    _check(lib, lib.sts_debug_conv1d_bench(device, x.ctypes.data, x.shape[0], x.shape[1], w.ctypes.data,
                                           None if b is None else b.ctypes.data, cout, k, pad, dil, stride_transposed,
                                           1 if depthwise else 0, in_slope, in_act, mode, C.byref(y), C.byref(lout),
                                           iters, C.byref(ms)))
    out = np.ctypeslib.as_array(y, shape=(cout, lout.value)).copy()
    lib.sts_free(y)
    return (out, float(ms.value)) if iters > 0 else out


def debug_conv_h2p(x: np.ndarray, w: np.ndarray, bias: Optional[np.ndarray], dil: int = 1, res: Optional[np.ndarray] = None,
                   in_slope: float = 0.1, out_slope: float = 0.1, tile: int = -1, members: int = 1, device: int = 0, iters: int = 0):
    lib = load_library()
    x = np.ascontiguousarray(x, np.float32)
    w = np.ascontiguousarray(w, np.float32)
    cout, k = w.shape[0], w.shape[1]
    b = None if bias is None else np.ascontiguousarray(bias, np.float32)
    r = None if res is None else np.ascontiguousarray(res, np.float32)
    L = x.shape[1]
    y = np.zeros((cout, L), np.float32); y16 = np.zeros((cout, L), np.float32); yp = np.zeros((cout, L), np.float32)
    ms = C.c_float(0.0)
    lib.sts_debug_conv_h2p.argtypes = [C.c_int, C.c_void_p, C.c_int32, C.c_int32, C.c_void_p, C.c_void_p, C.c_int32, C.c_int32, C.c_int32,
                                       C.c_void_p, C.c_float, C.c_float, C.c_int, C.c_int, C.c_void_p, C.c_void_p, C.c_void_p, C.c_int32,
                                       C.POINTER(C.c_float)]
    _check(lib, lib.sts_debug_conv_h2p(device, x.ctypes.data, x.shape[0], L, w.ctypes.data, None if b is None else b.ctypes.data, cout, k, dil,
                                       None if r is None else r.ctypes.data, in_slope, out_slope, tile, members, y.ctypes.data,
                                       y16.ctypes.data, yp.ctypes.data, iters, C.byref(ms)))
    return y, y16, yp, float(ms.value)


def debug_conv_h2w(x: np.ndarray, w: np.ndarray, bias: Optional[np.ndarray], dil: int = 1, res: Optional[np.ndarray] = None,
                   in_slope: float = 0.1, out_slope: float = 1.0, members: int = 1, device: int = 0, iters: int = 0):
    lib = load_library()
    x = np.ascontiguousarray(x, np.float32)
    w = np.ascontiguousarray(w, np.float32)
    c, k = w.shape[0], w.shape[1]
    b = None if bias is None else np.ascontiguousarray(bias, np.float32)
    r = None if res is None else np.ascontiguousarray(res, np.float32)
    L = x.shape[1]
    y = np.zeros((c, L), np.float32); y16 = np.zeros((c, L), np.float32)
    ms = C.c_float(0.0)
    lib.sts_debug_conv_h2w.argtypes = [C.c_int, C.c_void_p, C.c_int32, C.c_int32, C.c_void_p, C.c_void_p, C.c_int32, C.c_int32, C.c_void_p,
                                       C.c_float, C.c_float, C.c_int, C.c_void_p, C.c_void_p, C.c_int32, C.POINTER(C.c_float)]
    _check(lib, lib.sts_debug_conv_h2w(device, x.ctypes.data, c, L, w.ctypes.data, None if b is None else b.ctypes.data, k, dil,
                                       None if r is None else r.ctypes.data, in_slope, out_slope, members, y.ctypes.data, y16.ctypes.data, iters, C.byref(ms)))
    return y, y16, float(ms.value)


def debug_wino_pack(w: np.ndarray) -> np.ndarray:
    lib = load_library()
    w = np.ascontiguousarray(w, dtype=np.float32)
    co, k, ci = w.shape
    cip, cop = (ci + 15) // 16 * 16, (co + 31) // 32 * 32
    nseg = {0: k // 3, 2: (k - 2) // 3 + 1, 1: (k - 4) // 3 + 2}[k % 3]
    out = np.zeros((nseg, 4, cip, cop), np.float32)
    rc = lib.sts_debug_wino_pack(w.ctypes.data_as(C.c_void_p), co, k, ci, out.ctypes.data_as(C.c_void_p), C.c_int64(out.size))
    if rc != nseg:
        raise StsError(f"sts_debug_wino_pack: {rc}")
    return out


class Pool:

    def __init__(self, blob: np.ndarray, device: int = 0, n_engines: int = 2, max_batch: int = 8):
        self.lib = load_library()
        blob = np.ascontiguousarray(blob, dtype=np.float32)
        self.h = C.c_void_p()
        self.lib.sts_pool_last_error.restype = C.c_char_p
        self.lib.sts_pool_submit.restype = C.c_int64
        self.lib.sts_pool_submit.argtypes = [C.c_void_p, C.c_void_p, C.c_int32, C.c_int32, C.c_float]
        self.lib.sts_pool_submit_ex.restype = C.c_int64
        self.lib.sts_pool_submit_ex.argtypes = [C.c_void_p, C.c_void_p, C.c_int32, C.c_int32, C.c_float, C.c_float, C.c_float, C.c_uint64]
        self.lib.sts_pool_wait.argtypes = [C.c_void_p, C.c_int64, C.POINTER(C.POINTER(C.c_int16)), C.POINTER(C.c_int32)]
        self.lib.sts_pool_create.argtypes = [C.c_void_p, C.c_int64, C.c_int, C.c_int, C.c_int, C.POINTER(C.c_void_p)]
        self.lib.sts_pool_destroy.argtypes = [C.c_void_p]
        self.lib.sts_pool_stats.argtypes = [C.c_void_p, C.POINTER(C.c_int64), C.POINTER(C.c_int64)]
        self._streams: Dict[int, object] = {}
        rc = self.lib.sts_pool_create(blob.ctypes.data, blob.nbytes, device, n_engines, max_batch, C.byref(self.h))
        if rc != 0:
            raise StsError(f"sts_pool_create: {rc}: {self.lib.sts_pool_last_error().decode()}")

    def submit_stream(self, ids: Sequence[int], chunk_frames: int, on_chunk, sid: int = 0, length_scale: float = 1.0,
                      noise_scale: float = 0.0, noise_scale_w: float = 0.0, seed: int = 0) -> int:
        a = np.ascontiguousarray(ids, dtype=np.int32)

        def _cb(user, pcm, ns, off):
            arr = np.ctypeslib.as_array(pcm, shape=(ns,)).copy() if ns else np.zeros(0, np.int16)
            return 1 if on_chunk(arr, off) else 0
        cb = CHUNK_CB(_cb)
        t = int(self.lib.sts_pool_submit_stream(self.h, a.ctypes.data, a.size, sid, length_scale, float(noise_scale), float(noise_scale_w),
                                                int(seed) & 0xFFFFFFFFFFFFFFFF, int(chunk_frames), cb, None))
        if t <= 0:
            raise StsError(f"sts_pool_submit_stream: {t}: {self.lib.sts_pool_last_error().decode()}")
        self._streams[t] = cb
        return t

    def submit(self, ids: Sequence[int], sid: int = 0, length_scale: float = 1.0, noise_scale: float = 0.0,
               noise_scale_w: float = 0.0, seed: int = 0) -> int:
        a = np.ascontiguousarray(ids, dtype=np.int32)
        if noise_scale == 0.0 and noise_scale_w == 0.0 and seed == 0:
            t = int(self.lib.sts_pool_submit(self.h, a.ctypes.data, a.size, sid, length_scale))
        else:
            t = int(self.lib.sts_pool_submit_ex(self.h, a.ctypes.data, a.size, sid, length_scale, float(noise_scale),
                                                float(noise_scale_w), int(seed) & 0xFFFFFFFFFFFFFFFF))
        if t <= 0:
            raise StsError(f"sts_pool_submit: {t}: {self.lib.sts_pool_last_error().decode()}")
        return t

    def wait(self, ticket: int) -> np.ndarray:
# ... 167 lines not shown
```

Before: 67.04 million.

## Fuse FFN residual LayerNorm into split-K conv via last-arriver tail

Adds a last-block-arrives tail to the split-K MFMA conv kernel. The final workgroup for each output column tile sums the k-slice partials plus the residual and applies LayerNorm in place, replacing a separate layer_norm launch after FFN conv2 in the text encoder. It is only used when the next column-projection fusion is not eligible. This costs per-tile atomic counters, extra LDS, and serialized LN work in one block per tile, and it adds instrumentation counters and debug hooks.

```diff
diff --git a/include/summertts_hip.h b/include/summertts_hip.h
--- a/include/summertts_hip.h
+++ b/include/summertts_hip.h
@@ -99,6 +99,7 @@
        STS_DBG_FLOW_FUSED = 5  };
 enum { STS_DBG_STREAM_RETRY_STEP = 16, STS_DBG_STREAM_DIRECT = 17 };
 enum { STS_DBG_POISON = 18 };
+enum { STS_DBG_FFN_LN_TAIL = 19, STS_DBG_TAIL_COUNTERS = 20, STS_DBG_GLUE_LAUNCHES = 21 };
 int sts_debug_set(sts_engine* e, int key, int value);
 
 typedef struct sts_profile {
diff --git a/summertts_amd/csrc/capi.hip b/summertts_amd/csrc/capi.hip
--- a/summertts_amd/csrc/capi.hip
+++ b/summertts_amd/csrc/capi.hip
@@ -195,6 +195,9 @@
         case STS_DBG_STREAM_RETRY_STEP: e->eng.stream_retry_step = value < 0 ? -1 : value; return STS_OK;
         case STS_DBG_STREAM_DIRECT: e->eng.stream_direct = value != 0; return STS_OK;
         case STS_DBG_POISON: e->eng.poison = (unsigned)value; return STS_OK;
+        case STS_DBG_FFN_LN_TAIL: e->eng.ffn_ln_tail = value != 0; return STS_OK;
+        case STS_DBG_TAIL_COUNTERS: { const int n = e->eng.tail_counters_nonzero(); return n >= 0 ? n : set_err(STS_EDEVICE, e->eng.error()); }
+        case STS_DBG_GLUE_LAUNCHES: return (int)glue_launches_take();
         default: return set_err(STS_EINVAL, "unknown debug key");
     }
 }
diff --git a/summertts_amd/csrc/conv.hip b/summertts_amd/csrc/conv.hip
--- a/summertts_amd/csrc/conv.hip
+++ b/summertts_amd/csrc/conv.hip
@@ -1,5 +1,6 @@
 #include "kernels.hpp"
 #include "devmath.hpp"
+#include "ln_dev.hpp"
 #include "conv_common.hpp"
 
 namespace sts {
@@ -805,6 +806,62 @@
             });
         });
     }
+}
+
+__device__ __forceinline__ void splitk_ln_tail(const ConvArgs& a, float* red, int b, int nsl, int n0, int out_len, size_t out_base) {
+    const int tid = threadIdx.x;
+    asm volatile("s_waitcnt vmcnt(0)" ::: "memory");
+    __syncthreads();
+    unsigned* ctr = a.tail.ctr + (size_t)b * gridDim.x + blockIdx.x;
+    if (tid == 0) {
+        __builtin_amdgcn_fence(__ATOMIC_RELEASE, "agent");
+        asm volatile("s_waitcnt vmcnt(0)" ::: "memory");
+        const unsigned seen = __hip_atomic_fetch_add(ctr, 1u, __ATOMIC_RELAXED, __HIP_MEMORY_SCOPE_AGENT);
+        const bool last = seen + 1u == gridDim.y * (unsigned)nsl;
+        if (last) {
+            __builtin_amdgcn_fence(__ATOMIC_ACQUIRE, "agent");
+            asm volatile("s_waitcnt vmcnt(0)" ::: "memory");
+        }
+        red[0] = last ? 1.f : 0.f;
+    }
+    __syncthreads();
+    const bool last = red[0] != 0.f;
+    __syncthreads();
+    if (!last) return;
+    const int C = a.Cout;
+    float* vs = red;
+    float* rs = red + (size_t)C * 32;
+    float* rq = rs + LN_G * 33;
+    const int tx = tid & 31, cy0 = tid >> 5, ncy = (int)blockDim.x >> 5;
+    const int n = n0 + tx;
+    const bool live = n < out_len;
+    const size_t p = out_base + (size_t)(live ? n : 0);
+    if (live) {
+#pragma unroll 4
+        for (int c = cy0; c < C; c += ncy) {
+            float v = a.tail.a[(size_t)c * a.tail.a_ld + p];
+            v += ln_partial_sum(a.y, nsl, a.kslice_stride, (size_t)c * a.y_ld + p);
+            vs[c * 32 + tx] = v;
+        }
+    }
+    __syncthreads();
+    for (int cy = cy0; cy < LN_G; cy += ncy) {
+        float s = 0.f, sq = 0.f;
+        if (live)
+            for (int c = cy; c < C; c += LN_G) ln_accumulate(vs[c * 32 + tx], s, sq);
+        rs[cy * 33 + tx] = s; rq[cy * 33 + tx] = sq;
+    }
+    __syncthreads();
+    if (live) {
+        float s = 0.f, sq = 0.f;
+#pragma unroll
+        for (int k = 0; k < LN_G; k++) { s += rs[k * 33 + tx]; sq += rq[k * 33 + tx]; }
+        float mean, den;
+        ln_statistics(s, sq, C, mean, den);
+        for (int c = cy0; c < C; c += ncy)
+            a.tail.y[(size_t)c * a.tail.y_ld + p] = ln_normalize(vs[c * 32 + tx], mean, den, a.tail.gamma[c], a.tail.beta[c]);
+    }
+    if (tid == 0) __hip_atomic_store(ctr, 0u, __ATOMIC_RELAXED, __HIP_MEMORY_SCOPE_AGENT);
 }
 
 template <int MW, int NW>
@@ -957,6 +1014,9 @@
             epi_scalar(a, rowp, opos, v);
         }
     }
+    if constexpr (NW == 1) {
+        if (nsl > 1 && a.tail.ctr) splitk_ln_tail(a, red, b, nsl, n0, out_len, out_base);
+    }
 }
 
 struct TileCfg { int MW, NW, WM, WN; };
@@ -981,6 +1041,15 @@
     if (a.epi == EPI_GATE && !a.gate_perm) return false;
     if (a.epi == EPI_TANH_PCM) return false;
     return true;
+}
+
+bool conv_ln_tail_ok(const ConvArgs& a) {
+    if (!a.tail.ctr || !a.tail.a || !a.tail.gamma || !a.tail.beta || !a.tail.y) return false;
+    if (a.kslices < 2 || a.kslices > 8 || a.kslice_stride <= 0) return false;
+    if (a.transposed || a.epi != EPI_STORE || a.out_stride != 1 || a.out_off != 0) return false;
+    if (a.Cout < 1 || a.Cout > 256 || a.Cout_pad % 32 != 0) return false;
+    if (a.tail.y == a.x || a.tail.y == a.tail.a) return false;
+    return (long)((a.max_n + 31) / 32) * a.B <= kConvTailCounters;
 }
 
 static int pick_tile(const ConvArgs& a, int nphase) {
@@ -1011,6 +1080,10 @@
     while (ks < ks_cap && steps / (ks * 2) >= 6 && (long)mt * nt * nphase * a.B * nsl * ks * 2 <= 4096) ks *= 2;
     dim3 grid(nt, mt * nphase, a.B * nsl);
     size_t lds = (size_t)ks * E * 64 * sizeof(float);
+    if (NW == 1 && nsl > 1 && a.tail.ctr) {
+        const size_t need = ((size_t)a.Cout * 32 + 2 * LN_G * 33) * sizeof(float);
+        if (need > lds) lds = need;
+    }
     hipLaunchKernelGGL((conv_mfma_splitk_kernel<MW, NW>), grid, dim3(ks * 64), lds, st, a, mt);
 }
 
diff --git a/summertts_amd/csrc/engine.hip b/summertts_amd/csrc/engine.hip
--- a/summertts_amd/csrc/engine.hip
+++ b/summertts_amd/csrc/engine.hip
@@ -81,7 +81,7 @@
     a.base = nullptr; a.cap = 0;
     size_t want = bytes + bytes / 4 + (1u << 20);
     if (hipMalloc((void**)&a.base, want) != hipSuccess) { if (hipMalloc((void**)&a.base, bytes) != hipSuccess) return false; want = bytes; }
-    a.cap = want;
+    a.cap = want; a.fresh = true;
     return true;
 }
 
@@ -97,9 +97,9 @@
 }
 
 void Engine::poison_arena(const Arena& a) {
-    if (!poison || !a.base || a.used == 0) return;
-    const size_t words = (a.used + 3) / 4;
-    if (hipMemsetD32Async((hipDeviceptr_t)a.base, (int)poison, words, stream) == hipSuccess) poison_bytes_ += (int64_t)words * 4;
+    if (!poison || !a.base || a.used <= a.keep) return;
+    const size_t words = (a.used - a.keep + 3) / 4;
+    if (hipMemsetD32Async((hipDeviceptr_t)(a.base + a.keep), (int)poison, words, stream) == hipSuccess) poison_bytes_ += (int64_t)words * 4;
 }
 void Engine::poison_host16(void* p, size_t samples) {
     if (!poison || !p) return;
@@ -113,6 +113,16 @@
     uint32_t* q = (uint32_t*)p;
     for (size_t i = 0; i < words; i++) q[i] = poison;
     poison_bytes_ += (int64_t)words * 4;
+}
+
+int Engine::tail_counters_nonzero() {
+    if (!arenaT_.base || arenaT_.keep == 0) return 0;
+    std::vector<unsigned> h(arenaT_.keep / sizeof(unsigned));
+    if (hipSetDevice(device) != hipSuccess || hipStreamSynchronize(stream) != hipSuccess ||
+        hipMemcpy(h.data(), arenaT_.base, arenaT_.keep, hipMemcpyDeviceToHost) != hipSuccess) { fail(STS_EDEVICE, "arrival counters: read-back failed"); return -1; }
+    int n = 0;
+    for (unsigned v : h) n += v != 0;
+    return n;
 }
 
 void Engine::stage_begin(int s) { cur_stage_ = s; }
@@ -151,6 +161,7 @@
     a.epi = o.epi; a.epi_flag = o.epi_flag; a.epi_scale = o.epi_scale; a.H = c.H; a.gate_perm = c.gate_perm;
     a.in_seg = lin.seg; a.out_seg = lout.seg; a.B = lout.nb;
     a.kslices = o.kslices; a.kslice_stride = o.kslice_stride;
+    if (o.tail_done) *o.tail_done = false;
     if (o.nsum >= 2) { a.xs1 = o.sum1; a.xs2 = o.sum2; a.nsum = o.nsum; }
     const double positions = c.transposed ? (double)lin.total : (double)lout.total;
     const double fl = 2.0 * c.macs_per_out * positions;
@@ -189,6 +200,10 @@
         conv_bf3(a, cur_, bt);
     } else if (can_mfma) {
         if (in_mfma_region_) { mfma_flops_ += fl; mfma_exec_ += fl; mfma_launches_++; }
+        if (o.tail && o.tail_done && a.kslices > 1 && o.tile < 0 && conv_mode == 0) {
+            a.tail = *o.tail;
+            if (conv_ln_tail_ok(a)) *o.tail_done = true; else memset(&a.tail, 0, sizeof(a.tail));
+        }
         conv_mfma(a, cur_, o.tile >= 0 ? o.tile : (conv_mode >= 2 ? conv_mode - 2 : -1));
     } else {
         if (a.kslices > 1 && a.kslice_stride > 0)
@@ -381,6 +396,8 @@
     BufT& bt = c.bt;
     auto layoutT = [&](Arena& A) {
         A.used = 0;
+        bt.tail_ctr = A.get<unsigned>(kConvTailCounters);
+        A.keep = (size_t)kConvTailCounters * sizeof(unsigned);
         bt.meta_i = A.get<int>((size_t)9 * B + 8 + 5 * (size_t)B + 2 * (size_t)Ttot);
         bt.ls = (float*)(bt.meta_i + ((size_t)9 * B + 8));
         bt.ns = bt.ls + B; bt.nsw = bt.ns + B;
@@ -407,6 +424,7 @@
     arenaT_.measuring = true; layoutT(arenaT_);
     if (!ensure(arenaT_, arenaT_.used + 4096)) return fail(STS_EDEVICE, "out of device memory (phoneme-level workspace)");
     arenaT_.measuring = false; layoutT(arenaT_);
+    if (arenaT_.fresh) { HIPCK(hipMemsetAsync(arenaT_.base, 0, arenaT_.keep, stream)); arenaT_.fresh = false; }
     poison_arena(arenaT_);
 
     const size_t meta_ints = c.meta_ints = (size_t)9 * B + 8;
@@ -448,16 +466,26 @@
     static const bool no_colp = exp_flag("STS_NO_COL_LAYER") || exp_flag("STS_NO_COL_PROJ");
     const long colp_blocks = (long)((Ttot + 15) / 16);
     const bool colp_grid = (long)((maxT + 15) / 16) * B <= 512;
-    auto produce_x_and_conv = [&](int l, const DConv& c, float* y) {
-        ColProjArgs pj;
+    static const bool no_ln_tail = exp_flag("STS_NO_FFN_LN_TAIL");
+    bool x_done = false;
+    auto col_proj_args = [&](int l, const DConv& c, float* y, ColProjArgs& pj) {
         memset(&pj, 0, sizeof(pj));
         pj.x_out = bt.x; pj.x_ld = Ttot; pj.wc = c.wc; pj.bias = c.bias_rows; pj.Cout = c.Cout; pj.npass = (c.Cout + H - 1) / H;
         pj.y = y; pj.y_ld = Ttot; pj.C = H; pj.seg = lvT.seg; pj.B = B; pj.max_len = maxT;
         if (l == 0) { pj.ids = bt.ids; pj.emb = M.emb; pj.vocab = M.vocab; pj.emb_scale = sqrtf((float)M.hidden); }
         else { pj.a = bt.x1; pj.a_ld = Ttot; pj.bp = bt.y; pj.b_ld = Ttot; pj.nb = ffn2_slices; pj.b_stride = (long)H * Ttot;
                pj.gamma = M.ln2[l - 1].g; pj.beta = M.ln2[l - 1].b; }
-        const bool ok = !no_colp && conv_mode != 1 && colp_grid && (pj.npass == 1 || colp_blocks >= 24) && c.k == 1 && c.Cin == H && M.emb_size == H && c.wc &&
-                        (l == 0 || M.ln2[l - 1].C == H) && col_proj_eligible(pj);
+        return !no_colp && conv_mode != 1 && colp_grid && (pj.npass == 1 || colp_blocks >= 24) && c.k == 1 && c.Cin == H && M.emb_size == H && c.wc &&
+               (l == 0 || M.ln2[l - 1].C == H) && col_proj_eligible(pj);
+    };
+    auto produce_x_and_conv = [&](int l, const DConv& c, float* y) {
+        ColProjArgs pj;
+        const bool ok = col_proj_args(l, c, y, pj);
+        if (x_done) {
+            x_done = false;
+            conv(c, bt.x, lvT, y, lvT, ConvOpt());
+            return;
+        }
         if (ok) {
             flops_[0] += 2.0 * c.macs_per_out * (double)Ttot;
             bytes_[0] += 4.0 * ((double)H * Ttot * (l == 0 ? 1.0 : 2.0 + ffn2_slices) + (double)c.Cout * Ttot + (double)H * c.Cout);
@@ -500,7 +528,14 @@
         conv(f.c1, bt.x1, lvT, bt.ffh, lvT, o1);
         ConvOpt o2 = o1; o2.in_act = 1; o2.slope = 0.f;
         o2.kslices = ffn2_slices; o2.kslice_stride = (long)H * Ttot;
+        ConvLnTail tl{bt.tail_ctr, bt.x1, Ttot, M.ln2[l].g, M.ln2[l].b, bt.x, Ttot};
+        if (ffn_ln_tail && !no_ln_tail && ffn2_slices > 1 && M.ln2[l].C == H && f.c2.Cout == H) {
+            const bool more = l + 1 < M.n_layers;
+            ColProjArgs pj;
+            if (!col_proj_args(l + 1, more ? M.mha[l + 1].qkv : M.proj, more ? bt.qkv : bt.m, pj)) { o2.tail = &tl; o2.tail_done = &x_done; }
+        }
         conv(f.c2, bt.ffh, lvT, bt.y, lvT, o2);
+        if (x_done) bytes_[0] += 4.0 * (double)H * (double)Ttot * 3.0;
     }
     produce_x_and_conv(M.n_layers, M.proj, bt.m);
     if (bt.logs) conv(M.proj_logs, bt.x, lvT, bt.logs, lvT, ConvOpt());
diff --git a/summertts_amd/csrc/engine.hpp b/summertts_amd/csrc/engine.hpp
--- a/summertts_amd/csrc/engine.hpp
+++ b/summertts_amd/csrc/engine.hpp
@@ -15,6 +15,7 @@
 
 struct Arena {
     char* base = nullptr; size_t cap = 0, used = 0; bool measuring = false;
+    size_t keep = 0; bool fresh = false;
     void* alloc(size_t bytes) {
         size_t a = (used + 255) & ~(size_t)255;
         used = a + bytes;
@@ -38,6 +39,7 @@
     int pad_l = -1;
     int tile = -1;
     int kslices = 1; long kslice_stride = 0;
+    const ConvLnTail* tail = nullptr; bool* tail_done = nullptr;
     const float* sum1 = nullptr; const float* sum2 = nullptr; int nsum = 0; float* sum_dst = nullptr; long sum_n = 0;
 };
 
@@ -105,6 +107,8 @@
     int h2_consecutive = 0; bool h2_disabled = false;
     double products() const { return conv_math == 3 ? 3.0 : 6.0; }
     int pcm_direct = 1;
+    int ffn_ln_tail = 1;
+    int tail_counters_nonzero();
     int dds_tail = 1;
     int attn_reg = 1;
     int attn_block_min_wgs = 96;
diff --git a/summertts_amd/csrc/kernels.hpp b/summertts_amd/csrc/kernels.hpp
--- a/summertts_amd/csrc/kernels.hpp
+++ b/summertts_amd/csrc/kernels.hpp
@@ -19,6 +19,14 @@
     EPI_GATE = 4,
     EPI_RESSKIP = 5,
     EPI_TANH_PCM = 6,
+};
+
+constexpr int kConvTailCounters = 512;
+struct ConvLnTail {
+    unsigned* ctr;
+    const float* a; long a_ld;
+    const float* gamma; const float* beta;
+    float* y; long y_ld;
 };
 
 struct ConvArgs {
@@ -42,6 +50,7 @@
     SegView in_seg, out_seg;
     int B, max_n;
     int kslices; long kslice_stride;
+    ConvLnTail tail;
     const float* wu; int wino_n3, wino_n2;
     const void* wb3;
     int keep_lo, keep_hi;
@@ -142,6 +151,7 @@
 
 bool conv_mfma_eligible(const ConvArgs& a);
 void conv_mfma(const ConvArgs& a, hipStream_t st, int tile = -1);
+bool conv_ln_tail_ok(const ConvArgs& a);
 constexpr int kMaxGroup = 4;
 struct ConvGroup { ConvArgs g[kMaxGroup]; int n; };
 struct ResLayerArgs {
@@ -213,6 +223,7 @@
 void add_ubias(float* y, long ld, const float* u, int C, SegView seg, int B, int max_len, hipStream_t st);
 void gather_speaker(const float* emb_g, int spk_num, int gin, const int* sid, int B, float* g, hipStream_t st);
 void sum_scale(float* y, const float* const* r, int count, long n, hipStream_t st);
+long glue_launches_take();
 void flip_channels(float* x, long ld, int C, long n, float* tmp, hipStream_t st);
 
 void spline_step(const float* h, long ld, float filter_sqrt, const float* r0, const float* r1,
diff --git a/summertts_amd/csrc/ln_dev.hpp b/summertts_amd/csrc/ln_dev.hpp
--- /dev/null
+++ b/summertts_amd/csrc/ln_dev.hpp
@@ -0,0 +1,26 @@
+#pragma once
+#include <hip/hip_runtime.h>
+
+namespace sts {
+
+constexpr int LN_G = 32;
+
+__device__ __forceinline__ float ln_partial_sum(const float* b, int nb, long b_stride, size_t off) {
+    float pb[8];
+#pragma unroll
+    for (int q = 0; q < 8; q++) pb[q] = q < nb ? b[(size_t)q * b_stride + off] : 0.f;
+    float bs = pb[0];
+#pragma unroll
+    for (int q = 1; q < 8; q++) bs += pb[q];
+    return bs;
+}
+__device__ __forceinline__ void ln_accumulate(float v, float& s, float& sq) { s += v; sq += v * v; }
+__device__ __forceinline__ void ln_statistics(float s, float sq, int C, float& mean, float& den) {
+    mean = s / (float)C;
+    const float scale = (float)(1. / (float)C);
+    const float var = sq * scale - mean * mean;
+    den = (float)sqrt((double)var + 1e-05);
+}
+__device__ __forceinline__ float ln_normalize(float v, float mean, float den, float gamma, float beta) { return ((v - mean) / den) * gamma + beta; }
+
+}
diff --git a/summertts_amd/csrc/misc_kernels.hip b/summertts_amd/csrc/misc_kernels.hip
--- a/summertts_amd/csrc/misc_kernels.hip
+++ b/summertts_amd/csrc/misc_kernels.hip
@@ -1,10 +1,20 @@
 #include "kernels.hpp"
 #include "devmath.hpp"
+#include "ln_dev.hpp"
 #include "knobs.hpp"
 #include "noise.hpp"
 #include <stdlib.h>
+#include <string.h>
+#include <atomic>
 
 namespace sts {
+
+static std::atomic<long> g_glue_launches{0};
+static void count_glue_launch() {
+    const char* v = getenv("STS_TEST_HOOKS");
+    if (v && !strcmp(v, "1")) g_glue_launches.fetch_add(1, std::memory_order_relaxed);
+}
+long glue_launches_take() { return g_glue_launches.exchange(0, std::memory_order_relaxed); }
 
 __device__ __forceinline__ int seg_start(const SegView& s, int b) { return (s.off ? s.off[b] : s.ioff) * s.scale + b * s.extra; }
 __device__ __forceinline__ int seg_len(const SegView& s, int b) { return (s.off ? s.len[b] : s.ilen) * s.scale + s.extra; }
@@ -26,10 +36,10 @@
 void embed(const int* ids, const float* emb, int vocab, int H, float scale, float* x, long ld, int total, hipStream_t st) {
     long n = (long)H * total;
     if (n <= 0) return;
+    count_glue_launch();
     hipLaunchKernelGGL(embed_kernel, dim3((unsigned)((n + 255) / 256)), dim3(256), 0, st, ids, emb, vocab, H, scale, x, ld, total);
 }
 
-constexpr int LN_G = 32;
 __device__ __forceinline__ float ln_input(const LnArgs& a, int c, size_t p, int pos, int len) {
     float v;
     if (a.dw_w) {
@@ -53,13 +63,7 @@
     }
     if (a.b) {
         if (a.nb > 1) {
-            float pb[8];
-#pragma unroll
-            for (int q = 0; q < 8; q++) pb[q] = q < a.nb ? a.b[(size_t)q * a.b_stride + (size_t)c * a.b_ld + p] : 0.f;
-            float bs = pb[0];
-#pragma unroll
-            for (int q = 1; q < 8; q++) bs += pb[q];
-            v += bs;
+            v += ln_partial_sum(a.b, a.nb, a.b_stride, (size_t)c * a.b_ld + p);
         } else {
             v += a.b[(size_t)c * a.b_ld + p];
         }
@@ -87,9 +91,9 @@
 #pragma unroll
         for (int u = 0; u < MAXV; u++) {
             const int c = cy + u * LN_G;
-            if (c < a.C) { const float v = ln_input(a, c, p, pos, len); vals[u] = v; s += v; sq += v * v; }
-        }
-        for (int c = cy + MAXV * LN_G; c < a.C; c += LN_G) { const float v = ln_input(a, c, p, pos, len); s += v; sq += v * v; }
+            if (c < a.C) { const float v = ln_input(a, c, p, pos, len); vals[u] = v; ln_accumulate(v, s, sq); }
+        }
+        for (int c = cy + MAXV * LN_G; c < a.C; c += LN_G) ln_accumulate(ln_input(a, c, p, pos, len), s, sq);
     }
     rs[cy][tx] = s; rq[cy][tx] = sq;
     __syncthreads();
@@ -97,12 +101,10 @@
     s = 0.f; sq = 0.f;
 #pragma unroll
     for (int k = 0; k < LN_G; k++) { s += rs[k][tx]; sq += rq[k][tx]; }
-    const float mean = s / (float)a.C;
-    const float scale = (float)(1. / (float)a.C);
-    const float var = sq * scale - mean * mean;
-    const float den = (float)sqrt((double)var + 1e-05);
+    float mean, den;
+    ln_statistics(s, sq, a.C, mean, den);
     auto finish = [&](int c, float v) {
-        float o = ((v - mean) / den) * a.gamma[c] + a.beta[c];
+        float o = ln_normalize(v, mean, den, a.gamma[c], a.beta[c]);
         if (a.post_gelu) o = gelu_ref(o);
         if (a.res) o = a.res[(size_t)c * a.res_ld + p] + o;
         a.y[(size_t)c * a.y_ld + p] = o;
@@ -111,7 +113,7 @@
     for (int u = 0; u < MAXV; u++) {
         const int c = cy + u * LN_G;
         if (c < a.C) {
-            float o = ((vals[u] - mean) / den) * gam[u] + bet[u];
+            float o = ln_normalize(vals[u], mean, den, gam[u], bet[u]);
             if (a.post_gelu) o = gelu_ref(o);
             if (a.res) o = rsd[u] + o;
             a.y[(size_t)c * a.y_ld + p] = o;
@@ -121,6 +123,7 @@
 }
 void layer_norm(const LnArgs& a, hipStream_t st) {
     if (a.max_len <= 0 || a.B <= 0) return;
+    count_glue_launch();
     hipLaunchKernelGGL(layer_norm_kernel, dim3((a.max_len + 31) / 32, a.B), dim3(1024), 0, st, a);
 }
 
@@ -569,6 +572,7 @@
     int vec = ((uintptr_t)y & 15) == 0;
     for (int k = 0; k < count; k++) vec = vec && (((uintptr_t)r[k] & 15) == 0);
     long thr = (n + 3) / 4;
+    count_glue_launch();
     hipLaunchKernelGGL(sum_scale_kernel, dim3((unsigned)((thr + 255) / 256)), dim3(256), 0, st, y, p, count, (float)count, n, vec);
 }
 
diff --git a/summertts_amd/csrc/run_ctx.hpp b/summertts_amd/csrc/run_ctx.hpp
--- a/summertts_amd/csrc/run_ctx.hpp
+++ b/summertts_amd/csrc/run_ctx.hpp
@@ -15,6 +15,7 @@
     float *dh, *dt1, *dt2, *dc, *dhh, *dp29, *dr[4], *dlogw;
     int *dur, *cum, *frames;
     float *g, *cond_dp, *cond_dec, *cond_wn;
+    unsigned* tail_ctr;
 };
 struct BufF {
     float *z, *h, *acts, *out, *x0, *regA, *regB, *tailA, *tailB, *tailC, *wave, *fliptmp;
diff --git a/summertts_amd/engine.py b/summertts_amd/engine.py
--- a/summertts_amd/engine.py
+++ b/summertts_amd/engine.py
@@ -406,7 +406,13 @@
         _check(self.lib, self.lib.sts_set_conv_mode(self.h, mode))
 
     def debug_set(self, key: str, value: int):
-        _check(self.lib, self.lib.sts_debug_set(self.h, {"attn_block_min_wgs": 1, "flow_fused": 5, "launch_ahead": 6, "attn_reg": 7, "dds_tail": 8, "pcm_direct": 9, "memo_clear": 10, "h2p": 11, "h2p_tile": 12, "chain_streams": 13, "tail_fused": 14, "ups_rowph": 15, "stream_retry_step": 16, "stream_direct": 17, "poison": 18}[key], int(value)))
+        _check(self.lib, self.lib.sts_debug_set(self.h, {"attn_block_min_wgs": 1, "flow_fused": 5, "launch_ahead": 6, "attn_reg": 7, "dds_tail": 8, "pcm_direct": 9, "memo_clear": 10, "h2p": 11, "h2p_tile": 12, "chain_streams": 13, "tail_fused": 14, "ups_rowph": 15, "stream_retry_step": 16, "stream_direct": 17, "poison": 18, "ffn_ln_tail": 19}[key], int(value)))
+
+    def debug_get(self, key: str) -> int:
+        rc = self.lib.sts_debug_set(self.h, {"tail_counters": 20, "glue_launches": 21}[key], 0)
+        if rc < 0:
+            _check(self.lib, rc)
+        return rc
 
     def set_profiling(self, on):
         _check(self.lib, self.lib.sts_set_profiling(self.h, 2 if on == 2 else (1 if on else 0)))
```

New measurement: 65.59 million. 0.978x the previous value.
